# lehduong/Knowledge-Distillation-by-Replacing-Cheap-Conv

Measured on AMD Instinct MI355X. Metric: images/sec KD train step, DeepLabV3+(WRN38) student 1024x2048, higher is better.
Workload: dtype bf16; 1 GPU; KD train step (teacher fwd + student fwd + CE/KD/hint criteria + hint bwd + RAdam), DeepLabV3+(WRN-38) student P92, 1024x2048, 8 img/GPU, random init, teacher through the HIP engine; plan=P92, mode=A, arch=deeplab, hint_loss=mse, per_gpu_batch=8, global_batch=8, parallelism=dp1, teacher_backend=hip, ranks_seen=1

## Files before the change

include/kdcc.h:

```cpp
#ifndef KDCC_H
#define KDCC_H

#include <stddef.h>
#include <stdint.h>

#ifdef __cplusplus
extern "C" {
#endif

typedef void *kd_stream_t;

enum { KD_F32 = 0, KD_BF16 = 1 };
enum {
    KD_OK = 0,
    KD_ERR_INVALID = -1,
    KD_ERR_UNSUPPORTED = -2,
    KD_ERR_WORKSPACE = -3,
    KD_ERR_HIP = -4
};

int kd_version(void);
const char *kd_last_error(void);

typedef struct kd_conv_desc {
    int32_t dtype;
    int32_t N, H, W, Cin;
    int32_t Ho, Wo, Cout;
    int32_t kh, kw, stride, pad, dil;
    int32_t ldx;
} kd_conv_desc;

typedef struct kd_conv_epilogue {
    const void *res_pre;  int32_t ld_res_pre;
    const void *mask;     int32_t ld_mask;     const float *mask_scale;
    const void *res_post; int32_t ld_res_post;
    void *out_raw;        int32_t ld_raw;      int32_t raw_f32;
    void *out_act;        int32_t ld_act;      const float *act_scale; const float *act_shift; int32_t act_relu;
    float *bn_sums;
    const void *cls_w;    float *cls_out;      int32_t ld_cls;      int32_t ncls;
} kd_conv_epilogue;
int32_t kd_conv2d_cls_supported(const kd_conv_desc *d, const kd_conv_epilogue *ep);

int kd_conv2d_fwd(const kd_conv_desc *d, const void *x, const void *w_packed,
                  const kd_conv_epilogue *ep, kd_stream_t stream);
int32_t kd_conv2d_bn_sums_rows(const kd_conv_desc *d, const kd_conv_epilogue *ep);
size_t kd_bn_sums_finish_workspace(int32_t rows, int32_t C);
int kd_bn_sums_finish(const float *part, int32_t rows, int32_t C, float *s1, float *s2, void *workspace, size_t workspace_bytes,
                      kd_stream_t stream);

int32_t kd_conv1x1_dual_supported(const kd_conv_desc *d, int32_t Cin2, int32_t ldx2, const kd_conv_epilogue *ep);
int kd_conv1x1_dual_fwd(const kd_conv_desc *d, const void *x, const void *x2, int32_t Cin2, int32_t ldx2, const void *w_cat,
                        const kd_conv_epilogue *ep, kd_stream_t stream);

int kd_conv_set_persist_cus(int32_t n);

enum { KD_PACK_FWD = 0, KD_PACK_DGRAD = 1 };
int kd_pack_conv_weight(const float *src, void *dst, int32_t dtype, int32_t mode,
                        int32_t Cout, int32_t Cin, int32_t kh, int32_t kw, int32_t cin_pad,
                        kd_stream_t stream);

size_t kd_pw_wgrad_workspace(int32_t M, int32_t Cin, int32_t Cout);
int kd_pw_wgrad(int32_t dtype, int32_t M, int32_t Cin, int32_t Cout,
                const void *a, int32_t lda, const void *dy, int32_t ldy,
                float *dw, int32_t accumulate, void *workspace, size_t workspace_bytes,
                kd_stream_t stream);

size_t kd_conv2d_wgrad_workspace(const kd_conv_desc *d);
int kd_conv2d_wgrad(const kd_conv_desc *d, const void *x, const void *dy, int32_t ld_dy, float *dw,
                    int32_t accumulate, void *workspace, size_t workspace_bytes, kd_stream_t stream);

typedef struct kd_dw_desc {
    int32_t dtype;
    int32_t N, H, W, C;
    int32_t k, pad, dil;
    int32_t ldx, ldy;
} kd_dw_desc;
typedef struct kd_dw_epilogue {
    const void *res_pre;  int32_t ld_res_pre;
    const void *mask;     int32_t ld_mask;     const float *mask_scale;
    const void *res_post; int32_t ld_res_post;
} kd_dw_epilogue;
int kd_pack_dw_weight(const float *src , float *dst ,
                      int32_t C, int32_t k, int32_t flip, kd_stream_t stream);
int kd_dwconv_fwd(const kd_dw_desc *d, const void *x, const float *w_taps, const float *bias,
                  const kd_dw_epilogue *ep, void *y, kd_stream_t stream);
int kd_dwconv_fwd_sum(const kd_dw_desc *d, int32_t n, const void *const *xs, const float *const *w_taps, void *y,
                      kd_stream_t stream);
int kd_dwconv_fwd_fanout(const kd_dw_desc *d, int32_t n, const void *x, const float *const *w_taps, void *const *ys,
                         kd_stream_t stream);
size_t kd_dwconv_wgrad_workspace(const kd_dw_desc *d);
int kd_dwconv_wgrad(const kd_dw_desc *d, const void *x, const void *dy, int32_t ld_dy,
                    float *dw, int32_t accumulate, void *workspace, size_t workspace_bytes,
                    kd_stream_t stream);
size_t kd_dwconv_wgrad_multi_workspace(const kd_dw_desc *d, int32_t n);
int kd_dwconv_wgrad_multi(const kd_dw_desc *d, int32_t n, const void *x, const void *const *dys, int32_t ld_dy,
                          float *const *dws, int32_t accumulate, void *workspace, size_t workspace_bytes,
                          kd_stream_t stream);

int64_t kd_lattice_rows(int32_t N, int32_t H, int32_t W, int32_t dil);
int32_t kd_dwconv_lattice_ok(const kd_dw_desc *d, int32_t n);
int kd_lattice_rows_move(int32_t dtype, int32_t N, int32_t H, int32_t W, int32_t C, int32_t dil, void *img, int32_t ld_img,
                         void *rows, int32_t ld_rows, int32_t to_rows, kd_stream_t stream);
int kd_dwconv_fwd_fanout_lattice(const kd_dw_desc *d, int32_t n, const void *x, const float *const *w_taps, void *const *ys,
                                 kd_stream_t stream);
int kd_dwconv_fwd_sum_lattice(const kd_dw_desc *d, int32_t n, const void *const *xs, const float *const *w_taps, void *y,
                              kd_stream_t stream);
int kd_dwconv_wgrad_multi_lattice(const kd_dw_desc *d, int32_t n, const void *x, const void *const *dys, float *const *dws,
                                  int32_t accumulate, void *workspace, size_t workspace_bytes ,
                                  kd_stream_t stream);

int kd_stem_conv(int32_t dtype, const float *x_nchw, const float *w, void *y,
                 int32_t N, int32_t H, int32_t W, kd_stream_t stream);
int kd_stem_conv_pool(const float *x_nchw, const float *w, void *y_raw, void *y_act, const float *scale,
                      const float *shift, int32_t N, int32_t H, int32_t W, kd_stream_t stream);

int kd_maxpool3x3s2(int32_t dtype, const void *x, int32_t ldx, void *y_raw, int32_t ld_raw,
                    void *y_act, int32_t ld_act, const float *scale, const float *shift,
                    int32_t N, int32_t H, int32_t W, int32_t C, kd_stream_t stream);

int kd_upsample_bilinear_ac(const void *x, int32_t x_dtype, int32_t ldx, void *y, int32_t y_dtype, int32_t ldy,
                            int32_t N, int32_t H, int32_t W, int32_t C, int32_t Ho, int32_t Wo,
                            kd_stream_t stream);

int kd_upsample_bilinear(const void *x, int32_t x_dtype, int32_t ldx, void *y, int32_t y_dtype, int32_t ldy,
// ... 279 lines not shown
```

knowledge-distillation-by-replacing-cheap-conv_amd/_lib.py:

```python
import ctypes as C
import os

_HERE = os.path.dirname(os.path.abspath(__file__))
_sel = os.environ.get("KDCC_LIB", "")
LIB_PATH = (os.path.join(_HERE, "libkdcc_hip_tuning.so") if _sel == "tuning" else _sel if _sel.endswith(".so")
            else os.path.join(_HERE, "libkdcc_hip.so"))


def build_tuning():
    import subprocess
    subprocess.check_call(["make", "-s", "-j", str(min(8, os.cpu_count() or 1)), "-C", os.path.join(_HERE, "csrc"), "TUNING=1"])

KD_F32, KD_BF16 = 0, 1
KD_PACK_FWD, KD_PACK_DGRAD = 0, 1
KD_ERR_UNSUPPORTED = -2
KD_CIFAR_NCHW, KD_CIFAR_NHWC = 0, 1
KD_SEG_NCHW, KD_SEG_NHWC = 0, 1
KD_OPT_SGD, KD_OPT_ADAM, KD_OPT_ADAMW_REF = 0, 1, 2
KD_OPT_FIRST, KD_OPT_NESTEROV, KD_OPT_AMSGRAD, KD_OPT_MAXIMIZE = 1, 2, 4, 8

c_int, c_i64, c_f, c_vp, c_sz = C.c_int32, C.c_int64, C.c_float, C.c_void_p, C.c_size_t


class ConvDesc(C.Structure):
    _fields_ = [(n, c_int) for n in ("dtype", "N", "H", "W", "Cin", "Ho", "Wo", "Cout", "kh", "kw", "stride", "pad",
                                     "dil", "ldx")]


class ConvEpilogue(C.Structure):
    _fields_ = [("res_pre", c_vp), ("ld_res_pre", c_int),
                ("mask", c_vp), ("ld_mask", c_int), ("mask_scale", c_vp),
                ("res_post", c_vp), ("ld_res_post", c_int),
                ("out_raw", c_vp), ("ld_raw", c_int), ("raw_f32", c_int),
                ("out_act", c_vp), ("ld_act", c_int), ("act_scale", c_vp), ("act_shift", c_vp), ("act_relu", c_int),
                ("bn_sums", c_vp),
                ("cls_w", c_vp), ("cls_out", c_vp), ("ld_cls", c_int), ("ncls", c_int)]


class DwDesc(C.Structure):
    _fields_ = [(n, c_int) for n in ("dtype", "N", "H", "W", "C", "k", "pad", "dil", "ldx", "ldy")]


class RadamTensor(C.Structure):
    _fields_ = [("p", c_vp), ("g", c_vp), ("exp_avg", c_vp), ("exp_avg_sq", c_vp), ("n", c_i64), ("step", c_int),
                ("lr", c_f), ("beta1", c_f), ("beta2", c_f), ("eps", c_f), ("weight_decay", c_f)]


class OptimTensor(C.Structure):
    _fields_ = [("p", c_vp), ("g", c_vp), ("state", c_vp * 3), ("n", c_i64), ("step", c_i64), ("flags", c_int), ("reserved", c_int),
                ("lr", C.c_double), ("weight_decay", C.c_double), ("eps", C.c_double), ("momentum", C.c_double),
                ("dampening", C.c_double), ("beta1", C.c_double), ("beta2", C.c_double), ("warmup", C.c_double)]


class DwEpilogue(C.Structure):
    _fields_ = [("res_pre", c_vp), ("ld_res_pre", c_int), ("mask", c_vp), ("ld_mask", c_int), ("mask_scale", c_vp),
                ("res_post", c_vp), ("ld_res_post", c_int)]


class DConvDesc(C.Structure):
    _fields_ = [(n, c_int) for n in ("N", "C", "H", "W", "K", "kh", "kw", "stride", "pad", "dil", "groups")]


class View3(C.Structure):
    _fields_ = [("ptr", c_vp), ("dtype", c_int), ("sN", c_i64), ("sC", c_i64), ("sP", c_i64)]


class HrView(C.Structure):
    _fields_ = [("ptr", c_vp), ("H", c_int), ("W", c_int), ("ld", c_int)]


KD_MULTI_MAX = 16


class MultiTargets(C.Structure):
    _fields_ = [("n", c_int), ("t", View3 * KD_MULTI_MAX), ("w", c_f * KD_MULTI_MAX)]


_P = C.POINTER
_SIGS = {
    "kd_version": (c_int, []),
    "kd_last_error": (C.c_char_p, []),
    "kd_conv2d_fwd": (c_int, [_P(ConvDesc), c_vp, c_vp, _P(ConvEpilogue), c_vp]),
    "kd_conv1x1_dual_supported": (c_int, [_P(ConvDesc), c_int, c_int, _P(ConvEpilogue)]),
    "kd_conv1x1_dual_fwd": (c_int, [_P(ConvDesc), c_vp, c_vp, c_int, c_int, c_vp, _P(ConvEpilogue), c_vp]),
    "kd_conv_set_persist_cus": (c_int, [c_int]),
    "kd_conv2d_bn_sums_rows": (c_int, [_P(ConvDesc), _P(ConvEpilogue)]),
    "kd_conv2d_cls_supported": (c_int, [_P(ConvDesc), _P(ConvEpilogue)]),
    "kd_bn_sums_finish_workspace": (c_sz, [c_int, c_int]),
    "kd_bn_sums_finish": (c_int, [c_vp, c_int, c_int, c_vp, c_vp, c_vp, c_sz, c_vp]),
    "kd_pack_conv_weight": (c_int, [c_vp, c_vp, c_int, c_int, c_int, c_int, c_int, c_int, c_int, c_vp]),
    "kd_pw_wgrad_workspace": (c_sz, [c_int, c_int, c_int]),
    "kd_pw_wgrad": (c_int, [c_int, c_int, c_int, c_int, c_vp, c_int, c_vp, c_int, c_vp, c_int, c_vp, c_sz, c_vp]),
    "kd_conv2d_wgrad_workspace": (c_sz, [_P(ConvDesc)]),
    "kd_conv2d_wgrad": (c_int, [_P(ConvDesc), c_vp, c_vp, c_int, c_vp, c_int, c_vp, c_sz, c_vp]),
    "kd_stem_wgrad_workspace": (c_sz, [c_int, c_int, c_int]),
    "kd_stem_wgrad": (c_int, [c_int, c_vp, c_vp, c_int, c_vp, c_int, c_int, c_int, c_int, c_vp, c_sz, c_vp]),
    "kd_maxpool3x3s2_bwd_workspace": (c_sz, [c_int, c_int, c_int, c_int]),
    "kd_maxpool3x3s2_bwd": (c_int, [c_int, c_vp, c_int, c_vp, c_int, c_vp, c_int, c_int, c_int, c_int, c_int, c_vp, c_sz, c_vp]),
    "kd_upsample_bilinear_ac_bwd_workspace": (c_sz, [c_int] * 6),
    "kd_upsample_bilinear_ac_bwd": (c_int, [c_vp, c_int, c_int, c_vp, c_int, c_int, c_int, c_int, c_int, c_int, c_int, c_int, c_vp,
                                            c_sz, c_vp]),
    "kd_zero_insert": (c_int, [c_int, c_vp, c_int, c_vp, c_int, c_int, c_int, c_int, c_int, c_int, c_int, c_int, c_vp]),
    "kd_relu_bn_bwd": (c_int, [c_int, c_vp, c_int, c_vp, c_int, c_vp, c_vp, c_int, c_vp, c_int, c_i64, c_int, c_vp]),
    "kd_channel_sums_workspace": (c_sz, [c_int, c_i64, c_int]),
    "kd_channel_sums": (c_int, [c_int, c_vp, c_int, c_vp, c_int, c_vp, c_int, c_int, c_i64, c_int, c_vp, c_vp, c_vp, c_sz, c_vp]),
    "kd_bn_eval_param_grads": (c_int, [c_vp, c_vp, c_vp, c_vp, c_vp, c_vp, c_vp, c_int, c_int, c_vp]),
    "kd_broadcast_add": (c_int, [c_int, c_vp, c_vp, c_int, c_int, c_i64, c_int, c_f, c_int, c_vp]),
    "kd_conv2d_direct_fwd": (c_int, [_P(DConvDesc), c_vp, c_vp, c_vp, c_vp, c_vp]),
    "kd_conv2d_direct_dgrad": (c_int, [_P(DConvDesc), c_vp, c_vp, c_vp, c_vp]),
    "kd_conv2d_direct_wgrad": (c_int, [_P(DConvDesc), c_vp, c_vp, c_vp, c_vp, c_int, c_vp]),
    "kd_bn2d_fwd": (c_int, [c_vp, c_vp, c_vp, c_vp, c_vp, c_vp, c_vp, c_vp, c_f, c_f, c_int, c_int, c_int, c_int, c_int, c_vp]),
    "kd_bn2d_bwd": (c_int, [c_vp, c_vp, c_vp, c_vp, c_vp, c_vp, c_vp, c_vp, c_vp, c_int, c_int, c_int, c_int, c_int, c_int, c_vp]),
    "kd_bn_nhwc_workspace": (c_sz, [c_i64, c_int]),
    "kd_bn_nhwc_fwd": (c_int, [c_vp, c_int, c_vp, c_int, c_i64, c_int, c_vp, c_vp, c_vp, c_vp, c_vp, c_vp, c_f, c_f, c_int, c_int,
                               c_vp, c_sz, c_vp]),
    "kd_bn_nhwc_bwd": (c_int, [c_vp, c_int, c_vp, c_int, c_vp, c_int, c_vp, c_int, c_vp, c_int, c_i64, c_int, c_vp, c_vp, c_vp, c_vp,
                               c_vp, c_int, c_int, c_int, c_vp, c_sz, c_vp]),
    "kd_bn_nhwc_lp_workspace": (c_sz, [c_i64, c_int]),
    "kd_bn_nhwc_lp_fwd": (c_int, [c_vp, c_int, c_vp, c_int, c_i64, c_int, c_vp, c_vp, c_vp, c_vp, c_vp, c_vp, c_f, c_f, c_int, c_int,
                                  c_vp, c_sz, c_vp]),
    "kd_bn_nhwc_lp_bwd": (c_int, [c_vp, c_int, c_vp, c_int, c_vp, c_int, c_vp, c_int, c_vp, c_int, c_i64, c_int, c_vp, c_vp, c_vp, c_vp,
                                  c_vp, c_int, c_int, c_int, c_vp, c_sz, c_vp]),
    "kd_bn_nhwc_stats": (c_int, [c_vp, c_int, c_i64, c_int, c_vp, c_vp, c_vp, c_f, c_vp, c_sz, c_vp]),
    "kd_bn_nhwc_apply": (c_int, [c_vp, c_int, c_vp, c_int, c_i64, c_int, c_vp, c_vp, c_vp, c_vp, c_vp, c_vp, c_vp, c_f, c_int, c_vp]),
    "kd_avgpool2x2_nhwc": (c_int, [c_vp, c_int, c_vp, c_int, c_int, c_int, c_int, c_int, c_vp]),
    "kd_avgpool2x2_nhwc_bwd": (c_int, [c_vp, c_int, c_vp, c_int, c_int, c_int, c_int, c_int, c_vp]),
    "kd_pack_dw_weight": (c_int, [c_vp, c_vp, c_int, c_int, c_int, c_vp]),
    "kd_dwconv_fwd": (c_int, [_P(DwDesc), c_vp, c_vp, c_vp, _P(DwEpilogue), c_vp, c_vp]),
    "kd_dwconv_fwd_sum": (c_int, [_P(DwDesc), c_int, c_vp, c_vp, c_vp, c_vp]),
    "kd_dwconv_fwd_fanout": (c_int, [_P(DwDesc), c_int, c_vp, c_vp, c_vp, c_vp]),
    "kd_dwconv_wgrad_workspace": (c_sz, [_P(DwDesc)]),
    "kd_dwconv_wgrad": (c_int, [_P(DwDesc), c_vp, c_vp, c_int, c_vp, c_int, c_vp, c_sz, c_vp]),
    "kd_dwconv_wgrad_multi_workspace": (c_sz, [_P(DwDesc), c_int]),
    "kd_dwconv_wgrad_multi": (c_int, [_P(DwDesc), c_int, c_vp, c_vp, c_int, c_vp, c_int, c_vp, c_sz, c_vp]),
    "kd_lattice_rows": (c_i64, [c_int, c_int, c_int, c_int]),
    "kd_dwconv_lattice_ok": (c_int, [_P(DwDesc), c_int]),
    "kd_lattice_rows_move": (c_int, [c_int, c_int, c_int, c_int, c_int, c_int, c_vp, c_int, c_vp, c_int, c_int, c_vp]),
    "kd_dwconv_fwd_fanout_lattice": (c_int, [_P(DwDesc), c_int, c_vp, c_vp, c_vp, c_vp]),
    "kd_dwconv_fwd_sum_lattice": (c_int, [_P(DwDesc), c_int, c_vp, c_vp, c_vp, c_vp]),
    "kd_dwconv_wgrad_multi_lattice": (c_int, [_P(DwDesc), c_int, c_vp, c_vp, c_vp, c_int, c_vp, c_sz, c_vp]),
    "kd_stem_conv": (c_int, [c_int, c_vp, c_vp, c_vp, c_int, c_int, c_int, c_vp]),
    "kd_scale_by_device_scalar": (c_int, [c_vp, c_int, c_i64, c_vp, c_vp]),
    "kd_pointwise_small": (c_int, [c_vp, c_int, c_vp, c_vp, c_vp, c_int, c_i64, c_int, c_int, c_vp]),
    "kd_conv3x3_small": (c_int, [c_vp, c_int, c_vp, c_vp, c_vp, c_int, c_vp, c_int, c_int, c_int, c_int, c_int, c_int, c_vp]),
    "kd_stem_conv_pool": (c_int, [c_vp, c_vp, c_vp, c_vp, c_vp, c_vp, c_int, c_int, c_int, c_vp]),
    "kd_maxpool3x3s2": (c_int, [c_int, c_vp, c_int, c_vp, c_int, c_vp, c_int, c_vp, c_vp, c_int, c_int, c_int, c_int, c_vp]),
    "kd_upsample_bilinear_ac": (c_int, [c_vp, c_int, c_int, c_vp, c_int, c_int, c_int, c_int, c_int, c_int, c_int, c_int, c_vp]),
    "kd_upsample_bilinear": (c_int, [c_vp, c_int, c_int, c_vp, c_int, c_int, c_int, c_int, c_int, c_int, c_int, c_int, c_int, c_vp]),
    "kd_gated_conv": (c_int, [c_int, c_vp, c_int, c_vp, c_int, c_vp, c_vp, c_int, c_i64, c_int, c_vp]),
    "kd_edge_attention": (c_int, [c_int, c_vp, c_int, c_vp, c_vp, c_vp, c_i64, c_vp]),
    "kd_edge_aspp": (c_int, [c_int, c_vp, c_int, c_int, c_vp, c_vp, c_vp, c_vp, c_int, c_int, c_int, c_int, c_int, c_vp]),
    "kd_canny_workspace": (c_sz, [c_int, c_int, c_int]),
    "kd_canny": (c_int, [c_vp, c_int, c_int, c_int, c_int, c_int, c_int, c_vp, c_vp, c_vp, c_sz, c_vp]),
    "kd_canny_continue": (c_int, [c_int, c_int, c_int, c_int, c_vp, c_vp, c_vp, c_sz, c_vp]),
    "kd_aspp_image_pool_workspace": (c_sz, [c_int, c_int, c_int]),
    "kd_aspp_image_pool": (c_int, [c_int, c_vp, c_int, c_vp, c_vp, c_vp, c_vp, c_int, c_int, c_int, c_int, c_int, c_int,
                                   c_vp, c_sz, c_vp]),
    "kd_aspp_image_pool_sums": (c_int, [c_int, c_vp, c_vp, c_vp, c_vp, c_vp, c_int, c_int, c_int, c_int, c_int, c_int, c_vp, c_sz, c_vp]),
    "kd_bn_fold": (c_int, [c_vp, c_vp, c_vp, c_vp, c_f, c_vp, c_vp, c_int, c_vp]),
    "kd_copy_cast": (c_int, [c_vp, c_int, c_i64, c_i64, c_i64, c_vp, c_int, c_i64, c_i64, c_i64, c_int, c_int, c_i64, c_vp]),
    "kd_loss_workspace": (c_sz, [c_int, c_int, c_i64]),
    "kd_kldiv": (c_int, [_P(View3), _P(View3), c_f, c_int, c_int, c_i64, c_vp, _P(View3), c_f, c_vp, c_sz, c_vp]),
    "kd_hint_mse": (c_int, [_P(View3), _P(View3), c_f, c_int, c_int, c_i64, c_vp, _P(View3), c_f, c_vp, c_sz, c_vp]),
    "kd_weighted_hint_mse": (c_int, [_P(View3), _P(View3), c_vp, c_int, c_int, c_int, c_i64, c_vp, _P(View3), c_f, c_vp,
                                     c_sz, c_vp]),
    "kd_ce2d": (c_int, [_P(View3), c_vp, c_int, c_int, c_int, c_i64, c_vp, c_vp, c_sz, c_vp]),
    "kd_ce2d_up": (c_int, [c_vp, c_vp, c_int, c_int, c_int, c_int, c_int, c_int, c_int, c_int, c_vp, c_vp, c_sz, c_vp]),
    "kd_kldiv_up": (c_int, [c_vp, c_vp, c_f, c_int, c_int, c_int, c_int, c_int, c_int, c_int, c_vp, c_vp, c_sz, c_vp]),
    "kd_logit_metrics_up": (c_int, [c_vp, c_vp, c_vp, c_int, c_int, c_int, c_int, c_int, c_int, c_int, c_int, c_vp, c_vp, c_vp, c_int,
                                    c_vp, c_sz, c_vp]),
# ... 113 lines not shown
```

knowledge-distillation-by-replacing-cheap-conv_amd/csrc/conv_common.h:

```cpp
#pragma once
#include "igemm_core.h"

namespace kdconv {
struct ConvParams {
    const void *x;
    const void *w;
    int M, H, W, Cin, Ho, Wo, Cout, kh, kw, stride, pad, dil, ldx;
    int HoWo, nkc, nk, Ktot, tiles_n, ntiles, tiles_m, tn_group;
    int vec_ok;
    int epi_batch;
    int tune;
    int stagger_us;
    const void *x2;
    int ldx2, nk1;
    kd_conv_epilogue ep;
};
}
using kdconv::ConvParams;

namespace {

__device__ __forceinline__ void wait_vm_stores(int nst)
{
    if (nst == 16) asm volatile("s_waitcnt vmcnt(16) lgkmcnt(0)" ::: "memory");
    else if (nst == 32) asm volatile("s_waitcnt vmcnt(32) lgkmcnt(0)" ::: "memory");
    else if (nst == 48) asm volatile("s_waitcnt vmcnt(48) lgkmcnt(0)" ::: "memory");
    else if (nst == 20) asm volatile("s_waitcnt vmcnt(20) lgkmcnt(0)" ::: "memory");
    else if (nst == 36) asm volatile("s_waitcnt vmcnt(36) lgkmcnt(0)" ::: "memory");
    else asm volatile("s_waitcnt vmcnt(0) lgkmcnt(0)" ::: "memory");
    __builtin_amdgcn_s_barrier();
}

__device__ __forceinline__ void wait_vm_only(int nst)
{
    if (nst == 16) asm volatile("s_waitcnt vmcnt(16)" ::: "memory");
    else if (nst == 32) asm volatile("s_waitcnt vmcnt(32)" ::: "memory");
    else if (nst == 48) asm volatile("s_waitcnt vmcnt(48)" ::: "memory");
    else if (nst == 20) asm volatile("s_waitcnt vmcnt(20)" ::: "memory");
    else if (nst == 36) asm volatile("s_waitcnt vmcnt(36)" ::: "memory");
    else asm volatile("s_waitcnt vmcnt(0)" ::: "memory");
}

__device__ __forceinline__ uint2 ig_pack_acc(const f32x4_t &v) { return make_uint2(pack_bf16x2(v[0], v[1]), pack_bf16x2(v[2], v[3])); }
__device__ __forceinline__ uint2 ig_pack_acc(const uint2 &v) { return v; }

__device__ __forceinline__ uint32_t pack_bf16x2_v(float lo, float hi)
{
    typedef __bf16 bf16x2_t __attribute__((ext_vector_type(2)));
    typedef float f32x2_t __attribute__((ext_vector_type(2)));
    return __builtin_bit_cast(uint32_t, __builtin_convertvector((f32x2_t){lo, hi}, bf16x2_t));
}
__device__ __forceinline__ void st8_v(bf16_t *p, const float (&v)[8])
{
    *(uint4 *)p = make_uint4(pack_bf16x2_v(v[0], v[1]), pack_bf16x2_v(v[2], v[3]), pack_bf16x2_v(v[4], v[5]), pack_bf16x2_v(v[6], v[7]));
}

typedef float f32x2_v __attribute__((ext_vector_type(2)));
typedef short i16x2_v __attribute__((ext_vector_type(2)));
typedef unsigned int u32x4_v __attribute__((ext_vector_type(4)));
__device__ __forceinline__ __amdgpu_buffer_rsrc_t rows_rsrc(const void *base)
{
    return __builtin_amdgcn_make_buffer_rsrc((void *)base, 0, 0x7fffffff, 0x00020000);
}
__device__ __forceinline__ uint32_t act_pair(float lo, float hi, f32x2_v sc, f32x2_v sh, i16x2_v relu_lo)
{
    const f32x2_v r = __builtin_elementwise_fma((f32x2_v){lo, hi}, sc, sh);
    const i16x2_v q = __builtin_bit_cast(i16x2_v, pack_bf16x2_v(r[0], r[1]));
    return __builtin_bit_cast(uint32_t, __builtin_elementwise_max(q, relu_lo));
}

template <int MI, int NOPS_, int PT = 1, typename ACC = f32x4_t, int OUTS = 0>
__device__ __forceinline__ void ig_epilogue_rows16(const ConvParams &p, char *patch, ACC (&acc)[MI][4], int mw, int nw,
                                                   int lane)
{
    typedef bf16_t T;
    constexpr int NOPS = NOPS_ & 3;
    constexpr bool SUMS = (NOPS_ & 4) != 0;
    constexpr bool OSUMS = NOPS_ == 8;
    static_assert((MI == 8 || (MI == 4 && !(NOPS_ & 12))) && NOPS_ >= 0 && (NOPS_ <= 7 || NOPS_ == 8) && NOPS_ != 4,
                  "128-row wave sub-tiles (64 rows at a time: conv_row_duo_kernel, no sums); eval-BN sums need the mask operand, output sums no operand");
    const kd_conv_epilogue &e = p.ep;
    asm volatile("" : "+v"(lane));
    const int frow = lane & 15, fq = lane >> 4;
    const int c0 = nw + (lane & 7) * 8, lrow = lane >> 3, c2 = (lane & 7) * 2;
    float mscale[8], ascale[8], ashift[8];
#pragma unroll
    for (int q = 0; q < 8; ++q) { mscale[q] = 1.f; ascale[q] = 1.f; ashift[q] = 0.f; }
    const bool has_p = NOPS == 3 || (NOPS > 0 && e.res_pre != nullptr), has_m = NOPS == 3 || (NOPS > 0 && e.mask != nullptr),
               has_q = NOPS == 3 || (NOPS > 0 && e.res_post != nullptr);
    const float relu_lo = e.act_relu ? 0.f : -INFINITY;
    if (has_m && e.mask_scale) ld8(e.mask_scale + c0, mscale);
    if (e.act_scale) ld8(e.act_scale + c0, ascale);
    if (e.act_shift) ld8(e.act_shift + c0, ashift);
    const int mwu = __builtin_amdgcn_readfirstlane(mw);
    const __amdgpu_buffer_rsrc_t rs_raw = rows_rsrc((OUTS & 1) ? (const T *)e.out_raw + (size_t)mwu * e.ld_raw : nullptr);
    const __amdgpu_buffer_rsrc_t rs_act = rows_rsrc((OUTS & 2) ? (const T *)e.out_act + (size_t)mwu * e.ld_act : nullptr);
    const uint32_t vo_raw = (uint32_t)(lrow * e.ld_raw + c0) * 2u, vo_act = (uint32_t)(lrow * e.ld_act + c0) * 2u;
    const short relu_w = e.act_relu ? (short)0 : (short)-32768;
    const i16x2_v relu_i16 = {relu_w, relu_w};
    const T *s0 = (const T *)(has_p ? e.res_pre : has_m ? e.mask : e.res_post);
    const int ld0 = has_p ? e.ld_res_pre : has_m ? e.ld_mask : e.ld_res_post;
    const T *s1 = (const T *)(has_p && has_m ? e.mask : e.res_post);
    const int ld1 = has_p && has_m ? e.ld_mask : e.ld_res_post;
    constexpr int nops = NOPS;
    const bool m_in1 = has_p && has_m, q_in1 = has_q && nops == 2;
    uint4 ra[8], rb[8], rc[NOPS == 3 ? 8 : 1];
    auto rowof = [&](int pass) { return (size_t)(mw + pass * 8 + lrow); };
    auto load64 = [&](const T *src, int ld, int hb, uint4 (&r)[8]) __attribute__((always_inline)) {
        if constexpr (OUTS != 0) {
            const __amdgpu_buffer_rsrc_t rs = rows_rsrc(src + (size_t)__builtin_amdgcn_readfirstlane(mw) * ld);
            const uint32_t vo = (uint32_t)(lrow * ld + c0) * 2u;
#pragma unroll
            for (int ps = 0; ps < 8; ++ps) {
                const u32x4_v q = __builtin_amdgcn_raw_buffer_load_b128(rs, vo, (hb * 8 + ps) * 16 * ld, 0);
                r[ps] = make_uint4(q[0], q[1], q[2], q[3]);
            }
        } else {
#pragma unroll
            for (int ps = 0; ps < 8; ++ps) r[ps] = *(const uint4 *)(src + rowof(hb * 8 + ps) * ld + c0);
        }
    };
    float bs1[8], bs2[8];
#pragma unroll
    for (int q = 0; q < 8; ++q) { bs1[q] = 0.f; bs2[q] = 0.f; }
    uint2 pk[MI][4];
#pragma unroll
    for (int i = 0; i < MI; ++i)
#pragma unroll
        for (int j = 0; j < 4; ++j) pk[i][j] = ig_pack_acc(acc[i][j]);
    if (nops >= 1) load64(s0, ld0, 0, ra);
    if (nops >= 2) load64(s1, ld1, 0, rb);
    if (nops == 1 && MI == 8) load64(s0, ld0, 1, rb);
    if constexpr (NOPS == 3) load64((const T *)e.res_post, e.ld_res_post, 0, rc);
    asm volatile("" ::"v"(ascale[0]), "v"(ascale[1]), "v"(ascale[2]), "v"(ascale[3]), "v"(ascale[4]), "v"(ascale[5]), "v"(ascale[6]),
                 "v"(ascale[7]), "v"(ashift[0]), "v"(ashift[1]), "v"(ashift[2]), "v"(ashift[3]), "v"(ashift[4]), "v"(ashift[5]),
                 "v"(ashift[6]), "v"(ashift[7]));
    if (NOPS > 0)
        asm volatile("" ::"v"(mscale[0]), "v"(mscale[1]), "v"(mscale[2]), "v"(mscale[3]), "v"(mscale[4]), "v"(mscale[5]), "v"(mscale[6]),
                     "v"(mscale[7]));
    const f32x2_v asc2[4] = {{ascale[0], ascale[1]}, {ascale[2], ascale[3]}, {ascale[4], ascale[5]}, {ascale[6], ascale[7]}};
    const f32x2_v ash2[4] = {{ashift[0], ashift[1]}, {ashift[2], ashift[3]}, {ashift[4], ashift[5]}, {ashift[6], ashift[7]}};
#pragma unroll
    for (int hb = 0; hb < MI / 4; ++hb) {
        if (nops >= 2 && hb == 1) { load64(s0, ld0, 1, ra); load64(s1, ld1, 1, rb); }
        if constexpr (NOPS == 3) { if (hb == 1) load64((const T *)e.res_post, e.ld_res_post, 1, rc); }
#pragma unroll
        for (int ig = 0; ig < 4; ig += PT) {
#pragma unroll
            for (int it = 0; it < PT; ++it) {
                const int i = 4 * hb + ig + it;
#pragma unroll
                for (int j = 0; j < 4; ++j) *(uint2 *)(patch + it * 2048 + frow * 128 + (((j * 4 + fq) ^ frow) << 3)) = pk[i][j];
            }
            __builtin_amdgcn_fence(__ATOMIC_RELEASE, "wavefront");
            __builtin_amdgcn_wave_barrier();
            __builtin_amdgcn_fence(__ATOMIC_ACQUIRE, "wavefront");
#pragma unroll
            for (int it = 0; it < PT; ++it) {
            const int ii = ig + it;
            const char *pt = patch + it * 2048;
#pragma unroll
            for (int h = 0; h < 2; ++h) {
                const int row = h * 8 + lrow, ps = 2 * ii + h;
                const size_t m = rowof(hb * 8 + ps);
                const uint2 lo = *(const uint2 *)(pt + row * 128 + ((c2 ^ row) << 3));
                const uint2 hi = *(const uint2 *)(pt + row * 128 + (((c2 + 1) ^ row) << 3));
                const uint4 rawv = make_uint4(lo.x, lo.y, hi.x, hi.y);
                float v[8], t[8];
                ld8((const bf16_t *)&rawv, v);
                const uint4 o0 = (hb == 1 && nops == 1) ? rb[ps] : ra[ps], o1 = rb[ps];
                if (NOPS >= 1) asm volatile("" ::"v"(o0.x), "v"(o0.y), "v"(o0.z), "v"(o0.w));
                if (NOPS >= 2) asm volatile("" ::"v"(o1.x), "v"(o1.y), "v"(o1.z), "v"(o1.w));
                if constexpr (NOPS == 3) asm volatile("" ::"v"(rc[ps].x), "v"(rc[ps].y), "v"(rc[ps].z), "v"(rc[ps].w));
                if (has_p) {
                    ld8((const T *)&o0, t);
#pragma unroll
                    for (int q = 0; q < 8; ++q) v[q] += t[q];
                }
                if (has_m) {
                    const uint4 om = m_in1 ? o1 : o0;
                    ld8((const T *)&om, t);
#pragma unroll
                    for (int q = 0; q < 8; ++q) v[q] = t[q] > 0.f ? v[q] * mscale[q] : 0.f;
                    if constexpr (SUMS) {
#pragma unroll
                        for (int q = 0; q < 8; ++q) { bs1[q] += v[q]; bs2[q] = fmaf(v[q], t[q], bs2[q]); }
                    }
                }
                if (has_q) {
                    const uint4 oq = NOPS == 3 ? rc[NOPS == 3 ? ps : 0] : (q_in1 ? o1 : o0);
                    ld8((const T *)&oq, t);
#pragma unroll
                    for (int q = 0; q < 8; ++q) v[q] += t[q];
                }
                if constexpr (OSUMS) {
#pragma unroll
                    for (int q = 0; q < 8; ++q) bs1[q] += v[q];
                }
                if constexpr (OUTS != 0) {
                    const int srow = (hb * 8 + ps) * 16;
                    if constexpr ((OUTS & 1) != 0) {
                        const u32x4_v o = nops == 0 ? (u32x4_v){rawv.x, rawv.y, rawv.z, rawv.w}
                                                    : (u32x4_v){pack_bf16x2_v(v[0], v[1]), pack_bf16x2_v(v[2], v[3]), pack_bf16x2_v(v[4], v[5]), pack_bf16x2_v(v[6], v[7])};
                        __builtin_amdgcn_raw_buffer_store_b128(o, rs_raw, vo_raw + (uint32_t)(srow * e.ld_raw), 0, 0);
                    }
                    if constexpr ((OUTS & 2) != 0) {
                        const u32x4_v o = {act_pair(v[0], v[1], asc2[0], ash2[0], relu_i16), act_pair(v[2], v[3], asc2[1], ash2[1], relu_i16),
                                           act_pair(v[4], v[5], asc2[2], ash2[2], relu_i16), act_pair(v[6], v[7], asc2[3], ash2[3], relu_i16)};
#ifdef KDCC_TUNING
                        if (p.tune & 128) { asm volatile("" ::"v"(o)); continue; }
                        if (p.tune & 256) { *(u32x4_v *)((T *)e.out_act + (size_t)(((m & 15) + 16 * (blockIdx.x * 8 + (threadIdx.x >> 6))) % 4096) * e.ld_act + c0) = o; continue; }
#endif
                        __builtin_amdgcn_raw_buffer_store_b128(o, rs_act, vo_act + (uint32_t)(srow * e.ld_act), 0, 0);
                    }
                    continue;
                }
                if (OUTS ? (OUTS & 1) != 0 : e.out_raw != nullptr) {
                    if (nops == 0) *(uint4 *)((T *)e.out_raw + m * e.ld_raw + c0) = rawv;
                    else if (OUTS) st8_v((T *)e.out_raw + m * e.ld_raw + c0, v);
                    else st8((T *)e.out_raw + m * e.ld_raw + c0, v);
                }
                if (OUTS ? (OUTS & 2) != 0 : e.out_act != nullptr) {
#pragma unroll
                    for (int q = 0; q < 8; ++q) {
                        t[q] = fmaxf(v[q] * ascale[q] + ashift[q], relu_lo);
                    }
#ifdef KDCC_TUNING
                    if (p.tune & 128) { asm volatile("" ::"v"(t[0]), "v"(t[1]), "v"(t[2]), "v"(t[3]), "v"(t[4]), "v"(t[5]), "v"(t[6]), "v"(t[7])); continue; }
                    if (p.tune & 256) { st8((T *)e.out_act + (size_t)(((m & 15) + 16 * (blockIdx.x * 8 + (threadIdx.x >> 6))) % 4096) * e.ld_act + c0, t); continue; }
#endif
                    if (OUTS) st8_v((T *)e.out_act + m * e.ld_act + c0, t);
                    else st8((T *)e.out_act + m * e.ld_act + c0, t);
                }
            }
            }
            __builtin_amdgcn_fence(__ATOMIC_RELEASE, "wavefront");
            __builtin_amdgcn_wave_barrier();
            __builtin_amdgcn_fence(__ATOMIC_ACQUIRE, "wavefront");
        }
    }
    if constexpr (SUMS || OSUMS) {
#pragma unroll
        for (int q = 0; q < 8; ++q) {
#pragma unroll
            for (int sft = 8; sft < 64; sft <<= 1) {
                bs1[q] += __shfl_xor(bs1[q], sft, 64);
                bs2[q] += __shfl_xor(bs2[q], sft, 64);
            }
        }
        if (lane < 8) {
            float *dst = e.bn_sums + (size_t)(mw >> 7) * 2 * p.Cout + c0;
            *(float4 *)dst = make_float4(bs1[0], bs1[1], bs1[2], bs1[3]);
            *(float4 *)(dst + 4) = make_float4(bs1[4], bs1[5], bs1[6], bs1[7]);
            *(float4 *)(dst + p.Cout) = make_float4(bs2[0], bs2[1], bs2[2], bs2[3]);
            *(float4 *)(dst + p.Cout + 4) = make_float4(bs2[4], bs2[5], bs2[6], bs2[7]);
        }
    }
}

struct LwEpiConsts {
    float mscale[8], ascale[8], ashift[8];
};
template <int NOPS_>
__device__ __forceinline__ void lw_epilogue_consts(const ConvParams &p, int nw, int lane, LwEpiConsts &k)
{
    constexpr int NOPS = NOPS_ & 3;
    const kd_conv_epilogue &e = p.ep;
    asm volatile("" : "+v"(lane));
    const int c0 = nw + (lane & 7) * 8;
#pragma unroll
    for (int q = 0; q < 8; ++q) { k.mscale[q] = 1.f; k.ascale[q] = 1.f; k.ashift[q] = 0.f; }
    const bool has_m = NOPS == 3 || (NOPS > 0 && e.mask != nullptr);
    if (has_m && e.mask_scale) ld8(e.mask_scale + c0, k.mscale);
    if (e.act_scale) ld8(e.act_scale + c0, k.ascale);
    if (e.act_shift) ld8(e.act_shift + c0, k.ashift);
}

template <int NOPS_, int OUTS>
__device__ __forceinline__ void lw_epilogue_rows16(const ConvParams &p, char *patch, uint2 (&acc)[8][4], int mw, int nw, int lane, const LwEpiConsts &kc)
{
    typedef bf16_t T;
    constexpr int NOPS = NOPS_ & 3;
    constexpr bool SUMS = (NOPS_ & 4) != 0;
    static_assert(NOPS_ >= 0 && NOPS_ <= 7 && NOPS_ != 4 && OUTS >= 1 && OUTS <= 3, "operands | 4 (eval-BN sums, with the mask operand); raw / act / both");
    const kd_conv_epilogue &e = p.ep;
    asm volatile("" : "+v"(lane));
    const int frow = lane & 15, fq = lane >> 4;
    const int c0 = nw + (lane & 7) * 8, lrow = lane >> 3, c2 = (lane & 7) * 2;
    const bool has_p = NOPS == 3 || (NOPS > 0 && e.res_pre != nullptr), has_m = NOPS == 3 || (NOPS > 0 && e.mask != nullptr),
               has_q = NOPS == 3 || (NOPS > 0 && e.res_post != nullptr);
    const int mwu = __builtin_amdgcn_readfirstlane(mw);
    const __amdgpu_buffer_rsrc_t rs_raw = rows_rsrc((OUTS & 1) ? (const T *)e.out_raw + (size_t)mwu * e.ld_raw : nullptr);
    const __amdgpu_buffer_rsrc_t rs_act = rows_rsrc((OUTS & 2) ? (const T *)e.out_act + (size_t)mwu * e.ld_act : nullptr);
    const uint32_t vo_raw = (uint32_t)(lrow * e.ld_raw + c0) * 2u, vo_act = (uint32_t)(lrow * e.ld_act + c0) * 2u;
    const short relu_w = e.act_relu ? (short)0 : (short)-32768;
    const i16x2_v relu_i16 = {relu_w, relu_w};
    const T *s0 = (const T *)(has_p ? e.res_pre : has_m ? e.mask : e.res_post);
    const int ld0 = has_p ? e.ld_res_pre : has_m ? e.ld_mask : e.ld_res_post;
    const T *s1 = (const T *)(has_p && has_m ? e.mask : e.res_post);
    const int ld1 = has_p && has_m ? e.ld_mask : e.ld_res_post;
    constexpr int nops = NOPS;
    const bool m_in1 = has_p && has_m, q_in1 = has_q && nops == 2;
    uint4 ra[8], rb[8], rc[NOPS == 3 ? 8 : 1];
    auto load64 = [&](const T *src, int ld, int hb, uint4 (&r)[8]) __attribute__((always_inline)) {
        const __amdgpu_buffer_rsrc_t rs = rows_rsrc(src + (size_t)mwu * ld);
        const uint32_t vo = (uint32_t)(lrow * ld + c0) * 2u;
#pragma unroll
        for (int ps = 0; ps < 8; ++ps) {
            const u32x4_v q = __builtin_amdgcn_raw_buffer_load_b128(rs, vo, (hb * 8 + ps) * 16 * ld, 0);
            r[ps] = make_uint4(q[0], q[1], q[2], q[3]);
        }
    };
    float bs1[8], bs2[8];
#pragma unroll
    for (int q = 0; q < 8; ++q) { bs1[q] = 0.f; bs2[q] = 0.f; }
    if (nops >= 1) load64(s0, ld0, 0, ra);
    if (nops >= 2) load64(s1, ld1, 0, rb);
    if (nops == 1) load64(s0, ld0, 1, rb);
    if constexpr (NOPS == 3) load64((const T *)e.res_post, e.ld_res_post, 0, rc);
    const f32x2_v asc2[4] = {{kc.ascale[0], kc.ascale[1]}, {kc.ascale[2], kc.ascale[3]}, {kc.ascale[4], kc.ascale[5]}, {kc.ascale[6], kc.ascale[7]}};
    const f32x2_v ash2[4] = {{kc.ashift[0], kc.ashift[1]}, {kc.ashift[2], kc.ashift[3]}, {kc.ashift[4], kc.ashift[5]}, {kc.ashift[6], kc.ashift[7]}};

    auto write_tile = [&](int i) __attribute__((always_inline)) {
        char *pt = patch + (i & 1) * 2048;
#pragma unroll
        for (int j = 0; j < 4; ++j) *(uint2 *)(pt + frow * 128 + (((j * 4 + fq) ^ frow) << 3)) = acc[i][j];
    };
    auto read_tile = [&](int i, uint4 (&r)[2]) __attribute__((always_inline)) {
        const char *pt = patch + (i & 1) * 2048;
#pragma unroll
        for (int h = 0; h < 2; ++h) {
            const int row = h * 8 + lrow;
            const uint2 lo = *(const uint2 *)(pt + row * 128 + ((c2 ^ row) << 3));
            const uint2 hi = *(const uint2 *)(pt + row * 128 + (((c2 + 1) ^ row) << 3));
// ... 249 lines not shown
```

knowledge-distillation-by-replacing-cheap-conv_amd/csrc/conv_igemm.hip:

```cpp
#include <stdlib.h>
#include <atomic>
#include <string.h>

#include "conv_common.h"
#include "conv_select.h"

namespace {

constexpr int EP_LD = 68;

template <int MI_, int WM_, int WN_, int NST_, int RB_, int WPE_ = 2, int PIPE_ = 0> struct Cfg {
    static constexpr int MI = MI_, WM = WM_, WN = WN_, NST = NST_, RB = RB_, WPE = WPE_, PIPE = PIPE_;
    static constexpr int BM = WM * MI * 16, BN = WN * 64;
    static constexpr int STAGE_A = BM * RB, STAGE_B = BN * RB, STAGE = STAGE_A + STAGE_B;
    static constexpr int PR = 1024 / RB;
    static constexpr int NW = WM * WN;
    static constexpr int GA = BM / PR / NW, GB = BN / PR / NW;
    static constexpr int LDS_BYTES = NST * STAGE;
    static_assert(NW * 32 * EP_LD * 4 <= LDS_BYTES && NW * 16 * MI * 128 <= LDS_BYTES, "epilogue patches must fit the stage buffers");
    static_assert(LDS_BYTES <= 160 * 1024, "LDS budget");
};
typedef Cfg<4, 4, 2, 3, 128> CfgNarrow;
typedef Cfg<8, 2, 4, 2, 128, 2, 1> CfgWide;
typedef Cfg<8, 2, 4, 2, 128> CfgWideF;
// ... 848 lines not shown
    const T *__restrict__ xg = (const T *)p.x;
    const T *__restrict__ wg = (const T *)p.w;
    TileWalk walk(p.ntiles);
    if (walk.t >= walk.t_end) return;
    stagger_start(p);

    const int srow = lane / CPR;
    const int chunk = (lane & 7) ^ srow;
    const int frow = lane & 15, fq = lane >> 4;
    const bool early = (p.tune & 2048) ? true : wv < CF::NW / 2;

    int m0 = 0, n0 = 0, a_off0 = 0, b_off0 = 0, s_kt = 0;
    auto setup = [&](int tile) {
        int tn, tm;
        if (p.tn_group > 0) {
            const int per = p.tiles_m * p.tn_group, blk = tile / per, r = tile - blk * per;
            tm = r / p.tn_group;
            tn = blk * p.tn_group + (r - tm * p.tn_group);
        } else {
            tn = tile % p.tiles_n;
            tm = tile / p.tiles_n;
        }
        m0 = tm * CF::BM;
        n0 = tn * CF::BN;
        a_off0 = (m0 + wv * GA * PR + srow) * p.ldx + chunk * EPC;
        b_off0 = (n0 + wv * (PP ? 2 : 1) * GB * PR + srow) * p.Ktot + chunk * EPC;
        s_kt = 0;
    };
    auto stage = [&]() {
        char *la = lds + (s_kt & 1) * CF::STAGE + wv * (GA * 1024);
        static_assert(GA == 4 && GB == 4, "piece groups below");
        const char *ga[GA], *gb[GB];
#pragma unroll
        for (int j = 0; j < GA; ++j) ga[j] = (const char *)(xg + (a_off0 + j * PR * p.ldx + s_kt * BK)) - j * 1024;
        glds16_x4(ga[0], ga[1], ga[2], ga[3], la);
        if constexpr (PP) {
            if (wv < 4) {
                char *lb = lds + (s_kt & 1) * CF::STAGE + CF::STAGE_A + wv * (2 * GB * 1024);
#pragma unroll
                for (int h2 = 0; h2 < 2; ++h2) {
#pragma unroll
                    for (int j = 0; j < GB; ++j)
                        gb[j] = (const char *)(wg + (b_off0 + (h2 * GB + j) * PR * p.Ktot + s_kt * BK)) - j * 1024;
                    glds16_x4(gb[0], gb[1], gb[2], gb[3], lb + h2 * GB * 1024);
                }
            }
        } else {
            char *lb = lds + (s_kt & 1) * CF::STAGE + CF::STAGE_A + wv * (GB * 1024);
#pragma unroll
            for (int j = 0; j < GB; ++j) gb[j] = (const char *)(wg + (b_off0 + j * PR * p.Ktot + s_kt * BK)) - j * 1024;
            glds16_x4(gb[0], gb[1], gb[2], gb[3], lb);
        }
        ++s_kt;
        __builtin_amdgcn_sched_barrier(0);
    };
    const int nk = p.nk;
    auto prologue = [&]() {
        stage();
        if (nk > 1) stage();
    };

    f32x4_t acc[MI][4];
    uint4 a0[MI], b0[4], a1[MI], b1[4];
    auto read_frags = [&](int kt, int ks, uint4 (&a)[MI], uint4 (&b)[4]) __attribute__((always_inline)) {
        const char *sA = lds + (kt & 1) * CF::STAGE;
        const int sw = ((fq + 4 * ks) ^ (lane & 7)) << 4;
        const char *A = sA + (wm * 16 * MI + frow) * RB + sw, *B = sA + CF::STAGE_A + (wn * 64 + frow) * RB + sw;
#pragma unroll
        for (int i = 0; i < MI; ++i) a[i] = *(const uint4 *)(A + i * 16 * RB);
#pragma unroll
        for (int j = 0; j < 4; ++j) b[j] = *(const uint4 *)(B + j * 16 * RB);
        __builtin_amdgcn_sched_barrier(0);
    };
    auto mfmas = [&](const uint4 (&a)[MI], const uint4 (&b)[4]) __attribute__((always_inline)) {
        if (!(p.tune & 8192)) __builtin_amdgcn_s_setprio(2);
#pragma unroll
        for (int i = 0; i < MI; ++i)
#pragma unroll
            for (int j = 0; j < 4; ++j) Mma<T>::run(b[j], a[i], acc[i][j]);
        if (!(p.tune & 8192)) __builtin_amdgcn_s_setprio(0);
        __builtin_amdgcn_sched_barrier(0);
    };

    const int nst_epi = 2 * MI * ((p.ep.out_raw ? 1 : 0) + (p.ep.out_act ? 1 : 0)) + ((NOPS & 12) ? 4 : 0);
    if constexpr (PP) {
        auto offsets = [&](int tile, int &tm0, int &tn0, int &ao, int &bo) {
            int tn, tm;
            if (p.tn_group > 0) {
                const int per = p.tiles_m * p.tn_group, blk = tile / per, r = tile - blk * per;
                tm = r / p.tn_group;
                tn = blk * p.tn_group + (r - tm * p.tn_group);
            } else {
                tn = tile % p.tiles_n;
                tm = tile / p.tiles_n;
            }
            tm0 = tm * CF::BM;
            tn0 = tn * CF::BN;
            ao = tm0 + wv * GA * PR + srow;
            bo = (tn0 + wv * 2 * GB * PR + srow) * p.Ktot + chunk * EPC;
        };
        int it_tile = walk.t, it_k = 0, it_g = 0, it_ao = 0, it_bo = 0, it_m0, it_n0;
        offsets(it_tile, it_m0, it_n0, it_ao, it_bo);
        const T *__restrict__ xg2 = (const T *)p.x2;
        auto issue = [&]() {
            if (it_tile >= walk.t_end) return;
            char *la = lds + (it_g & 1) * CF::STAGE + wv * (GA * 1024);
            const char *ga[GA], *gb[GB];
            const bool second = it_k >= p.nk1;
            const T *src = second ? xg2 : xg;
            const int ldr = second ? p.ldx2 : p.ldx, ks = second ? it_k - p.nk1 : it_k;
            const int a0 = it_ao * ldr + chunk * EPC + ks * BK;
#pragma unroll
            for (int j = 0; j < GA; ++j) ga[j] = (const char *)(src + (a0 + j * PR * ldr)) - j * 1024;
            glds16_x4(ga[0], ga[1], ga[2], ga[3], la);
            if (wv < 4) {
                char *lb = lds + (it_g & 1) * CF::STAGE + CF::STAGE_A + wv * (2 * GB * 1024);
#pragma unroll
                for (int h2 = 0; h2 < 2; ++h2) {
#pragma unroll
                    for (int j = 0; j < GB; ++j)
                        gb[j] = (const char *)(wg + (it_bo + (h2 * GB + j) * PR * p.Ktot + it_k * BK)) - j * 1024;
                    glds16_x4(gb[0], gb[1], gb[2], gb[3], lb + h2 * GB * 1024);
                }
            }
            ++it_g;
            if (++it_k == nk) {
                it_k = 0;
                it_tile += walk.step;
                if (it_tile < walk.t_end) offsets(it_tile, it_m0, it_n0, it_ao, it_bo);
            }
            __builtin_amdgcn_sched_barrier(0);
        };
        auto read_all = [&](int g) __attribute__((always_inline)) {
            read_frags(g, 0, a0, b0);
            read_frags(g, 1, a1, b1);
            asm volatile("s_waitcnt lgkmcnt(0)" ::: "memory");
        };
        int g = 0;
        bool first = true;
        if (wv < 4) { issue(); issue(); } else { issue(); }
        asm volatile("s_waitcnt vmcnt(0)" ::: "memory");
        __builtin_amdgcn_s_barrier();
#pragma unroll 1
        for (int tile = walk.t; tile < walk.t_end; tile += walk.step) {
            int a_dummy, b_dummy;
            offsets(tile, m0, n0, a_dummy, b_dummy);
#pragma unroll
            for (int i = 0; i < MI; ++i)
#pragma unroll
                for (int j = 0; j < 4; ++j) acc[i][j] = (f32x4_t){0.f, 0.f, 0.f, 0.f};
            if (wv < 4) {
#pragma unroll 1
                for (int sc = 0; sc < nk; ++sc, ++g) {
                    read_all(g);
                    __builtin_amdgcn_s_barrier();
                    mfmas(a0, b0);
                    mfmas(a1, b1);
                    asm volatile("s_waitcnt vmcnt(0)" ::: "memory");
                    __builtin_amdgcn_s_barrier();
                    issue();
                }
            } else {
#pragma unroll 1
                for (int sc = 0; sc < nk; ++sc, ++g) {
                    if (sc == 0 && !first) wait_vm_only((p.tune & 64) ? 0 : nst_epi);
                    else asm volatile("s_waitcnt vmcnt(0)" ::: "memory");
                    __builtin_amdgcn_s_barrier();
// ... 208 lines not shown
                __builtin_amdgcn_s_barrier();
                if (DBG) c5 = clock64();
                mfmas();
                if (DBG) { const unsigned long long c6 = clock64(); ph[0] += c1 - c0; ph[1] += c2 - c1; ph[2] += c3 - c2; ph[3] += c4 - c3; ph[4] += c5 - c4; ph[5] += c6 - c5; }
            }
        }
        if (DBG && lane == 0 && tcount == 1) {
            unsigned long long *o = kd_conv_tlog + 256 * 32 * 8 + (blockIdx.x * 8 + wv) * 8;
            for (int q = 0; q < 6; ++q) o[q] = ph[q];
            o[6] = ns;
        }
        ++tcount;
        const int mw = m0 + wm * 128, nw = n0 + wn * 64;
        walk.t += walk.step;
        const bool more = walk.t < walk.t_end;
        if (more) { setup(walk.t); prologue(); }
        if (!(p.tune & 64)) ig_epilogue_rows16<MI, NOPS, 4>(p, lds + NEED + wv * 8192, acc, mw, nw, lane);
        if (!more) break;
        nst = (p.tune & 64) ? 0 : nst_epi;
    }
}

template <typename T>
__global__ void pack_conv_weight_kernel(const float *__restrict__ src, T *__restrict__ dst, int mode, int Cout,
                                        int Cin, int kh, int kw, int cin_pad)
{
    const int taps = kh * kw;
    const size_t total = mode == KD_PACK_FWD ? (size_t)Cout * taps * cin_pad : (size_t)Cin * taps * Cout;
    for (size_t i = (size_t)blockIdx.x * blockDim.x + threadIdx.x; i < total; i += (size_t)gridDim.x * blockDim.x) {
        float v = 0.f;
        if (mode == KD_PACK_FWD) {
            const int ci = (int)(i % cin_pad);
            const size_t r = i / cin_pad;
            const int t = (int)(r % taps), co = (int)(r / taps);
            if (ci < Cin) v = src[((size_t)co * Cin + ci) * taps + t];
        } else {
            const int co = (int)(i % Cout);
            const size_t r = i / Cout;
            const int tf = (int)(r % taps), ci = (int)(r / taps);
            const int t = taps - 1 - tf;
            v = src[((size_t)co * Cin + ci) * taps + t];
        }
        Elem<T>::st(dst + i, v);
    }
}

}

template <typename CF> constexpr bool tile_is(ConvTile t) { return CF::BM == 256 && CF::BN == t.bn && CF::RB == t.rb; }
static_assert(tile_is<CfgNarrow>(CONV_TILE_128) && tile_is<CfgWide>(CONV_TILE_256) && tile_is<CfgWideF>(CONV_TILE_256) && tile_is<CfgDeep>(CONV_TILE_256_K64) &&
                  tile_is<CfgHalf>(CONV_TILE_128_K64) && tile_is<CfgNarrow2>(CONV_TILE_128_K64) && tile_is<CfgRow>(CONV_TILE_256) && tile_is<CfgRowX>(CONV_TILE_256) &&
                  tile_is<CfgRowF>(CONV_TILE_256) && tile_is<CfgRowXF>(CONV_TILE_256) && tile_is<CfgRowH>(CONV_TILE_128_K64) && tile_is<CfgRowHX>(CONV_TILE_128_K64) &&
                  tile_is<CfgRowN>(CONV_TILE_128_K64) && CfgRow::MAXDIL == CONV_ROW_MAXDIL && CfgRowX::MAXDIL == CONV_ROWX_MAXDIL && CfgRowN::MAXDIL == CONV_ROWN_MAXDIL,
              "conv_select.h restates a tile configuration wrongly");

static const ConvSwitches &conv_switches()
{
    static const ConvSwitches sw = [] {
        auto on = [](const char *name) { const char *v = getenv(name); return !(v && v[0] == '0') ? 1 : 0; };
        auto num = [](const char *name, int dflt) { const char *v = getenv(name); return v ? atoi(v) : dflt; };
        ConvSwitches s;
        s.lw = on("KDCC_CONV_LW"); s.pp = on("KDCC_CONV_PP"); s.persist = on("KDCC_CONV_PERSIST");
        s.dual = on("KDCC_CONV_DUAL"); s.epi_batch = on("KDCC_EPI_BATCH");
        s.duo = num("KDCC_CONV_DUO", 0); s.tngroup = num("KDCC_CONV_TNGROUP", 4); s.persist_cus = num("KDCC_PERSIST_CUS", 0);
        if (const char *v = getenv("KDCC_CONV_LW_PW")) s.lw_pw = v[0] == '1';
        if (const char *e = getenv("KDCC_CONV_CFG"))
            s.cfg = !strcmp(e, "narrow") ? CONV_CFG_NARROW : !strcmp(e, "norow") ? CONV_CFG_NOROW : !strcmp(e, "half") ? CONV_CFG_HALF
                  : !strcmp(e, "deep") ? CONV_CFG_DEEP : !strcmp(e, "narrow1") ? CONV_CFG_NARROW1 : CONV_CFG_DEFAULT;
        s.tune = KD_TUNING_ENV_INT("KDCC_CONV_TUNE");
        s.stagger_us = KD_TUNING_ENV_INT("KDCC_CONV_STAGGER");
        return s;
    }();
    return sw;
}

static int conv_ncu()
{
    static const int ncu = [] {
        int dev = 0, n = 0;
        return hipGetDevice(&dev) == hipSuccess && hipDeviceGetAttribute(&n, hipDeviceAttributeMultiprocessorCount, dev) == hipSuccess && n > 0 ? n : 256;
    }();
    return ncu;
}
static ConvSel conv_select_here(const kd_conv_desc *d, const kd_conv_epilogue *ep, int cin1) { return conv_select(d, ep, cin1, conv_ncu(), conv_switches()); }

extern "C" int32_t kd_conv2d_bn_sums_rows(const kd_conv_desc *d, const kd_conv_epilogue *ep)
{
    if (!d || !ep || d->dtype != KD_BF16 || d->N <= 0 || d->Ho <= 0 || d->Wo <= 0) return 0;
    return conv_select_here(d, ep, 0).sums_rows;
}

extern "C" int32_t kd_conv2d_cls_supported(const kd_conv_desc *d, const kd_conv_epilogue *ep)
{
    if (!d || !ep || !ep->cls_w || !ep->cls_out || d->dtype != KD_BF16 || d->N <= 0 || d->Ho <= 0 || d->Wo <= 0) return 0;
    if (d->Cout != 256 || ep->ncls < 1 || ep->ncls > 32 || ep->ld_cls < ep->ncls || !kd_aligned16(ep->cls_w)) return 0;
    if (ep->out_raw || ep->out_act || ep->bn_sums || ep->raw_f32) return 0;
    return conv_select_here(d, ep, 0).cls_ok;
}

static std::atomic<int> g_persist_cus{-1};
extern "C" int kd_conv_set_persist_cus(int32_t n)
{
    KD_REQUIRE(n >= 0, KD_ERR_INVALID, "kd_conv_set_persist_cus: n must be >= 0 (0 = one workgroup per CU)");
    g_persist_cus.store(n);
    return KD_OK;
}

static int conv2d_fwd_impl(const kd_conv_desc *d, const void *x, const void *w_packed, const kd_conv_epilogue *ep,
                           kd_stream_t stream, const void *x2, int cin1, int ldx2)
{
    KD_REQUIRE(d && x && w_packed && ep, KD_ERR_INVALID, "kd_conv2d_fwd: null argument");
    KD_REQUIRE(d->dtype == KD_F32 || d->dtype == KD_BF16, KD_ERR_INVALID, "kd_conv2d_fwd: bad dtype %d", d->dtype);
    const int es = kd_elem_size(d->dtype);
    const int bk = 128 / es;
    KD_REQUIRE(d->N > 0 && d->H > 0 && d->W > 0 && d->Cin > 0 && d->Cout > 0 && d->Ho > 0 && d->Wo > 0,
               KD_ERR_INVALID, "kd_conv2d_fwd: non-positive dimension");
    KD_REQUIRE((d->kh == 1 && d->kw == 1) || (d->kh == 3 && d->kw == 3), KD_ERR_UNSUPPORTED,
               "kd_conv2d_fwd: kernel %dx%d not supported (1x1, 3x3)", d->kh, d->kw);
    KD_REQUIRE(d->stride >= 1 && d->dil >= 1 && d->pad >= 0, KD_ERR_INVALID, "kd_conv2d_fwd: bad stride/dil/pad");
    KD_REQUIRE(d->Cin % bk == 0, KD_ERR_UNSUPPORTED, "kd_conv2d_fwd: Cin=%d must be a multiple of %d", d->Cin, bk);
    KD_REQUIRE(d->ldx >= (x2 ? cin1 : d->Cin) && (d->ldx * es) % 16 == 0, KD_ERR_INVALID, "kd_conv2d_fwd: bad ldx=%d", d->ldx);
    KD_REQUIRE(kd_aligned16(x) && kd_aligned16(w_packed), KD_ERR_INVALID, "kd_conv2d_fwd: x/w must be 16-B aligned");
    const int ho = (d->H + 2 * d->pad - d->dil * (d->kh - 1) - 1) / d->stride + 1;
    const int wo = (d->W + 2 * d->pad - d->dil * (d->kw - 1) - 1) / d->stride + 1;
    KD_REQUIRE(ho == d->Ho && wo == d->Wo, KD_ERR_INVALID, "kd_conv2d_fwd: Ho/Wo (%d,%d) inconsistent, expect (%d,%d)",
               d->Ho, d->Wo, ho, wo);
    const long long in_elems = (long long)d->N * d->H * d->W * d->ldx;
    const long long w_elems = (long long)d->Cout * d->kh * d->kw * d->Cin;
    KD_REQUIRE(in_elems < (1ll << 31) && w_elems < (1ll << 31), KD_ERR_UNSUPPORTED,
               "kd_conv2d_fwd: tensor exceeds 2^31 elements");
    const bool cls = ep->cls_w != nullptr || ep->cls_out != nullptr;
    KD_REQUIRE(!cls || (!x2 && kd_conv2d_cls_supported(d, ep)), KD_ERR_UNSUPPORTED,
               "kd_conv2d_fwd: the classifier epilogue needs conv_row_lw_kernel with one N tile and nothing else in the epilogue (ask kd_conv2d_cls_supported first)");
    KD_REQUIRE(cls || ep->out_raw || ep->out_act, KD_ERR_INVALID, "kd_conv2d_fwd: no output requested");

    const ConvSwitches &sw = conv_switches();
    ConvParams p;
    p.x = x; p.w = w_packed;
    p.M = d->N * d->Ho * d->Wo;
    p.H = d->H; p.W = d->W; p.Cin = d->Cin; p.Ho = d->Ho; p.Wo = d->Wo; p.Cout = d->Cout;
    p.kh = d->kh; p.kw = d->kw; p.stride = d->stride; p.pad = d->pad; p.dil = d->dil; p.ldx = d->ldx;
    p.HoWo = d->Ho * d->Wo;
    p.Ktot = d->kh * d->kw * d->Cin;
    p.x2 = x2; p.ldx2 = ldx2;
    p.ep = *ep;
    p.epi_batch = sw.epi_batch; p.tune = sw.tune; p.stagger_us = sw.stagger_us;
    const ConvSel sel = conv_select_here(d, ep, x2 ? cin1 : 0);
    p.vec_ok = sel.vec_ok;
    p.nkc = sel.nkc; p.nk = sel.nk; p.nk1 = sel.nk1;
    p.tiles_m = sel.tiles_m; p.tiles_n = sel.tiles_n; p.ntiles = sel.ntiles; p.tn_group = sel.tn_group;
    KD_REQUIRE(!ep->bn_sums || kd_conv2d_bn_sums_rows(d, ep) > 0, KD_ERR_UNSUPPORTED,
               "kd_conv2d_fwd: bn_sums is not produced by the kernel this problem selects (ask kd_conv2d_bn_sums_rows first)");
    if (ep->bn_sums) KD_NOTE_KERNEL(ep->mask ? "bn_sums_epilogue" : "out_sums_epilogue");
    if (cls) KD_NOTE_KERNEL("cls_epilogue");
    if (x2)
        KD_REQUIRE(sel.dual_ok, KD_ERR_UNSUPPORTED,
                   "kd_conv1x1_dual_fwd: this shape does not select conv_igemm_persist_kernel<pp> (ask kd_conv1x1_dual_supported first)");
    hipStream_t s = (hipStream_t)stream;
    const int nops = sel.nops, gpc = g_persist_cus.load(std::memory_order_relaxed);
    const dim3 grid(conv_grid(sel, conv_persist_cus(gpc < 0 ? sw.persist_cus : gpc, conv_ncu())));
#define KD_LAUNCH(threads, ...) hipLaunchKernelGGL((__VA_ARGS__), grid, dim3(threads), 0, s, p)
#define KD_CASE(epi, ...) case epi: KD_LAUNCH(512, __VA_ARGS__); break;
    switch (sel.kernel) {
    case CONV_ROW_DUO: KD_NOTE_KERNEL("conv_row_duo_kernel");
        KD_REQUIRE(kd_launch_conv_row_duo(p, sel.epi, grid.x, s), KD_ERR_UNSUPPORTED, "kd_conv2d_fwd: no conv_row_duo_kernel instantiation"); break;
    case CONV_ROW_PERSIST_DBG: KD_NOTE_KERNEL("conv_row_persist_kernel<dbg>");
        switch (sel.epi) {
        KD_CASE(0, conv_row_persist_kernel<CfgRow, 0, true, true>) KD_CASE(1, conv_row_persist_kernel<CfgRow, 1, true, true>)
        default: KD_LAUNCH(512, conv_row_persist_kernel<CfgRow, 2, true, true>);
        } break;
    case CONV_ROW_LW: KD_NOTE_KERNEL("conv_row_lw_kernel");
        KD_REQUIRE(kd_launch_conv_row_lw(p, sel.epi, grid.x, s), KD_ERR_UNSUPPORTED, "kd_conv2d_fwd: no conv_row_lw_kernel instantiation for %d epilogue operands", nops); break;
    case CONV_ROW_PERSIST_PP: KD_NOTE_KERNEL("conv_row_persist_kernel<pp>");
        switch (sel.epi) {
        KD_CASE(0, conv_row_persist_kernel<CfgRow, 0, false, true>) KD_CASE(5, conv_row_persist_kernel<CfgRow, 5, false, true>)
        KD_CASE(6, conv_row_persist_kernel<CfgRow, 6, false, true>) KD_CASE(1, conv_row_persist_kernel<CfgRow, 1, false, true>)
        KD_CASE(2, conv_row_persist_kernel<CfgRow, 2, false, true>) default: KD_LAUNCH(512, conv_row_persist_kernel<CfgRow, 3, false, true>);
        } break;
    case CONV_ROW_PERSIST_LOCKSTEP: KD_NOTE_KERNEL("conv_row_persist_kernel<lockstep>");
        switch (sel.epi) {
        KD_CASE(0, conv_row_persist_kernel<CfgRow, 0>) KD_CASE(1, conv_row_persist_kernel<CfgRow, 1>) default: KD_LAUNCH(512, conv_row_persist_kernel<CfgRow, 2>);
        } break;
    case CONV_PW_LW: KD_NOTE_KERNEL("conv_pw_lw_kernel");
        KD_REQUIRE(kd_launch_conv_pw_lw(p, sel.epi, grid.x, s), KD_ERR_UNSUPPORTED, "kd_conv2d_fwd: no conv_pw_lw_kernel instantiation for %d epilogue operands", nops); break;
    case CONV_IGEMM_PERSIST_PP_DUAL:
    case CONV_IGEMM_PERSIST_PP:
        if (sel.kernel == CONV_IGEMM_PERSIST_PP_DUAL) KD_NOTE_KERNEL("conv_igemm_persist_kernel<pp,dual>");
        else KD_NOTE_KERNEL("conv_igemm_persist_kernel<pp>");
        switch (sel.epi) {
        KD_CASE(8, conv_igemm_persist_kernel<CfgWide, 8, true>) KD_CASE(0, conv_igemm_persist_kernel<CfgWide, 0, true>) KD_CASE(5, conv_igemm_persist_kernel<CfgWide, 5, true>)
        KD_CASE(6, conv_igemm_persist_kernel<CfgWide, 6, true>) KD_CASE(1, conv_igemm_persist_kernel<CfgWide, 1, true>) KD_CASE(2, conv_igemm_persist_kernel<CfgWide, 2, true>)
        default: KD_LAUNCH(512, conv_igemm_persist_kernel<CfgWide, 3, true>);
        } break;
    case CONV_IGEMM_PERSIST_LOCKSTEP: KD_NOTE_KERNEL("conv_igemm_persist_kernel<lockstep>");
        switch (sel.epi) {
        KD_CASE(0, conv_igemm_persist_kernel<CfgWide, 0>) KD_CASE(1, conv_igemm_persist_kernel<CfgWide, 1>) default: KD_LAUNCH(512, conv_igemm_persist_kernel<CfgWide, 2>);
        } break;
    case CONV_ROW_HALF: KD_NOTE_KERNEL("conv_igemm_row_kernel<half>");
        if (sel.row_x) KD_LAUNCH(256, conv_igemm_row_kernel<bf16_t, CfgRowHX>);
        else KD_LAUNCH(256, conv_igemm_row_kernel<bf16_t, CfgRowH>);
        break;
    case CONV_ROW_TALL: KD_NOTE_KERNEL("conv_row_tall_kernel");
        KD_REQUIRE(kd_launch_conv_row_tall(p, sel.epi, grid.x, s), KD_ERR_UNSUPPORTED, "kd_conv2d_fwd: no conv_row_tall_kernel instantiation for %d epilogue operands", nops); break;
    case CONV_ROW_PP128: KD_NOTE_KERNEL("conv_row_pp128_kernel");
        switch (sel.epi) {
        KD_CASE(-1, conv_row_pp128_kernel<0, true>)
        KD_CASE(0, conv_row_pp128_kernel<0>) KD_CASE(5, conv_row_pp128_kernel<5>) KD_CASE(6, conv_row_pp128_kernel<6>) KD_CASE(1, conv_row_pp128_kernel<1>)
        default: KD_LAUNCH(512, conv_row_pp128_kernel<2>);
        } break;
    case CONV_ROW_NARROW: KD_NOTE_KERNEL("conv_igemm_row_kernel<narrow>"); KD_LAUNCH(512, conv_igemm_row_kernel<bf16_t, CfgRowN>); break;
    case CONV_ROW_X: KD_NOTE_KERNEL("conv_igemm_row_kernel<x>"); KD_LAUNCH(512, conv_igemm_row_kernel<bf16_t, CfgRowX>); break;
    case CONV_ROW_WIDE: KD_NOTE_KERNEL("conv_igemm_row_kernel<wide>"); KD_LAUNCH(512, conv_igemm_row_kernel<bf16_t, CfgRow>); break;
    case CONV_ROW_F32_X: KD_NOTE_KERNEL("conv_igemm_row_kernel<f32,x>"); KD_LAUNCH(512, conv_igemm_row_kernel<float, CfgRowXF>); break;
    case CONV_ROW_F32_WIDE: KD_NOTE_KERNEL("conv_igemm_row_kernel<f32,wide>"); KD_LAUNCH(512, conv_igemm_row_kernel<float, CfgRowF>); break;
    case CONV_IGEMM_HALF: KD_NOTE_KERNEL("conv_igemm_kernel<half>");
        if (sel.plain) KD_LAUNCH(64 * CfgWideF::NW, conv_igemm_kernel<bf16_t, CfgWideF>);
        else KD_LAUNCH(64 * CfgHalf::NW, conv_igemm_kernel<bf16_t, CfgHalf>);
        break;
    case CONV_IGEMM_WIDE: KD_NOTE_KERNEL("conv_igemm_kernel<wide>");
        if (sel.plain) KD_LAUNCH(64 * CfgWideF::NW, conv_igemm_kernel<bf16_t, CfgWideF>);
        else KD_LAUNCH(64 * CfgWide::NW, conv_igemm_kernel<bf16_t, CfgWide>);
        break;
    case CONV_IGEMM_DEEP: KD_NOTE_KERNEL("conv_igemm_kernel<deep>"); KD_LAUNCH(64 * CfgDeep::NW, conv_igemm_kernel<bf16_t, CfgDeep>); break;
    case CONV_IGEMM_NARROW: KD_NOTE_KERNEL("conv_igemm_kernel<narrow>"); KD_LAUNCH(64 * CfgNarrow::NW, conv_igemm_kernel<bf16_t, CfgNarrow>); break;
    case CONV_IGEMM_NARROW2: KD_NOTE_KERNEL("conv_igemm_kernel<narrow2>"); KD_LAUNCH(64 * CfgNarrow2::NW, conv_igemm_kernel<bf16_t, CfgNarrow2>); break;
    case CONV_IGEMM_F32_WIDE: KD_NOTE_KERNEL("conv_igemm_kernel<f32,wide>"); KD_LAUNCH(64 * CfgWideF::NW, conv_igemm_kernel<float, CfgWideF>); break;
    case CONV_IGEMM_F32_DEEP: KD_NOTE_KERNEL("conv_igemm_kernel<f32,deep>"); KD_LAUNCH(64 * CfgDeep::NW, conv_igemm_kernel<float, CfgDeep>); break;
    case CONV_IGEMM_F32_NARROW: KD_NOTE_KERNEL("conv_igemm_kernel<f32,narrow>"); KD_LAUNCH(64 * CfgNarrow::NW, conv_igemm_kernel<float, CfgNarrow>); break;
    }
#undef KD_CASE
#undef KD_LAUNCH
    KD_CHECK_LAUNCH("kd_conv2d_fwd");
    return KD_OK;
}

extern "C" int kd_conv2d_fwd(const kd_conv_desc *d, const void *x, const void *w_packed, const kd_conv_epilogue *ep,
                             kd_stream_t stream)
{
    return conv2d_fwd_impl(d, x, w_packed, ep, stream, nullptr, 0, 0);
}

static bool dual_shape_ok(const kd_conv_desc *d, int Cin2, int ldx2, const kd_conv_epilogue *ep, kd_conv_desc *tot)
{
    if (!d || !ep || d->dtype != KD_BF16 || d->kh != 1 || d->kw != 1 || d->stride != 1 || d->pad != 0 || d->H != d->Ho || d->W != d->Wo) return false;
    if (Cin2 <= 0 || d->Cin % 64 != 0 || Cin2 % 64 != 0 || ldx2 < Cin2 || (ldx2 * 2) % 16 != 0) return false;
    *tot = *d;
    tot->Cin = d->Cin + Cin2;
    return conv_select_here(tot, ep, d->Cin).dual_ok;
}

extern "C" int32_t kd_conv1x1_dual_supported(const kd_conv_desc *d, int32_t Cin2, int32_t ldx2, const kd_conv_epilogue *ep)
{
    kd_conv_desc tot;
    return dual_shape_ok(d, Cin2, ldx2, ep, &tot) ? 1 : 0;
}

extern "C" int kd_conv1x1_dual_fwd(const kd_conv_desc *d, const void *x, const void *x2, int32_t Cin2, int32_t ldx2, const void *w_cat,
                                   const kd_conv_epilogue *ep, kd_stream_t stream)
{
    KD_REQUIRE(d && x && x2 && w_cat && ep, KD_ERR_INVALID, "kd_conv1x1_dual_fwd: null argument");
    KD_REQUIRE(kd_aligned16(x2), KD_ERR_INVALID, "kd_conv1x1_dual_fwd: x2 must be 16-B aligned");
    kd_conv_desc tot;
    KD_REQUIRE(dual_shape_ok(d, Cin2, ldx2, ep, &tot), KD_ERR_UNSUPPORTED,
               "kd_conv1x1_dual_fwd: needs a bf16 1x1 / stride-1 conv on the persistent 256 x 256 tiles (kd_conv1x1_dual_supported)");
    KD_REQUIRE((long long)d->N * d->H * d->W * ldx2 < (1ll << 31), KD_ERR_UNSUPPORTED, "kd_conv1x1_dual_fwd: x2 exceeds 2^31 elements");
    return conv2d_fwd_impl(&tot, x, w_cat, ep, stream, x2, d->Cin, ldx2);
}

extern "C" int kd_debug_conv_tlog(unsigned long long *dst, size_t bytes)
{
    if (conv_switches().tune & 1024) return kd_lw_tlog_copy(dst, bytes) == 0 ? KD_OK : KD_ERR_HIP;
    return hipMemcpyFromSymbol(dst, HIP_SYMBOL(kd_conv_tlog), bytes < sizeof(kd_conv_tlog) ? bytes : sizeof(kd_conv_tlog), 0,
// ... 25 lines not shown
```

knowledge-distillation-by-replacing-cheap-conv_amd/csrc/conv_select.h:

```cpp
#pragma once
#include <stdint.h>

#include "../../include/kdcc.h"

enum ConvKernel {
    CONV_ROW_DUO, CONV_ROW_PERSIST_DBG, CONV_ROW_LW, CONV_ROW_PERSIST_PP, CONV_ROW_PERSIST_LOCKSTEP,
    CONV_PW_LW, CONV_IGEMM_PERSIST_PP_DUAL, CONV_IGEMM_PERSIST_PP, CONV_IGEMM_PERSIST_LOCKSTEP,
    CONV_ROW_HALF, CONV_ROW_TALL, CONV_ROW_PP128,
    CONV_ROW_NARROW, CONV_ROW_F32_X, CONV_ROW_X, CONV_ROW_F32_WIDE, CONV_ROW_WIDE,
    CONV_IGEMM_HALF, CONV_IGEMM_WIDE, CONV_IGEMM_DEEP, CONV_IGEMM_NARROW, CONV_IGEMM_NARROW2,
    CONV_IGEMM_F32_WIDE, CONV_IGEMM_F32_DEEP, CONV_IGEMM_F32_NARROW,
};
enum ConvCfgSwitch { CONV_CFG_DEFAULT, CONV_CFG_NARROW, CONV_CFG_NOROW, CONV_CFG_HALF, CONV_CFG_DEEP, CONV_CFG_NARROW1 };

struct ConvSwitches {
    int lw = 1;
    int pp = 1;
    int persist = 1;
    int cfg = CONV_CFG_DEFAULT;
    int duo = 0;
    int lw_pw = 0;
    int tngroup = 4;
    int dual = 1;
    int epi_batch = 1;
    int persist_cus = 0;
    int tune = 0, stagger_us = 0;
};

struct ConvTile { int bn, rb; };
constexpr ConvTile CONV_TILE_128{128, 128}, CONV_TILE_256{256, 128}, CONV_TILE_256_K64{256, 64}, CONV_TILE_128_K64{128, 64};
constexpr int CONV_ROW_MAXDIL = 32, CONV_ROWX_MAXDIL = 64, CONV_ROWN_MAXDIL = 64;
struct ConvSel {
    ConvKernel kernel;
    int epi;
    bool row_x, plain;
    int vec_ok, nops;
    int nkc, nk, nk1;
    int tiles_m, tiles_n, ntiles, tn_group;
    int wg_per_cu;
    int sums_rows;
    bool cls_ok, dual_ok;
};

static inline int conv_persist_cus(int n, int ncu)
{
    if (n <= 0 || n > ncu) n = ncu;
    if (n < 8) n = 8;
    return n - n % 8;
}
static inline unsigned conv_grid(const ConvSel &c, int persist_cus)
{
    if (!c.wg_per_cu) return (unsigned)c.ntiles;
    const int cap = c.wg_per_cu * persist_cus, nwg = c.ntiles < cap ? c.ntiles : cap;
    return (unsigned)((nwg + 7) / 8 * 8);
}

static inline ConvSel conv_select(const kd_conv_desc *d, const kd_conv_epilogue *ep, int cin1, int ncu, const ConvSwitches &sw)
{
    ConvSel c{};
    const bool bf16 = d->dtype == KD_BF16, lw_row = sw.lw != 0, pp_row = sw.pp != 0, dbg = (sw.tune & 512) != 0, sums = ep->bn_sums != nullptr;
    const int es = bf16 ? 2 : 4, M = d->N * d->Ho * d->Wo;
    auto ok = [&](const void *ptr, int ld, int esz) { return !ptr || (((uintptr_t)ptr & 15u) == 0 && (ld * esz) % 16 == 0); };
    c.vec_ok = ok(ep->res_pre, ep->ld_res_pre, es) && ok(ep->mask, ep->ld_mask, es) && ok(ep->res_post, ep->ld_res_post, es) &&
               ok(ep->out_raw, ep->ld_raw, ep->raw_f32 ? 4 : es) && ok(ep->out_act, ep->ld_act, es);
    const int nops = c.nops = (ep->res_pre ? 1 : 0) + (ep->mask ? 1 : 0) + (ep->res_post ? 1 : 0);
    const long long wide_tiles = (long long)((M + 255) / 256) * ((d->Cout + CONV_TILE_256.bn - 1) / CONV_TILE_256.bn);
    int cfg = (d->Cout > 128 && wide_tiles >= 224) ? 1 : 0;
    if (sw.cfg == CONV_CFG_NARROW) cfg = 0;
    else if (sw.cfg == CONV_CFG_DEEP && cfg == 1) cfg = 2;
    else if (sw.cfg == CONV_CFG_NARROW1 && cfg == 0) cfg = 3;
    const bool norow = sw.cfg == CONV_CFG_NOROW, half = sw.cfg == CONV_CFG_HALF;
    const bool row_geom = !norow && d->kh == 3 && d->kw == 3 && d->stride == 1 && d->pad == d->dil && d->W % 256 == 0;
    const bool row_wide = row_geom && cfg == 1 && d->dil <= CONV_ROWX_MAXDIL;
    const bool row_x = c.row_x = row_wide && d->dil > CONV_ROW_MAXDIL;
    const bool row_narrow = row_geom && cfg == 0 && bf16 && d->dil <= CONV_ROWN_MAXDIL;
    const bool persist_ok = sw.persist && !half && bf16 && cfg == 1 && c.vec_ok && !ep->raw_f32 && M % 256 == 0 && d->Cout % 256 == 0 &&
                            (nops <= 2 || (pp_row && !dbg));
    const bool use_row_persist = persist_ok && row_wide && !row_x;
    const bool use_igemm_persist = !use_row_persist && persist_ok && d->kh == 1 && d->stride == 1 && d->pad == 0;
    const bool use_pp128 = !use_row_persist && !use_igemm_persist && !(row_wide && half && bf16) && row_narrow && pp_row && sw.persist &&
                           c.vec_ok && !ep->raw_f32 && nops <= 2 && d->Cout % 128 == 0 && d->W % 512 == 0 && d->dil <= 16 && d->Cin % 32 == 0;
    const bool lone_wave_row = lw_row && bf16 && d->kh == 3 && d->kw == 3 && d->stride == 1 && d->pad == d->dil && d->dil <= 32 && d->H >= 2 * d->dil && !dbg;
    const bool duo_ok = sw.duo > 0 && lone_wave_row && d->W % 256 == 0 && M % 256 == 0 && d->Cout % 128 == 0 && d->Cin % 64 == 0 && c.vec_ok &&
                        !ep->raw_f32 && nops <= 1 && !sums && (long long)(M / 256) * (d->Cout / 128) >= 2 * ncu && (sw.duo >= 2 || d->Cout == 128);
    const bool sums_ok = pp_row && !dbg &&
                         (ep->mask ? (use_row_persist || use_igemm_persist || use_pp128) && !(use_row_persist && d->dil > 32) && nops <= 2
                                   : use_igemm_persist && nops == 0 && ep->out_raw && !ep->out_act && !ep->raw_f32 && !sw.lw_pw);
    c.sums_rows = sums_ok ? (int)((long long)d->N * d->Ho * d->Wo / 128) : 0;
    const int pp_epi = (sums && nops >= 1 && nops <= 2) ? (nops | 4) : nops, two_epi = nops < 2 ? nops : 2, lw_epi = nops | (sums ? 4 : 0);
    int bm = 256;
    ConvTile t = CONV_TILE_256;
    if (duo_ok) {
        c.kernel = CONV_ROW_DUO; c.epi = nops; t = CONV_TILE_128_K64; c.wg_per_cu = 2;
    } else if (use_row_persist) {
        const bool lw = lone_wave_row && pp_row;
        c.kernel = dbg ? CONV_ROW_PERSIST_DBG : lw ? CONV_ROW_LW : (pp_row && d->dil <= 32) ? CONV_ROW_PERSIST_PP : CONV_ROW_PERSIST_LOCKSTEP;
        c.epi = c.kernel == CONV_ROW_LW ? ((ep->cls_w || ep->cls_out) ? 16 : lw_epi) : c.kernel == CONV_ROW_PERSIST_PP ? pp_epi : two_epi;
        c.wg_per_cu = 1;
    } else if (use_igemm_persist) {
        const bool lw = sw.lw_pw && lw_row && pp_row && d->Cin % 128 == 0 && !dbg && !cin1;
        c.kernel = lw ? CONV_PW_LW : !pp_row ? CONV_IGEMM_PERSIST_LOCKSTEP : cin1 ? CONV_IGEMM_PERSIST_PP_DUAL : CONV_IGEMM_PERSIST_PP;
        c.epi = lw ? lw_epi : !pp_row ? two_epi : (sums && nops == 0) ? 8 : pp_epi;
        c.wg_per_cu = 1;
    } else if (row_wide && half && bf16) {
        c.kernel = CONV_ROW_HALF; t = CONV_TILE_128_K64;
    } else if (use_pp128) {
        const bool tall = lw_row && d->Cin % 64 == 0 && d->H > d->dil && !dbg && !(sums && nops == 0);
        c.kernel = tall ? CONV_ROW_TALL : CONV_ROW_PP128;
        c.epi = tall ? lw_epi : dbg ? -1 : pp_epi;
        bm = 512; t = CONV_TILE_128_K64; c.wg_per_cu = 1;
    } else if (row_wide || row_narrow) {
        c.kernel = row_narrow ? CONV_ROW_NARROW : row_x ? (bf16 ? CONV_ROW_X : CONV_ROW_F32_X) : (bf16 ? CONV_ROW_WIDE : CONV_ROW_F32_WIDE);
        if (row_narrow) t = CONV_TILE_128_K64;
    } else if (bf16) {
        c.kernel = cfg == 1 ? (half ? CONV_IGEMM_HALF : CONV_IGEMM_WIDE) : cfg == 2 ? CONV_IGEMM_DEEP : cfg == 3 ? CONV_IGEMM_NARROW : CONV_IGEMM_NARROW2;
        c.plain = cfg == 1 && (sw.tune & 8);
        t = c.plain ? CONV_TILE_256 : cfg == 1 ? (half ? CONV_TILE_128_K64 : CONV_TILE_256) : cfg == 2 ? CONV_TILE_256_K64 : cfg == 3 ? CONV_TILE_128 : CONV_TILE_128_K64;
    } else {
        c.kernel = cfg == 1 ? CONV_IGEMM_F32_WIDE : cfg == 2 ? CONV_IGEMM_F32_DEEP : CONV_IGEMM_F32_NARROW;
        t = cfg == 1 ? CONV_TILE_256 : cfg == 2 ? CONV_TILE_256_K64 : CONV_TILE_128;
    }
    c.nkc = d->Cin / (t.rb / es);
    c.nk = d->kh * d->kw * c.nkc;
    c.nk1 = c.kernel == CONV_IGEMM_PERSIST_PP_DUAL ? cin1 / (t.rb / es) : 0x7fffffff;
    c.tiles_m = (M + bm - 1) / bm;
    c.tiles_n = (d->Cout + t.bn - 1) / t.bn;
    c.ntiles = c.tiles_m * c.tiles_n;
    const int tng = (256 / t.bn) * sw.tngroup;
    c.tn_group = (c.wg_per_cu && bm == 256 && sw.tngroup > 0 && c.tiles_n > tng && c.tiles_n % tng == 0) ? tng : 0;
    c.cls_ok = c.kernel == CONV_ROW_LW && nops == 0 && sw.duo < 2;
    c.dual_ok = c.kernel == CONV_IGEMM_PERSIST_PP_DUAL && sw.dual && cin1 % (t.rb / es) == 0;
    return c;
}

enum WgradKernel { WGRAD_LW, WGRAD_ROW, WGRAD_PW_LW, WGRAD_WIDE, WGRAD_WIDE_GENERAL, WGRAD_TR, WGRAD_BF16, WGRAD_F32 };

struct WgradSwitches {
    int row = 2;
    int lw = 1;
    int wide = 1;
    int wide_general = 0;
    int pw_lw = 1;
    int target = 0, wide_target = 0;
    int nst = 2;
    int il = 1;
    int dbg = 0;
};

struct WgradSel {
    WgradKernel kernel;
    int tiles, tiles_ci, splits, rps;
    unsigned grid[3];
};

constexpr int WR_XROWS = 96;

static inline void wgrad_plan(int dtype, int M, int Cin, int Cout, int taps, WgradSel &c)
{
    const int krows = 128 / (dtype == KD_BF16 ? 2 : 4);
    c.tiles_ci = (Cin + 127) / 128;
    c.tiles = c.tiles_ci * ((Cout + 127) / 128);
    const int stages = (M + krows - 1) / krows;
    const int want = (1024 + c.tiles * taps - 1) / (c.tiles * taps);
    const int max_splits = (stages + 3) / 4;
    c.splits = want > max_splits ? max_splits : want;
    if (c.splits < 1) c.splits = 1;
    c.rps = (stages + c.splits - 1) / c.splits * krows;
    c.splits = (M + c.rps - 1) / c.rps;
}

static inline int wgrad_fill_splits(int per, int max_splits)
{
    int splits = 1;
    double best = -1.0;
    for (int k = 1; k <= 4; ++k) {
        int sp = (256 * k) / per;
        sp = sp < 1 ? 1 : (sp > max_splits ? max_splits : sp);
        const long long w = (long long)sp * per;
        const double fill = (double)w / (double)(((w + 255) / 256) * 256);
        if (fill >= 0.95) return sp;
        if (fill > best) { best = fill; splits = sp; }
    }
    return splits;
}

// ... 63 lines not shown
```

knowledge-distillation-by-replacing-cheap-conv_amd/csrc/losses.hip:

```cpp
#include <algorithm>
#include <type_traits>

#include "kd_common.h"
#include "loss_select.h"

namespace {

template <int K> __device__ __forceinline__ void block_partials(const double (&v)[K], double *const (&out)[K])
{
    __shared__ double w[K][4];
    const int lane = threadIdx.x & 63, wv = threadIdx.x >> 6;
#pragma unroll
    for (int q = 0; q < K; ++q) {
        const double s = wave_sum_d(v[q]);
        if (lane == 0) w[q][wv] = s;
    }
    __syncthreads();
    if (threadIdx.x == 0) {
#pragma unroll
        for (int q = 0; q < K; ++q) out[q][blockIdx.x] = w[q][0] + w[q][1] + w[q][2] + w[q][3];
    }
}

__global__ __launch_bounds__(256) void finish_kernel(const double *partial, int n, double scale, const double *count,
// ... 1368 lines not shown
const PairNhwcLaunch pair_nhwc_launches[] = {KD_PAIR_FORMS(PAIR_KLD), KD_PAIR_FORMS(PAIR_JSD), KD_PAIR_FORMS(PAIR_EKL)};
#undef KD_PAIR_FORMS
static_assert(sizeof(pair_nhwc_launches) / sizeof(pair_nhwc_launches[0]) == LK_PAIR_NHWC_LAST - LK_PAIR_NHWC + 1, "a launch per channels-last form");
}

static int pair_impl(const char *who, int kind, const kd_view3 *s, const kd_view3 *t, float invT, int32_t N, int32_t C, int64_t P,
                     float *loss, const kd_mview3 *grad, float gscale, double loss_scale, void *workspace, kd_stream_t stream)
{
    double *partial = (double *)workspace;
    hipStream_t st = (hipStream_t)stream;
    const LossSel sel = loss_select_pair((LossPair)kind, s, t, grad, N, C, P);
    KD_NOTE_PLUMBING(loss_kernel_name(sel.kernel));
    if (sel.kernel >= LK_PAIR_NHWC && sel.kernel <= LK_PAIR_NHWC_LAST) {
        pair_nhwc_launches[sel.kernel - LK_PAIR_NHWC](sel, st, s->ptr, t->ptr, grad ? grad->ptr : nullptr, C, (long long)N * P, invT, gscale, partial);
    } else {
        auto fn = launch_of(sel.kernel, LK_PAIR_KLD, pair_kernel<PAIR_KLD>, LK_PAIR_JSD, pair_kernel<PAIR_JSD>, LK_PAIR_EKL, pair_kernel<PAIR_EKL>);
        if (!fn) return no_launch(who, sel);
        hipLaunchKernelGGL(fn, dim3(sel.blocks), dim3(256), 0, st, v3(s), v3(t), m3(grad), invT, gscale, N, C, (long long)P, partial);
    }
    KD_CHECK_LAUNCH(who);
    hipLaunchKernelGGL(finish_kernel, dim3(1), dim3(256), 0, st, (const double *)partial, sel.blocks, loss_scale, (const double *)nullptr, loss);
    KD_CHECK_LAUNCH(who);
    return KD_OK;
}

extern "C" int kd_kldiv(const kd_view3 *s, const kd_view3 *t, float temperature, int32_t N, int32_t C, int64_t P, float *loss,
                        const kd_mview3 *grad, float grad_scale, void *workspace, size_t workspace_bytes, kd_stream_t stream)
{
    KD_LOSS_COMMON("kd_kldiv");
    KD_REQUIRE(temperature > 0.f, KD_ERR_INVALID, "kd_kldiv: temperature must be positive");
    const float gscale = grad_scale * temperature / ((float)N * (float)P);
    const double scale = (double)temperature * temperature / ((double)N * (double)P);
    return pair_impl("kd_kldiv", PAIR_KLD, s, t, 1.f / temperature, N, C, P, loss, grad, gscale, scale, workspace, stream);
}

extern "C" int kd_jsdiv(const kd_view3 *s, const kd_view3 *t, float temperature, int32_t N, int32_t C, int64_t P, float *loss,
                        const kd_mview3 *grad, float grad_scale, void *workspace, size_t workspace_bytes, kd_stream_t stream)
{
    KD_LOSS_COMMON("kd_jsdiv");
    KD_REQUIRE(temperature > 0.f, KD_ERR_INVALID, "kd_jsdiv: temperature must be positive");
    const float gscale = grad_scale * temperature / (2.f * (float)N);
    const double scale = (double)temperature * temperature / (2.0 * (double)N);
    return pair_impl("kd_jsdiv", PAIR_JSD, s, t, 1.f / temperature, N, C, P, loss, grad, gscale, scale, workspace, stream);
}

extern "C" int kd_ensemble_kldiv(const kd_view3 *s, const kd_view3 *t, int32_t N, int32_t C, int64_t P, float *loss, const kd_mview3 *grad,
                                 float grad_scale, void *workspace, size_t workspace_bytes, kd_stream_t stream)
{
    KD_LOSS_COMMON("kd_ensemble_kldiv");
    const float gscale = grad_scale / ((float)N * (float)P);
    const double scale = 1.0 / ((double)N * (double)P);
    return pair_impl("kd_ensemble_kldiv", PAIR_EKL, s, t, 1.f, N, C, P, loss, grad, gscale, scale, workspace, stream);
}

extern "C" int kd_hint_mse(const kd_view3 *s, const kd_view3 *t, float num_classes, int32_t N, int32_t C, int64_t P,
                           float *loss, const kd_mview3 *grad, float grad_scale, void *workspace, size_t workspace_bytes,
                           kd_stream_t stream)
{
    KD_LOSS_COMMON("kd_hint_mse");
    double *partial = (double *)workspace;
    const long long numel = (long long)N * C * P;
    const float gscale = grad_scale * 2.f * num_classes / (float)numel;
    hipStream_t st = (hipStream_t)stream;
    const LossSel sel = loss_select_mse(s, t, grad, N, C, P);
    KD_NOTE_PLUMBING(loss_kernel_name(sel.kernel));
    auto vec = [&](auto z) {
        using T = decltype(z);
        hipLaunchKernelGGL(mse_vec_kernel<T>, dim3(sel.blocks), dim3(256), 0, st, (const T *)s->ptr, (const T *)t->ptr,
                           (T *)(grad ? grad->ptr : nullptr), gscale, numel / 8, partial);
    };
    switch (sel.kernel) {
    case LK_MSE_VEC_F32: vec(float{}); break;
    case LK_MSE_VEC_BF16: vec(bf16_t{}); break;
    case LK_MSE_STRIDED:
        hipLaunchKernelGGL(mse_strided_kernel, dim3(sel.blocks), dim3(256), 0, st, v3(s), v3(t), m3(grad), gscale, N, C, (long long)P,
                           s->sC == 1 ? 1 : 0, partial);
        break;
    default: return no_launch("kd_hint_mse", sel);
    }
    KD_CHECK_LAUNCH("kd_hint_mse");
    hipLaunchKernelGGL(finish_kernel, dim3(1), dim3(256), 0, st, (const double *)partial, sel.blocks, (double)num_classes / (double)numel,
                       (const double *)nullptr, loss);
    KD_CHECK_LAUNCH("kd_hint_mse(finish)");
    return KD_OK;
}

extern "C" int kd_weighted_hint_mse(const kd_view3 *s, const kd_view3 *t, const float *w, int32_t w_per_sample, int32_t N,
                                    int32_t C, int64_t P, float *loss, const kd_mview3 *grad, float grad_scale, void *workspace,
                                    size_t workspace_bytes, kd_stream_t stream)
{
    KD_LOSS_COMMON("kd_weighted_hint_mse");
    KD_REQUIRE(w, KD_ERR_INVALID, "kd_weighted_hint_mse: null weight");
    hipStream_t st = (hipStream_t)stream;
    const LossSel sel = loss_select_whmse(N, C, P);
    const dim3 grid((unsigned)sel.chunks, (unsigned)((C + 255) / 256), (unsigned)N);
    double *partial = (double *)workspace;
    float *wsum = (float *)((char *)workspace + sel.aux_off);
    KD_NOTE_PLUMBING(loss_kernel_name(LK_WHMSE));
    hipLaunchKernelGGL(wsum_kernel, dim3(N), dim3(64), 0, st, w, w_per_sample, N, C, wsum);
    hipLaunchKernelGGL(whmse_kernel, grid, dim3(256), 0, st, v3(s), v3(t), m3(grad), w, w_per_sample, (const float *)wsum,
                       grad_scale, N, C, (long long)P, sel.per_chunk, partial);
    KD_CHECK_LAUNCH("kd_weighted_hint_mse");
    hipLaunchKernelGGL(finish_kernel, dim3(1), dim3(256), 0, st, (const double *)partial, sel.blocks, 1.0 / (double)N,
                       (const double *)nullptr, loss);
    KD_CHECK_LAUNCH("kd_weighted_hint_mse(finish)");
    return KD_OK;
}

static int ce2d_impl(const char *who, const kd_view3 *x, const int64_t *target, const float *class_weight, int32_t sum_reduction, int32_t ignore_index,
                     int32_t N, int32_t C, int64_t P, float *loss, void *workspace, size_t workspace_bytes, kd_stream_t stream)
{
    KD_REQUIRE(x && x->ptr && target && loss && workspace, KD_ERR_INVALID, "%s: null argument", who);
    KD_REQUIRE(ok_dt(x->dtype) && N > 0 && C > 0 && P > 0, KD_ERR_INVALID, "%s: bad argument", who);
    KD_REQUIRE(workspace_bytes >= kd_loss_workspace(N, C, P), KD_ERR_WORKSPACE, "%s: workspace too small", who);
    double *partial = (double *)workspace, *count = partial + LOSS_MAX_BLOCKS;
    hipStream_t st = (hipStream_t)stream;
    const LossSel sel = loss_select_ce2d(x, N, C, P);
    KD_NOTE_PLUMBING(loss_kernel_name(sel.kernel));
    auto nhwc = [&](auto z) {
        using T = decltype(z);
        hipLaunchKernelGGL(ce2d_nhwc_kernel<T>, dim3(sel.blocks), dim3(256), sel.lds, st, (const T *)x->ptr, target, ignore_index, C,
                           (long long)N * P, partial, count, class_weight);
    };
    switch (sel.kernel) {
    case LK_CE2D_NHWC_F32: nhwc(float{}); break;
    case LK_CE2D_NHWC_BF16: nhwc(bf16_t{}); break;
    case LK_CE2D:
        hipLaunchKernelGGL(ce2d_kernel, dim3(sel.blocks), dim3(256), 0, st, v3(x), target, ignore_index, N, C, (long long)P, partial, count, class_weight);
        break;
    default: return no_launch(who, sel);
    }
    KD_CHECK_LAUNCH(who);
    hipLaunchKernelGGL(finish_kernel, dim3(1), dim3(256), 0, st, (const double *)partial, sel.blocks, 1.0,
                       sum_reduction ? (const double *)nullptr : (const double *)count, loss);
    KD_CHECK_LAUNCH(who);
    return KD_OK;
}

extern "C" int kd_ce2d(const kd_view3 *x, const int64_t *target, int32_t ignore_index, int32_t N, int32_t C, int64_t P,
                       float *loss, void *workspace, size_t workspace_bytes, kd_stream_t stream)
{
    return ce2d_impl("kd_ce2d", x, target, nullptr, 0, ignore_index, N, C, P, loss, workspace, workspace_bytes, stream);
}

extern "C" int kd_ce2d_weighted(const kd_view3 *x, const int64_t *target, const float *class_weight, int32_t sum_reduction, int32_t ignore_index,
                                int32_t N, int32_t C, int64_t P, float *loss, void *workspace, size_t workspace_bytes, kd_stream_t stream)
{
    return ce2d_impl("kd_ce2d_weighted", x, target, class_weight, sum_reduction, ignore_index, N, C, P, loss, workspace, workspace_bytes, stream);
}

static int ce2d_grad_impl(const char *who, const kd_view3 *x, const int64_t *target, const float *class_weight, int32_t sum_reduction, int32_t ignore_index,
                          int32_t N, int32_t C, int64_t P, const kd_mview3 *grad, float grad_scale, void *workspace, size_t workspace_bytes,
                          kd_stream_t stream)
{
    KD_REQUIRE(x && x->ptr && target && grad && grad->ptr && workspace, KD_ERR_INVALID, "%s: null argument", who);
    KD_REQUIRE(ok_dt(x->dtype) && ok_dt(grad->dtype) && N > 0 && C > 0 && P > 0, KD_ERR_INVALID, "%s: bad argument", who);
    KD_REQUIRE(workspace_bytes >= kd_loss_workspace(N, C, P), KD_ERR_WORKSPACE, "%s: workspace too small", who);
    double *count = (double *)workspace;
    const LossSel sel = loss_flat(LK_CE2D_GRAD, (long long)N * P);
    hipStream_t st = (hipStream_t)stream;
    KD_NOTE_PLUMBING(loss_kernel_name(sel.kernel));
    hipLaunchKernelGGL(ce2d_count_kernel, dim3(sel.blocks), dim3(256), 0, st, target, ignore_index, C, (long long)N * P, count, class_weight);
    KD_CHECK_LAUNCH(who);
    hipLaunchKernelGGL(ce2d_grad_kernel, dim3(sel.blocks), dim3(256), 0, st, v3(x), target, ignore_index, N, C, (long long)P, m3(grad), grad_scale,
                       (const double *)count, sel.blocks, class_weight, (int)sum_reduction);
    KD_CHECK_LAUNCH(who);
// ... 459 lines not shown
```

knowledge-distillation-by-replacing-cheap-conv_amd/engine.py:

```python
import itertools
import os

import torch
from torch import nn

from . import ops
from ._lib import KD_PACK_DGRAD, KD_PACK_FWD
from .lazy import LazyLogits
from .models.students.transform_blocks import DepthwiseSeparableBlock, GateLayer, RandomMask2d
from .models.wider_resnet import IdentityResidualBlock

_SMALL_CONV = os.environ.get("KDCC_SMALL_CONV", "1") != "0"
_SPLIT_DEC_DGRAD = os.environ.get("KDCC_SPLIT_DEC_DGRAD", "1") != "0"
_STEM_POOL = os.environ.get("KDCC_STEM_POOL", "1") != "0"
_DW_SUM = os.environ.get("KDCC_DW_SUM", "1") != "0"
_CONV_DUAL = os.environ.get("KDCC_CONV_DUAL", "1") != "0"
_FUSE_BN_SUMS = os.environ.get("KDCC_FUSE_BN_SUMS", "1") != "0"
_FUSE_GAP = os.environ.get("KDCC_FUSE_GAP", "1") != "0"


class EngineError(RuntimeError):
    pass


# ... 7 lines not shown
def _bn_of(bn_seq):
    return bn_seq[0] if isinstance(bn_seq, nn.Sequential) else bn_seq


def _gate_split(mod):
    if isinstance(mod, nn.Sequential) and len(mod) == 2 and isinstance(mod[1], GateLayer):
        return mod[0], mod[1]
    return mod, None


def _is_masked(mod):
    return (isinstance(mod, nn.Sequential) and len(mod) == 3 and isinstance(mod[0], nn.Conv2d) and isinstance(mod[1], RandomMask2d)
            and isinstance(mod[2], nn.Conv2d))


def _act_gate(bn_seq):
    if isinstance(bn_seq, nn.Sequential) and len(bn_seq) > 1:
        return _gate_split(bn_seq[1])[1]
    return None


class _Site:

    def __init__(self, name, mod):
        mod, self.gate = _gate_split(mod)
        self.name, self.mod = name, mod
        self.cheap = isinstance(mod, DepthwiseSeparableBlock)
        self.masked = _is_masked(mod)
        if self.masked:
            self._init_masked(name, mod)
            return
        if self.cheap and self.gate is not None:
            raise EngineError(f"{name}: a gate behind a cheap-conv block is not supported (gates rank the TEACHER's filters)")
        if not self.cheap and not isinstance(mod, nn.Conv2d):
            raise EngineError(f"{name}: unsupported module {type(mod).__name__} in the student graph")
        conv = mod.pointwise_conv if self.cheap else mod
        self.cout = conv.out_channels
        self.cin = (mod.separable_conv if self.cheap else conv).in_channels
        if self.cheap:
            self.k, self.pad, self.dil = mod.geometry
            self.stride = 1
            if mod.separable_conv.bias is not None or mod.pointwise_conv.bias is not None:
                raise EngineError(f"{name}: biased cheap conv inside the fused graph is not supported")
        else:
            if conv.bias is not None or conv.groups != 1:
                raise EngineError(f"{name}: only bias-free dense convs are supported")
            self.k, self.pad, self.dil, self.stride = conv.kernel_size[0], conv.padding[0], conv.dilation[0], conv.stride[0]
        self.trainable = _is_trainable(mod) or (self.gate is not None and self.gate.weight.requires_grad)

    def _init_masked(self, name, mod):
        conv, mask, pw = mod[0], mod[1], mod[2]
        if self.gate is not None:
            raise EngineError(f"{name}: a gate behind a masked site is not supported")
        if conv.bias is not None or conv.groups != 1 or _is_trainable(conv):
            raise EngineError(f"{name}: the conv in front of a RandomMask2d must be a frozen, bias-free dense conv")
        if pw.bias is not None or pw.kernel_size != (1, 1) or pw.stride != (1, 1) or pw.padding != (0, 0) or pw.groups != 1 or \
                pw.in_channels != conv.out_channels or mask.in_channels != conv.out_channels:
            raise EngineError(f"{name}: the conv behind a RandomMask2d must be a bias-free 1x1 over the masked channels")
        self.cin, self.cout = conv.in_channels, pw.out_channels
        self.k, self.pad, self.dil, self.stride = conv.kernel_size[0], conv.padding[0], conv.dilation[0], conv.stride[0]
        self.trainable = pw.weight.requires_grad


class StudentEngine:
    def __init__(self, net, dtype=torch.bfloat16):
        self.net = net
        self.dtype = dtype
        self.hint_names = []
        self._pack = {}
        self._bn = {}
        self._tape = None
        self.last_hint_names = []
        self.reducer = None
        self.probe_names = []
        self.probe_grads = {}
        self._probe_active = False
        self._probes = set()
        self.is_gscnn = net is not None and hasattr(net, "gate1")
        self._gate_prm = {}
        self._persist = {}
        self.edge_prior = None
        self.exported = None
        self._next_prefix = None
        self.logits_need_grad = False
        self.lazy_logits = os.environ.get("KDCC_LAZY_LOGITS", "1") != "0"
        self._lazy_call = False
        self._differentiable = False

    def compute_edge_prior(self, x_nchw):
        fn = getattr(self.net, "canny_fn", None)
        N, _, H, W = x_nchw.shape
        if fn is None:
            return ops.canny(x_nchw.detach().float().contiguous())
        return fn(x_nchw).reshape(N, H, W).float().contiguous()

    def _final(self):
        return self.net.final_seg if self.is_gscnn else self.net.final

    def _aspp_lead(self, aspp):
        return 2 if hasattr(aspp, "edge_conv") else 1

    def _grad_like(self, p):
        if self.reducer is not None:
            return self.reducer.grad_buffer(p)
        return torch.empty_like(p, dtype=torch.float32, memory_format=torch.contiguous_format)

    def _grad_done(self, p):
        if self.reducer is not None:
            self.reducer.grad_ready(p)

    def _packed(self, p, tag, fn, extra=None):
        key = (id(p), tag)
        ent = self._pack.get(key)
        if ent is not None:
            first = ent[1][0] if isinstance(ent[1], tuple) else ent[1]
        ver = p._version if extra is None else (p._version, extra)
        if ent is None or ent[2] is not p or ent[0] != ver or first.device != p.device:
            ent = (ver, fn(), p)
            self._pack[key] = ent
        return ent[1]

    def drop_caches(self):
        self._pack.clear()
        self._bn.clear()
        self._persist.clear()

    def _w_fwd(self, conv, cin_pad=None, cin_rot=0, cout_pad=None, gate=None):
        def make():
            w = conv.weight if not cin_rot else torch.cat([conv.weight.detach()[:, cin_rot:], conv.weight.detach()[:, :cin_rot]], 1).contiguous()
            if gate is not None:
                gv = gate.weight.detach().float()
                if not bool((gv != 0).all()):
                    raise EngineError("a gate folded into a conv's weights has a zero entry: d loss / d gate is recovered from the "
                                      "gated output by a division (_probe), which a zero gate makes undefined (gates start at 1 and "
                                      "the reference's optimizer moves them by ~1e-5 per step)")
                w = w.detach().float() * gv.view(-1, 1, 1, 1)
            if cout_pad is not None and cout_pad > w.shape[0]:
                wp = torch.zeros((cout_pad,) + tuple(w.shape[1:]), dtype=w.dtype, device=w.device)
                wp[:w.shape[0]] = w.detach()
                w = wp
            return ops.pack_conv_weight(w, self.dtype, KD_PACK_FWD, cin_pad)
        return self._packed(conv.weight, ("fwd", self.dtype, cin_pad, cin_rot, cout_pad, id(gate) if gate is not None else None), make,
                            extra=gate.weight._version if gate is not None else None)

    def _w_dgrad(self, conv, cout_pad=None, cin_rot=0, gate=None):
        def make():
            w = conv.weight.detach()
            if gate is not None:
                w = w.float() * gate.weight.detach().float().view(-1, 1, 1, 1)
            if cin_rot:
                w = torch.cat([w[:, cin_rot:], w[:, :cin_rot]], 1).contiguous()
            if cout_pad is not None and cout_pad != w.shape[0]:
                wp = torch.zeros((cout_pad,) + tuple(w.shape[1:]), dtype=w.dtype, device=w.device)
                wp[:w.shape[0]] = w
                w = wp
            return ops.pack_conv_weight(w, self.dtype, KD_PACK_DGRAD)
        return self._packed(conv.weight, ("dgrad", self.dtype, cout_pad, cin_rot, id(gate) if gate is not None else None), make,
                            extra=gate.weight._version if gate is not None else None)

    def _w_cat(self, conv_a, conv_b, mode):
        def make():
            wa = (self._w_fwd if mode == "fwd" else self._w_dgrad)(conv_a)
            wb = (self._w_fwd if mode == "fwd" else self._w_dgrad)(conv_b)
            return torch.cat([wa, wb], dim=3).contiguous()
        return self._packed(conv_a.weight, ("cat", mode, self.dtype, id(conv_b.weight)), make, extra=conv_b.weight._version)

# ... 82 lines not shown
    def _act_fold(self, bn, gate):
        scale, shift = self._bn_fold(bn)
        if gate is None:
            return scale, shift
        key = ("gated", id(_bn_of(bn)), id(gate))
        ver = (scale._kd_serial, gate.weight._version, gate.weight.device)
        ent = self._bn.get(key)
        if ent is None or ent[0] != ver or ent[2] is not gate:
            g = gate.weight.detach().float()
            if not bool((g > 0).all()):
                raise EngineError("a gate behind a ReLU must stay positive to be folded into the BN+ReLU epilogue "
                                  "(gates start at 1 and the reference's optimizer moves them by ~1e-5 per step)")
            ent = (ver, ((scale * g).contiguous(), (shift * g).contiguous()), gate)
            ent[1][0]._kd_serial = next(_FOLD_SERIAL)
            self._bn[key] = ent
        return ent[1]

    def _new(self, N, H, W, C, dtype=None, zero=False):
        f = torch.zeros if zero else torch.empty
        return f((N, H, W, C), dtype=dtype or self.dtype, device=self.device)

    def check_hint_names(self, names):
        ok = {f"aspp.features.{i}.0" for i in range(len(self.net.aspp.features))}
        ok.add("aspp")
        for name, blk in self._flat_blocks():
            ok.add(name)
            ok.add(f"{name}.convs")
            ok.update(f"{name}.convs.{n}" for n, _ in blk.convs.named_children() if n.startswith("conv"))
        bad = [n for n in names if n not in ok]
        if bad:
            raise EngineError(f"hint layers the fused student graph cannot capture: {bad} (supported: conv sites, "
                              "`<block>.convs`, `<block>`, `aspp.features.N.0`, `aspp`)")

    def _flat_blocks(self):
        net = self.net
        flat = [(f"mod{i}.{bn}", blk) for i in range(2, 8) for bn, blk in getattr(net, f"mod{i}").named_children()]
        for name, blk in flat:
            if not isinstance(blk, IdentityResidualBlock):
                raise EngineError(f"{name}: expected an IdentityResidualBlock")
        return flat

    def shareable_prefix(self, teacher_engine):
        if self.is_gscnn or teacher_engine.is_gscnn or self.dtype != teacher_engine.dtype:
            return 0
        sn, tn = self.net, teacher_engine.net
        key = tuple((id(p), p._version, p.requires_grad) for p in sn.parameters()) + tuple(self.hint_names) + tuple(self.probe_names)
        ent = getattr(self, "_prefix_cache", None)
        if ent is not None and ent[0] == key and ent[1] is tn:
            return ent[2]

        def same(a, b):
            sa, sb = a.state_dict(), b.state_dict()
            if list(sa) != list(sb) or any(p.requires_grad for p in a.parameters()):
                return False
            return all(type(x) is type(y) for x, y in zip(a.modules(), b.modules())) and \
                all(sa[k].shape == sb[k].shape and sa[k].device == sb[k].device and torch.equal(sa[k], sb[k]) for k in sa)
        k = 0
        if same(sn.mod1, tn.mod1):
            sflat, tflat = self._flat_blocks(), teacher_engine._flat_blocks()
            named = set(self.hint_names) | set(self.probe_names)
            for (name, sb), (_, tb) in zip(sflat, tflat):
                if any(h == name or h.startswith(name + ".") for h in named) or not same(sb, tb):
                    break
                k += 1
            while k > 0 and k < len(sflat) and not same(sflat[k][1].bn1, tflat[k][1].bn1):
                k -= 1
        self._prefix_cache = (key, tn, k)
        return k

    def forward(self, x, collect_hints=True, export_at=None, prefix=None):
        net = self.net
        if x.dim() != 4 or x.shape[1] != 3:
            raise EngineError(f"expected an (N,3,H,W) batch, got {tuple(x.shape)}")
        if x.shape[2] % 8 or x.shape[3] % 8:
            raise EngineError("input height/width must be multiples of 8 (two stride-2 pools and one stride-2 conv)")
        self.device = x.device
        N, _, H, W = x.shape
        want = set(self.hint_names) if collect_hints else set()
        self._probes = set(self.probe_names) if self._probe_active else set()
        seen = []
        hints = []
        tape = {"blocks": [], "aspp": None, "hint_slots": [], "pools": {}}

        def note_hint(name, tensor, slot):
            seen.append(name)
            hints.append(tensor)
            tape["hint_slots"].append(slot)

        xin = x.detach()
        if xin.dtype != torch.float32 or not xin.is_contiguous():
            xin = xin.float().contiguous()
        flat = self._flat_blocks()
        start = 0
        if prefix is None:
            stem = net.mod1.conv1
            stem_w = stem.weight.detach()
            stem_w = stem_w if stem_w.is_contiguous() else stem_w.contiguous()
            rg = stem.weight.requires_grad
            sc1, sh1 = self._bn_fold(flat[0][1].bn1)
            if _STEM_POOL and self.dtype == torch.bfloat16 and not rg and not self.is_gscnn:
                s = None
                _, a = ops.stem_conv_pool(xin, stem_w, sc1, sh1, want_raw=False)
            else:
                s = ops.stem_conv(xin, stem_w, self.dtype)
                _, a = ops.maxpool3x3s2(s, sc1, sh1, want_raw=False)
            tape["stem"] = dict(x=xin, s=s, rg=rg)
            x_raw = None
            m2 = None
        else:
            start, a, x_raw, m2, s, rg = prefix["k"], prefix["a"], prefix["x_raw"], prefix["m2"], None, False
            tape["blocks"] = [None] * start
            if prefix["pool3"] is not None:
                tape["pools"]["pool3"] = dict(prefix["pool3"], rg=False)
        self.exported = None
        for bi, (name, blk) in enumerate(flat):
            if bi < start:
                continue
            if export_at is not None and bi == export_at:
                self.exported = dict(k=bi, a=a, x_raw=x_raw, m2=m2, pool3=tape["pools"].get("pool3"))
            last_of_mod2 = name.startswith("mod2.") and (bi + 1 == len(flat) or not flat[bi + 1][0].startswith("mod2."))
            is_last = bi + 1 == len(flat)
            nxt = None if (is_last or last_of_mod2) else flat[bi + 1][1]
            need_raw = is_last or last_of_mod2 or (nxt is not None and not hasattr(nxt, "proj_conv"))
            mod_end = is_last or flat[bi + 1][0].split(".")[0] != name.split(".")[0]
            if self.is_gscnn and mod_end and name.split(".")[0] in ("mod3", "mod4"):
                need_raw = True
            gap = [] if (is_last and _FUSE_GAP and self.dtype == torch.bfloat16) else None
            x_raw, a, rg, rec = self._block_fwd(name, blk, x_raw, a, rg, nxt.bn1 if nxt is not None else None, need_raw,
                                                want, note_hint, bi, out_sums=gap)
            if gap:
                tape["x7_sums"] = gap[0]
            tape["blocks"].append(rec)
            if self.is_gscnn and mod_end:
                tape.setdefault("mods", {})[name.split(".")[0]] = x_raw
                tape.setdefault("mod_end", {})[name.split(".")[0]] = (bi, rg)
            if last_of_mod2:
                m2 = x_raw
                sc, sh = self._bn_fold(flat[bi + 1][1].bn1)
                _, a = ops.maxpool3x3s2(m2, sc, sh, want_raw=False)
                tape["pools"]["pool3"] = dict(x=m2, after=bi, rg=rg)
                x_raw = None
        x7, rg7 = x_raw, rg

        if self.is_gscnn:
            train_shape = self._differentiable and (self.logits_need_grad or "aspp" in want)
            tape["shape"] = {} if train_shape else None
            tape["acts"] = self._shape_stream(xin, s, tape["mods"]["mod3"], tape["mods"]["mod4"], x7, rec=tape["shape"])
        cat, rg_cat = self._aspp_fwd(net.aspp, x7, rg7, want, note_hint, tape)
        logits = self._decoder_fwd(cat, rg_cat, m2, tape["pools"]["pool3"]["rg"], (H, W), tape)

        missing = want - set(seen)
        if missing:
            raise EngineError(f"hint layers not found in the student graph: {sorted(missing)}")
        self._tape = tape
        self.last_hint_names = list(seen)
        return logits, hints

    def _aspp_fwd(self, aspp, x7, rg7, want, note_hint, tape):
        N, h8, w8, _ = x7.shape
        red = aspp.img_conv[0].out_channels
        nb = len(aspp.features)
        lead = self._aspp_lead(aspp)
        cat = self._new(N, h8, w8, red * (nb + lead))
        sc, sh = self._bn_fold(aspp.img_conv[1])
        ops.aspp_image_pool(x7, aspp.img_conv[0].weight.detach(), sc, sh, cat[..., 0:red], sums=tape.get("x7_sums"))
        if lead == 2:
            sc, sh = self._bn_fold(aspp.edge_conv[1])
            ops.edge_aspp(tape["acts"], aspp.edge_conv[0].weight.detach().float().reshape(-1).contiguous(), sc, sh, cat[..., red:2 * red])
        arec = {"x7": x7, "rg7": rg7, "branches": [], "cat": cat, "red": red, "mod": aspp, "lead": lead}
        rg_cat = rg7 or _is_trainable(aspp.img_conv)
        mids, fan = {}, {}
        if _DW_SUM:
            for i, br in enumerate(aspp.features):
                site = _Site(f"aspp.features.{i}.0", br[0])
                if site.cheap:
                    fan.setdefault((site.k, site.pad, site.dil), []).append((i, site))
            for (k, pad, dil), members in fan.items():
                if len(members) > 1:
                    outs = ops.dwconv_fanout(x7, [self._w_dw(st.mod.separable_conv, False) for _, st in members], k, pad, dil)
                    mids.update({i: o for (i, _), o in zip(members, outs)})
        for i, br in enumerate(aspp.features):
            site = _Site(f"aspp.features.{i}.0", br[0])
            act_gate = _gate_split(br[2])[1] if len(br) > 2 else None
            sc, sh = self._act_fold(br[1], act_gate)
            hinted = site.name in want
            probed = site.name in self._probes or site.gate is not None
            raw = self._new(N, h8, w8, red) if (hinted or probed) else None
            out = cat[..., red * (i + lead):red * (i + lead + 1)]
            mid = None
            if site.cheap:
                mid = mids.get(i)
                if mid is None:
                    mid = ops.dwconv(x7, self._w_dw(site.mod.separable_conv, False), site.k, site.pad, site.dil)
                ops.conv2d(mid, self._w_fwd(site.mod.pointwise_conv), out_raw=raw, out_act=out, act_scale=sc, act_shift=sh,
                           act_relu=True)
            elif site.masked:
                mid = self._masked_fwd(site, x7, out_raw=raw, out_act=out, act_scale=sc, act_shift=sh, act_relu=True)
            else:
                ops.conv2d(x7, self._w_fwd(site.mod, gate=site.gate), 1, site.pad, site.dil, out_raw=raw, out_act=out, act_scale=sc,
                           act_shift=sh, act_relu=True)
            if hinted:
                note_hint(site.name, raw, ("aspp", i))
            arec["branches"].append({"site": site, "mid": mid, "bn": br[1], "probe_raw": raw if probed else None, "act_gate": act_gate})
            rg_cat = rg_cat or site.trainable or _is_trainable(br[1]) or probed or act_gate is not None
        if "aspp" in want:
            note_hint("aspp", cat, ("aspp_out",))
        tape["aspp"] = arec
        return cat, rg_cat

    def _w_bn_folded(self, conv, bn, cpad):
        def make():
            scale, shift = self._bn_fold(bn)
            w = conv.weight.detach().float() * scale.view(-1, 1, 1, 1)
            wp = torch.zeros((cpad, cpad) + tuple(w.shape[2:]), dtype=torch.float32, device=w.device)
            wp[:w.shape[0], :w.shape[1]] = w
            sp = torch.zeros(cpad, dtype=torch.float32, device=w.device)
            sp[:shift.numel()] = shift
            return (ops.pack_conv_weight(wp, self.dtype, KD_PACK_FWD), sp)
        bnm = _bn_of(bn)
        return self._packed(conv.weight, ("bnfold", self.dtype, cpad, id(bn)), make,
                            extra=(bnm.weight._version, bnm.bias._version, bnm.running_mean._version, bnm.running_var._version))

    def _basic_block(self, blk, x, cpad=64, rec=None):
        if rec is None:
            for p in blk.parameters():
                if p.requires_grad:
                    raise EngineError("trainable shape-stream parameters need the differentiable shape stream: set "
                                      "DepthwiseStudent.logits_need_grad = True (trainers that back-propagate a logit loss do)")
        N, H, W, cx = x.shape
        planes = blk.conv1.out_channels
        if rec is None and _SMALL_CONV and self.dtype == torch.bfloat16 and planes in (16, 32, 64) and blk.conv1.in_channels == planes:
            w1, s1 = self._w_bn_folded(blk.conv1, blk.bn1, planes)
            w2, s2 = self._w_bn_folded(blk.conv2, blk.bn2, planes)
            xin = x if cx == planes else x[..., :planes]
            t = self._new(N, H, W, planes)
            ops.conv3x3_small(xin, w1, s1, relu=True, out=t)
            y = self._zero_padded(("basic_block", id(blk)), N, H, W, cpad) if planes < cpad else self._new(N, H, W, planes)
            ops.conv3x3_small(t, w2, s2, res=xin, relu=True, out=y[..., :planes])
            return y
        w1, s1 = self._w_bn_folded(blk.conv1, blk.bn1, cpad)
        w2, s2 = self._w_bn_folded(blk.conv2, blk.bn2, cpad)
        t = self._new(N, H, W, cpad)
        ops.conv2d(x, w1, 1, 1, 1, out_act=t, act_shift=s1, act_relu=True)
        y = self._new(N, H, W, cpad)
        ops.conv2d(t, w2, 1, 1, 1, res_pre=x, out_act=y, act_shift=s2, act_relu=True)
        if rec is not None:
            rec.append((blk, x, t, y))
        return y

    def _zero_padded(self, tag, N, H, W, C):
        key = (tag, N, H, W, C, self.dtype)
        buf = self._persist.get(key)
        if buf is None or buf.device != self.device:
            buf = torch.zeros((N, H, W, C), dtype=self.dtype, device=self.device)
            self._persist[key] = buf
        return buf

    def _gate_params(self, gate):
        ent = self._gate_prm.get(id(gate))
        ver = tuple(t._version for t in list(gate.parameters()) + list(gate.buffers()))
        if ent is not None and ent[0] is gate and ent[2] == ver:
            return ent[1]
        bn0, c1, _, c2, bn4, _ = gate._gate_conv
        hdim = c1.in_channels
        s0, t0 = self._bn_fold(bn0)
        s4, t4 = self._bn_fold(bn4)
        w1 = c1.weight.detach().float().view(hdim, hdim)
        prm = torch.cat([(w1 * s0.view(1, -1)).reshape(-1), c1.bias.detach().float() + w1 @ t0,
                         c2.weight.detach().float().view(hdim) * s4, c2.bias.detach().float() * s4 + t4,
                         gate.weight.detach().float().reshape(-1)]).contiguous()
        self._gate_prm[id(gate)] = (gate, prm, ver)
        return prm

    def _w_bn_folded_dgrad(self, conv, bn, cpad):
        def make():
            scale, _ = self._bn_fold(bn)
            w = conv.weight.detach().float() * scale.view(-1, 1, 1, 1)
            wp = torch.zeros((cpad, cpad) + tuple(w.shape[2:]), dtype=torch.float32, device=w.device)
            wp[:w.shape[0], :w.shape[1]] = w
            return ops.pack_conv_weight(wp, self.dtype, KD_PACK_DGRAD)
        bnm = _bn_of(bn)
        return self._packed(conv.weight, ("bnfold_dgrad", self.dtype, cpad, id(bn)), make,
                            extra=(bnm.weight._version, bnm.bias._version, bnm.running_var._version))

    def _shape_stream(self, x_nchw, m1, m3, m4, m7, rec=None):
# ... 198 lines not shown
        ops.conv2d(dec0, self._w_fwd(f[0], cin_pad=cpad, cin_rot=nf), 1, 1, 1, out_act=d1, act_scale=sc, act_shift=sh, act_relu=True,
                   algo_cin=cdec)
        sc, sh = self._bn_fold(f[4])
        ncls = f[6].out_channels
        d3 = self._new(N, h2, w2, ncls, dtype=torch.float32)
        fuse_cls = (not self.logits_need_grad and not any(q.requires_grad for q in list(f[3].parameters()) + list(f[6].parameters())) and
                    f[6].bias is None and ncls <= 32 and f[6].kernel_size == (1, 1) and ops.conv_cls_ok(d1, f[3].out_channels, 3, 1))
        d2 = None
        if fuse_cls:
            try:
                ops.conv2d(d1, self._w_fwd(f[3]), 1, 1, 1, act_scale=sc, act_shift=sh, act_relu=True, cls_w=self._w_fwd(f[6], cout_pad=32), cls_out=d3)
            except ops.ClsUnsupported:
                fuse_cls = False
        if not fuse_cls:
            d2 = self._new(N, h2, w2, f[3].out_channels)
            ops.conv2d(d1, self._w_fwd(f[3]), 1, 1, 1, out_act=d2, act_scale=sc, act_shift=sh, act_relu=True)
            ops.conv2d(d2, self._w_fwd(f[6]), out_raw=d3)
        if self.lazy_logits and self._lazy_call and not self.logits_need_grad:
            logits = LazyLogits(d3, size, align_corners=not self.is_gscnn)
        else:
            logits = ops.upsample_bilinear_ac(d3, size, out_dtype=torch.float32, align_corners=not self.is_gscnn)
        tape["dec"] = dict(cat=cat, rg_cat=rg_cat, m2=m2, rg_m2=rg_m2, dec0=dec0, d1=d1, d2=d2, cdec=cdec, nf=nf, nu=nu, size=size,
                           small=(h8, w8))
        return logits

    def _block_fwd(self, name, blk, x_raw, a1, rg_in, next_bn, need_raw, want, note_hint, bi, out_sums=None):
        convs = [(n, m) for n, m in blk.convs.named_children() if n.startswith("conv")]
        bns = {n: m for n, m in blk.convs.named_children() if n.startswith("bn")}
        for n, m in blk.convs.named_children():
            if isinstance(m, (nn.Dropout, nn.Dropout2d)) and m.training:
                raise EngineError(f"{name}: training-mode dropout is not supported (student runs in eval mode, SURVEY F3)")
        sites = [_Site(f"{name}.convs.{n}", m) for n, m in convs]
        N = a1.shape[0]
        rec = {"name": name, "blk": blk, "sites": sites, "a_in": [], "mid": [], "rg_a": [], "hint_raw": [None] * len(sites),
               "x_raw": x_raw, "rg_in": rg_in, "proj": hasattr(blk, "proj_conv")}
        rg_a1 = rg_in or _is_trainable(blk.bn1)
        dual = (rec["proj"] and len(sites) == 3 and sites[-1].k == 1 and sites[-1].stride == 1 and
                self._dual_ok(a1.shape, sites[-1].cin, a1.shape[3], sites[-1].cout, 0, sites[-1].mod, blk.proj_conv, sites[-1]))
        rec["dual"] = dual
        if dual:
            shortcut = None
            rg_short = rg_a1 or blk.proj_conv.weight.requires_grad
        elif rec["proj"]:
            pc = blk.proj_conv
            ho = ops.conv_out_size(a1.shape[1], 1, pc.stride[0], 0, 1)
            wo = ops.conv_out_size(a1.shape[2], 1, pc.stride[0], 0, 1)
            shortcut = self._new(N, ho, wo, pc.out_channels)
            ops.conv2d(a1, self._w_fwd(pc), pc.stride[0], 0, 1, out_raw=shortcut)
            rg_short = rg_a1 or pc.weight.requires_grad
        else:
            if x_raw is None:
                raise EngineError(f"{name}: identity shortcut needs the raw block input")
            shortcut = x_raw
            rg_short = rg_in
        a, rg = a1, rg_a1
        x_out = a_next = None
        for i, site in enumerate(sites):
            last = i + 1 == len(sites)
            rec["a_in"].append(a)
            rec["rg_a"].append(rg)
            ho = ops.conv_out_size(a.shape[1], site.k, site.stride, site.pad, site.dil)
            wo = ops.conv_out_size(a.shape[2], site.k, site.stride, site.pad, site.dil)
            hinted = site.name in want or (last and (f"{name}.convs" in want or name in want))
            probed = site.name in self._probes or site.gate is not None
            kw = {}
            if last:
                want_raw = need_raw or hinted or probed
                raw = self._new(N, ho, wo, site.cout) if want_raw else None
                if not dual:
                    kw["res_pre"] = shortcut
                if next_bn is not None:
                    sc, sh = self._bn_fold(next_bn)
                    a_next = self._new(N, ho, wo, site.cout)
                    kw.update(out_act=a_next, act_scale=sc, act_shift=sh, act_relu=True)
                kw["out_raw"] = raw
                x_out = raw
                if out_sums is not None and not site.cheap and not site.masked and site.gate is None and (ho * wo) % 128 == 0:
                    kw["out_sums"] = out_sums
            else:
                sc, sh = self._act_fold(bns[f"bn{i + 2}"], _act_gate(bns[f"bn{i + 2}"]))
                act = self._new(N, ho, wo, site.cout)
                raw = self._new(N, ho, wo, site.cout) if (hinted or probed) else None
                kw.update(out_raw=raw, out_act=act, act_scale=sc, act_shift=sh, act_relu=True)
            if site.cheap:
                mid = ops.dwconv(a, self._w_dw(site.mod.separable_conv, False), site.k, site.pad, site.dil)
                ops.conv2d(mid, self._w_fwd(site.mod.pointwise_conv), **kw)
            elif site.masked:
                mid = self._masked_fwd(site, a, **kw)
            elif last and dual:
                mid = None
                try:
                    ops.conv2d(a, self._w_cat(site.mod, blk.proj_conv, "fwd"), x2=a1, **kw)
                except ops.DualUnsupported:
                    rec["dual"] = False
                    if kw.get("out_sums") is not None:
                        del kw["out_sums"][:]
                    shortcut = self._new(N, ho, wo, site.cout)
                    ops.conv2d(a1, self._w_fwd(blk.proj_conv), 1, 0, 1, out_raw=shortcut)
                    ops.conv2d(a, self._w_fwd(site.mod, gate=site.gate), site.stride, site.pad, site.dil, res_pre=shortcut, **kw)
            else:
                mid = None
                ops.conv2d(a, self._w_fwd(site.mod, gate=site.gate), site.stride, site.pad, site.dil, **kw)
            rec["mid"].append(mid)
            rg = rg or site.trainable or probed
            if probed:
                rec.setdefault("probe", {})[i] = (raw, shortcut if last else None)
            if hinted:
                if last:
                    for nm in (site.name, f"{name}.convs", name):
                        if nm in want:
                            note_hint(nm, raw, ("block", bi, "out"))
                else:
                    rec["hint_raw"][i] = raw
                    note_hint(site.name, raw, ("block", bi, i))
            if not last:
                a = act
                rg = rg or _is_trainable(bns[f"bn{i + 2}"])
        rec["rg_out"] = rg or rg_short
        return x_out, a_next, rec["rg_out"], rec

    def grad_production_order(self):
        net, order = self.net, []

        def add_p(*ps):
            for p in ps:
                if p is not None and p.requires_grad and all(p is not q for q in order):
                    order.append(p)

        def add_conv(mod):
            mod, gate = _gate_split(mod)
            if gate is not None:
                add_p(gate.weight)
            if isinstance(mod, DepthwiseSeparableBlock):
                add_p(mod.pointwise_conv.weight, mod.separable_conv.weight)
            elif _is_masked(mod):
                add_p(mod[2].weight)
            else:
                add_p(mod.weight)

        def add_bn(seq, gate=None):
            bn = _bn_of(seq)
            gate = gate if gate is not None else _act_gate(seq)
            if gate is not None:
                add_p(gate.weight)
            add_p(bn.weight, bn.bias)
        f = self._final()
        add_conv(f[6]); add_bn(f[4]); add_conv(f[3]); add_bn(f[1]); add_conv(f[0])
        add_conv(net.bot_fine); add_conv(net.bot_aspp)
        add_bn(net.aspp.img_conv[1]); add_conv(net.aspp.img_conv[0])
        if self.is_gscnn:
            add_bn(net.aspp.edge_conv[1]); add_conv(net.aspp.edge_conv[0])
            add_p(net.fuse.weight, net.cw.weight)
            for gate, dsn, d, res in ((net.gate3, net.dsn7, net.d3, net.res3), (net.gate2, net.dsn4, net.d2, net.res2),
                                      (net.gate1, net.dsn3, net.d1, net.res1)):
                add_p(*gate.parameters()); add_p(*dsn.parameters()); add_p(*d.parameters()); add_p(*res.parameters())
        for br in net.aspp.features:
            add_bn(br[1], _gate_split(br[2])[1] if len(br) > 2 else None); add_conv(br[0])
        for _, blk in reversed(self._flat_blocks()):
            items = list(blk.convs.named_children())
            for n, m in reversed(items):
                if n.startswith("conv"):
                    add_conv(m)
                elif n.startswith("bn"):
                    add_bn(m)
            if hasattr(blk, "proj_conv"):
                add_conv(blk.proj_conv)
            add_bn(blk.bn1)
        add_conv(net.mod1.conv1)
        return order

    def backward(self, hint_grads, g_logits=None):
        tape = self._tape
        if tape is None:
            raise EngineError("backward() called without a recorded forward()")
        if len(hint_grads) != len(tape["hint_slots"]):
            raise EngineError("hint gradient list does not match the recorded hints")
        grads = {}
        self.probe_grads = {}
        g_block_out = {}
        g_site_hint = {}
        g_aspp = {}
        g_cat_hint = None

        def acc(d, k, g):
            d[k] = g if k not in d else d[k] + g
        for g, slot in zip(hint_grads, tape["hint_slots"]):
            if g is None:
                continue
            g = self._as_nhwc(g)
            if slot[0] == "aspp":
                acc(g_aspp, slot[1], g)
            elif slot[0] == "aspp_out":
                g_cat_hint = g if g_cat_hint is None else g_cat_hint + g
            elif slot[2] == "out":
                acc(g_block_out, slot[1], g)
            else:
                acc(g_site_hint, (slot[1], slot[2]), g)
# ... 419 lines not shown
            tmp = torch.empty((kpad, f[6].weight.shape[1], 1, 1), dtype=torch.float32, device=g_d3.device)
            ops.conv2d_wgrad(dec["d2"], g_d3, tmp, 1, 0, 1)
            gw = self._grad_like(f[6].weight)
            gw.copy_(tmp[:ncls])
            grads[f[6].weight] = gw
            self._grad_done(f[6].weight)
        else:
            self._conv_wgrad(f[6], dec["d2"], g_d3[..., :ncls], grads)
        if not rg_d2:
            return None, None
        sc, _ = self._bn_fold(f[4])
        g_c2 = self._new(N, h2, w2, f[3].out_channels)
        fused = [] if _FUSE_BN_SUMS and self._wants_bn_sums(f[4]) else None
        ops.conv2d(g_d3, self._w_dgrad(f[6], cout_pad=kpad), out_raw=g_c2, mask=dec["d2"], mask_scale=sc, bn_sums=fused)
        self._bn_param_grads(f[4], g_c2, dec["d2"], grads, sums=fused[0] if fused else None)
        self._conv_wgrad(f[3], dec["d1"], g_c2, grads)
        if not rg_d1:
            return None, None
        sc, _ = self._bn_fold(f[1])
        fused = [] if _FUSE_BN_SUMS and self._wants_bn_sums(f[1]) else None
        g_c1 = self._dense_dgrad(_Site("final.3", f[3]), g_c2, mask=dec["d1"], mask_scale=sc, bn_sums=fused)
        self._bn_param_grads(f[1], g_c1, dec["d1"], grads, sums=fused[0] if fused else None)
        self._conv_wgrad(f[0], dec["dec0"], g_c1, grads, cin=cdec, cin_rot=nf)
        if not rg_dec0:
            return None, None
        nu = dec["nu"]
        kf = ((nf + 63) // 64) * 64
        g_dec0 = self._new(N, h2, w2, nu + kf)
        if nu + kf > cdec:
            g_dec0[..., cdec:].zero_()
        wd = self._w_dgrad(f[0], cin_rot=nf)
        if _SPLIT_DEC_DGRAD and self.dtype == torch.bfloat16 and nu % 256 == 0 and cdec > nu:
            ops.conv2d(g_c1, wd[:nu], 1, 1, 1, out_raw=g_dec0[..., 0:nu])
            ops.conv2d(g_c1, wd[nu:cdec], 1, 1, 1, out_raw=g_dec0[..., nu:cdec])
        else:
            ops.conv2d(g_c1, wd, 1, 1, 1, out_raw=g_dec0[..., 0:cdec])
        g_m2 = None
        self._conv_wgrad(net.bot_fine, dec["m2"], g_dec0[..., nu:cdec], grads)
        if dec["rg_m2"]:
            g_m2 = self._new(N, h2, w2, net.bot_fine.in_channels)
            ops.conv2d(g_dec0[..., nu:nu + kf], self._w_dgrad(net.bot_fine, cout_pad=kf), out_raw=g_m2)
        g_cat = None
        if dec["rg_cat"] or _is_trainable(net.bot_aspp):
            g_up = ops.upsample_bilinear_ac_bwd(g_dec0[..., 0:nu], dec["small"])
            self._conv_wgrad(net.bot_aspp, dec["cat"], g_up, grads)
            if dec["rg_cat"]:
                cat = dec["cat"]
                g_cat = self._new(N, cat.shape[1], cat.shape[2], cat.shape[3])
                fused = [] if _FUSE_BN_SUMS else None
                ops.conv2d(g_up, self._w_dgrad(net.bot_aspp), out_raw=g_cat, mask=cat, mask_scale=self._cat_scale(net.aspp), bn_sums=fused)
                self._tape["aspp"]["cat_sums"] = fused[0] if fused else None
        return g_cat, g_m2


class _StudentFunction(torch.autograd.Function):

    @staticmethod
    def forward(ctx, engine, x, *params):
        ctx.set_materialize_grads(False)
        logits, hints = engine.forward(x, prefix=engine._next_prefix)
        ctx.engine, ctx.params = engine, params
        lazy = isinstance(logits, LazyLogits)
        outs = (logits if lazy else logits.permute(0, 3, 1, 2),) + tuple(h.permute(0, 3, 1, 2) for h in hints)
        ctx.nh = len(hints)
        if lazy:
            ctx.mark_non_differentiable(outs[0])
            outs = outs + (x.new_zeros(()),)
        ctx.lazy = outs[0] if lazy else None
        return outs

    @staticmethod
    def backward(ctx, g_logits, *g_rest):
        g_hints = g_rest[:ctx.nh]
        if ctx.lazy is not None:
            g_logits, ctx.lazy.pending_grad = ctx.lazy.pending_grad, None
            ctx.lazy = None
        grads = ctx.engine.backward(list(g_hints), g_logits)
        return (None, None) + tuple(grads.get(p) for p in ctx.params)


def run_student(engine, x, prefix=None):
    engine._next_prefix = prefix
    engine._lazy_call = True
    try:
        return _run_student(engine, x, prefix)
    finally:
        engine._next_prefix = None
        engine._lazy_call = False


def _run_student(engine, x, prefix):
    params = tuple(p for p in engine.net.parameters() if p.requires_grad)
    if torch.is_grad_enabled() and (params or engine.probe_names):
        if not params:
            x = x.detach().requires_grad_(True)
        engine._probe_active = bool(engine.probe_names)
        engine._differentiable = True
        try:
            outs = _StudentFunction.apply(engine, x, *params)
            if isinstance(outs[0], LazyLogits):
                outs[0].anchor = outs[-1]
                outs = outs[:-1]
        finally:
            engine._probe_active = False
            engine._differentiable = False
    else:
        logits, hints = engine.forward(x, prefix=prefix)
        engine._tape = None
        outs = (logits if isinstance(logits, LazyLogits) else logits.permute(0, 3, 1, 2),) + tuple(h.permute(0, 3, 1, 2) for h in hints)
    return outs[0], list(outs[1:])
```

knowledge-distillation-by-replacing-cheap-conv_amd/losses/__init__.py:

```python
import torch
from torch import nn

from .. import ops
from .._lib import KdccError
from ..lazy import LazyLogits, deferred


class _FusedLoss(torch.autograd.Function):

    @staticmethod
    def forward(ctx, kind, inputs, targets, arg, weight):
        want = inputs.requires_grad
        s, t = inputs.detach(), targets.detach()
        if kind == "kld":
            loss, grad = ops.kldiv(s, t, arg, want_grad=want)
        elif kind == "mse":
            loss, grad = ops.hint_mse(s, t, arg, want_grad=want)
        elif kind == "jsd":
            loss, grad = ops.jsdiv(s, t, arg, want_grad=want)
        elif kind == "ekl":
            loss, grad = ops.ensemble_kldiv(s, t, want_grad=want)
        elif kind == "topk":
            loss, grad, _ = ops.topk_hint_mse(s, t, arg, want_grad=want)
        else:
            loss, grad = ops.weighted_hint_mse(s, t, weight, want_grad=want)
        ctx.grad = grad
        return loss

    @staticmethod
    def backward(ctx, g):
        grad = ctx.grad
        ctx.grad = None
        if grad is None:
            return None, None, None, None, None
        if g.numel() == 1 and grad.dtype in (torch.float32, torch.bfloat16) and grad.data_ptr() % 16 == 0:
            return None, ops.scale_by_device_scalar_(grad, g), None, None, None
        return None, grad * g.to(grad.dtype), None, None, None


def _same_device_dtype(inputs, targets):
    if targets.dtype != inputs.dtype and not (targets.dtype in (torch.float32, torch.bfloat16)):
        targets = targets.to(inputs.dtype)
    return targets


class KLDivergenceLoss(nn.Module):

    def __init__(self, temperature=1):
        super().__init__()
        self.temperature = temperature

    def forward(self, inputs, targets):
        if isinstance(inputs, LazyLogits) and isinstance(targets, LazyLogits) and inputs.pending and targets.pending and \
                inputs.size_hw == targets.size_hw and inputs.align_corners == targets.align_corners:
            try:
                return deferred(ops.kldiv_up(inputs.low, targets.low, inputs.size_hw, float(self.temperature), inputs.align_corners),
                                "kld", inputs, targets, float(self.temperature))
            except KdccError:
                pass
        return _FusedLoss.apply("kld", inputs, _same_device_dtype(inputs, targets), float(self.temperature), None)


class MSELoss(nn.Module):

    def __init__(self, reduction='mean', num_classes=19):
        super().__init__()
        if reduction not in ('mean', 'sum'):
            raise NotImplementedError("reduction='none' returns a tensor no KD trainer consumes: 'mean' or 'sum'")
        self.reduction = reduction
        self.num_classes = num_classes

    def forward(self, inputs, targets):
        scale = float(self.num_classes) * (inputs.numel() if self.reduction == 'sum' else 1)
        return _FusedLoss.apply("mse", inputs, _same_device_dtype(inputs, targets), scale, None)


class WeightedHintMSELoss(nn.Module):

    def __init__(self, reduction='mean', num_classes=19):
        super().__init__()
        self.reduction = reduction
        self.num_classes = num_classes

    def forward(self, inputs, targets, filter_weight):
        return _FusedLoss.apply("whmse", inputs, _same_device_dtype(inputs, targets), None, filter_weight)


class _CEFunction(torch.autograd.Function):
    @staticmethod
    def forward(ctx, inputs, targets, ignore_index, weight=None, size_average=True):
        ctx.save_for_backward(inputs.detach(), targets)
        ctx.ignore_index, ctx.weight, ctx.size_average = ignore_index, weight, size_average
        return ops.ce2d(inputs.detach(), targets, ignore_index, weight, size_average)

    @staticmethod
    def backward(ctx, g):
        x, tgt = ctx.saved_tensors
        grad = ops.ce2d_grad(x, tgt, ctx.ignore_index, 1.0, ctx.weight, ctx.size_average)
        return grad * g.to(grad.dtype), None, None, None, None


class CrossEntropyLoss2d(nn.Module):

    def __init__(self, weight=None, size_average=True, ignore_index=255):
        super().__init__()
        self.register_buffer('weight', None if weight is None else torch.as_tensor(weight, dtype=torch.float32))
        self.size_average = bool(size_average)
        self.ignore_index = ignore_index

    def forward(self, inputs, targets):
        if self.weight is not None and self.weight.device != inputs.device:
            self.weight = self.weight.to(inputs.device)
        if self.weight is not None or not self.size_average:
            if inputs.requires_grad and torch.is_grad_enabled():
                return _CEFunction.apply(inputs, targets, self.ignore_index, self.weight, self.size_average)
            return ops.ce2d(inputs, targets, self.ignore_index, self.weight, self.size_average)
        if isinstance(inputs, LazyLogits) and inputs.pending:
            try:
                return deferred(ops.ce2d_up(inputs.low, targets, inputs.size_hw, self.ignore_index, inputs.align_corners),
                                "ce", inputs, targets, self.ignore_index)
            except KdccError:
                pass
        if inputs.requires_grad and torch.is_grad_enabled():
            return _CEFunction.apply(inputs, targets, self.ignore_index)
        return ops.ce2d(inputs, targets, self.ignore_index)


class JSDivergenceLoss(nn.Module):

    def __init__(self, temperature=1):
        super().__init__()
        self.temperature = temperature

    def forward(self, inputs, targets):
        if isinstance(inputs, LazyLogits) and isinstance(targets, LazyLogits) and inputs.pending and targets.pending and \
                inputs.size_hw == targets.size_hw and inputs.align_corners == targets.align_corners:
            try:
                return deferred(ops.jsdiv_up(inputs.low, targets.low, inputs.size_hw, float(self.temperature), inputs.align_corners),
                                "jsd", inputs, targets, float(self.temperature))
            except KdccError:
                pass
        return _FusedLoss.apply("jsd", inputs, _same_device_dtype(inputs, targets), float(self.temperature), None)


class EnsembleKLDivergenceLoss(nn.Module):

    def __init__(self):
        super().__init__()

    def forward(self, inputs, targets):
        return _FusedLoss.apply("ekl", inputs, _same_device_dtype(inputs, targets), None, None)


class TopkHintMSELoss(nn.Module):

    def __init__(self, reduction='mean', num_classes=19, topk=0.5):
        super().__init__()
        self.reduction = reduction
        self.num_classes = num_classes
        self.topk = topk

    def forward(self, inputs, targets):
        if targets.dim() != 4 or inputs.shape != targets.shape:
            raise ValueError(f"TopkHintMSELoss: (N,C,H,W) inputs and targets of one shape only, got {tuple(inputs.shape)} and "
                             f"{tuple(targets.shape)}")
        num_channels = targets.shape[1]
        k = int(self.topk * num_channels)
        if k <= 0:
            raise ValueError(f"TopkHintMSELoss: topk={self.topk} keeps no channel of {num_channels}")
        return _FusedLoss.apply("topk", inputs, _same_device_dtype(inputs, targets), min(k, num_channels), None)


class _FocalFunction(torch.autograd.Function):

    @staticmethod
    def forward(ctx, inputs, targets, gamma, alpha, ignore_index, reduction):
        x = inputs.detach()
        loss, stats, amap, cemap = ops.focal(x, targets, gamma, alpha, ignore_index, reduction)
        ctx.save_for_backward(x, targets)
        ctx.args, ctx.stats, ctx.maps = (gamma, alpha, ignore_index, reduction), stats, (amap, cemap)
        if reduction == 'none':
            N, sp = x.shape[0], tuple(x.shape[2:])
            return amap.view(N, 1, *sp) * cemap.view(N, *sp)
        return loss

    @staticmethod
    def backward(ctx, g):
        x, tgt = ctx.saved_tensors
        gamma, alpha, ignore_index, reduction = ctx.args
        grad = ops.focal_grad(x, tgt, gamma, alpha, ignore_index, reduction, g, ctx.stats, *ctx.maps)
        ctx.stats = ctx.maps = None
        return grad, None, None, None, None, None


class FocalLoss(nn.CrossEntropyLoss):

    def __init__(self, gamma, alpha=None, ignore_index=-100, reduction='none'):
        if alpha is not None and not torch.is_tensor(alpha):
            alpha = torch.as_tensor(alpha, dtype=torch.float32)
        super().__init__(weight=alpha, ignore_index=ignore_index, reduction='none')
        if reduction not in ('none', 'mean', 'sum'):
            raise ValueError(f"FocalLoss: reduction must be 'none', 'mean' or 'sum', got {reduction!r}")
        self.reduction = reduction
        self.gamma = gamma

    def forward(self, input_, target):
        if self.weight is not None and self.weight.device != input_.device:
            self.weight = self.weight.to(input_.device)
        gamma = float(self.gamma)
        if isinstance(input_, LazyLogits) and input_.pending and self.reduction in ('mean', 'sum'):
            try:
                loss, stats = ops.focal_up(input_.low, target, input_.size_hw, gamma, self.weight, self.ignore_index, self.reduction,
                                           input_.align_corners)
                return deferred(loss, "focal", input_, target, (gamma, self.weight, self.ignore_index, self.reduction, stats))
            except KdccError:
                pass
        return _FocalFunction.apply(input_, target, gamma, self.weight, self.ignore_index, self.reduction)
```

knowledge-distillation-by-replacing-cheap-conv_amd/models/students/depthwise_student.py:

```python
import copy
import gc
from functools import reduce

import torch
from torch import nn

from ..deeplabv3 import DeepWV3Plus
from ..gscnn import GSCNN
from ..hrnet_ocr import HighResolutionNet
from ..cifar_models.wrn import WideResNet
from ... import nn_hip
from ...lazy import LazyLogits
from .transform_blocks import DepthwiseSeparableBlock

BLOCKS_LEVEL_SPLIT_CHAR = '.'


class DepthwiseStudent(nn.Module):
    def __init__(self, teacher_model, config=None, dtype=None):
        super().__init__()
        self.config = config
        self.teacher = copy.deepcopy(teacher_model)
        if self.teacher.training:
            self.teacher.eval()
# ... 189 lines not shown
            k = 0
            if self.share_frozen_prefix and self.engine_plan and not self.hip_teacher_side_stream:
                k = self._student_engine().shareable_prefix(eng)
            eng._lazy_call = True
            try:
                with torch.no_grad():
                    logits, hints = eng.forward(x, export_at=k if k > 0 else None)
            finally:
                eng._lazy_call = False
            self._prefix = eng.exported if k > 0 else None
            eng.exported = None
            eng._tape = None
            if self.save_hidden:
                self.teacher_hidden_outputs = [h.permute(0, 3, 1, 2) for h in hints]
            return logits if hasattr(logits, "materialize") else logits.permute(0, 3, 1, 2)
        self._prepare_teacher(x.device)
        xt = x.to(dtype=self.dtype, memory_format=torch.channels_last)
        with torch.no_grad():
            return self.teacher(xt)

    def prefetch_teacher(self, x):
        self._prefetched = None
        if not self.engine_plan or not x.is_cuda or self.share_frozen_prefix or isinstance(self.teacher, GSCNN):
            return False
        if self._side_stream is None or self._side_stream.device != x.device:
            self._side_stream = torch.cuda.Stream(device=x.device)
        main = torch.cuda.current_stream()
        ready = torch.cuda.Event()
        ready.record(main)
        self._side_stream.wait_event(ready)
        x.record_stream(self._side_stream)
        keep = self.teacher_hidden_outputs
        self.teacher_hidden_outputs = []
        import os
        tcus, scus = os.environ.get("KDCC_TEACHER_CUS"), os.environ.get("KDCC_STUDENT_CUS")
        if tcus is not None:
            from ... import _lib
            _lib.check(_lib.lib().kd_conv_set_persist_cus(int(tcus)), "kd_conv_set_persist_cus")
        with torch.cuda.stream(self._side_stream):
            pred = self._teacher_forward(x)
        if tcus is not None:
            _lib.check(_lib.lib().kd_conv_set_persist_cus(int(scus or 0)), "kd_conv_set_persist_cus")
        hints = self.teacher_hidden_outputs
        self.teacher_hidden_outputs = keep
        self._prefix = None
        done = torch.cuda.Event()
        done.record(self._side_stream)
        self._prefetched = ((x.data_ptr(), tuple(x.shape), x._version), pred, hints, done)
        return True

    def forward(self, x):
        self.student_hidden_outputs = []
        self.teacher_hidden_outputs = []
        pre, self._prefetched = getattr(self, "_prefetched", None), None
        if not self.engine_plan:
            if self.fused:
                self._check_module_graph_input(x)
            x = self._module_graph_batch(x)
            with torch.no_grad():
                teacher_pred = self.teacher(x)
            return self.student(x), teacher_pred
        if not x.is_cuda:
            raise RuntimeError("the fused DeepWV3Plus student runs on the GPU only (no CPU fallback)")
        from ...engine import run_student
        engine = self._student_engine()
        if engine.is_gscnn:
            engine.edge_prior = engine.compute_edge_prior(x)
            if self._teacher_engine is not None:
                self._teacher_engine.edge_prior = engine.edge_prior
            self._shared_prior = engine.edge_prior
        hip_teacher = self.teacher_backend == "hip" and isinstance(self.teacher, (DeepWV3Plus, GSCNN))
        if pre is not None and pre[0] == (x.data_ptr(), tuple(x.shape), x._version):
            _, teacher_pred, thints, done = pre
            main = torch.cuda.current_stream()
            main.wait_event(done)
            for t in [teacher_pred] + list(thints):
                if isinstance(t, LazyLogits) and t.pending:
                    t.low.record_stream(main)
                else:
                    t.record_stream(main)
            self.teacher_hidden_outputs = thints
            self.prefetch_hits = getattr(self, "prefetch_hits", 0) + 1
            self._prefix = None
            student_pred, hints = run_student(engine, x)
        elif self.overlap_teacher and (not hip_teacher or self.hip_teacher_side_stream):
            if self._side_stream is None or self._side_stream.device != x.device:
                self._side_stream = torch.cuda.Stream(device=x.device)
            main = torch.cuda.current_stream()
            self._side_stream.wait_stream(main)
            with torch.cuda.stream(self._side_stream):
                teacher_pred = self._teacher_forward(x)
            student_pred, hints = run_student(engine, x)
            main.wait_stream(self._side_stream)
            for t in [teacher_pred] + list(self.teacher_hidden_outputs):
                if isinstance(t, LazyLogits) and t.pending:
                    t.low.record_stream(main)
                else:
                    t.record_stream(main)
        else:
            self._prefix = None
            teacher_pred = self._teacher_forward(x)
            student_pred, hints = run_student(engine, x, prefix=self._prefix)
            self._prefix = None
        if self.save_hidden:
            self.student_hidden_outputs = hints
            self.student_hint_names = list(engine.last_hint_names)
        engine.edge_prior = None
        self._shared_prior = None
        if self._teacher_engine is not None:
            self._teacher_engine.edge_prior = None
        return student_pred, teacher_pred

    def _check_module_graph_input(self, x):
        if not x.is_cuda:
            raise RuntimeError(f"the {type(self.student).__name__} student runs on the GPU only (no CPU fallback)")
        if x.dtype != torch.float32:
            raise TypeError(f"the {type(self.student).__name__} student is fp32 only (bf16 is not implemented for this network)")

    def inference(self, x):
        self.student_hidden_outputs = []
        self.teacher_hidden_outputs = []
        if not self.engine_plan:
            if self.fused:
                self._check_module_graph_input(x)
            return self.student(self._module_graph_batch(x))
        from ...engine import run_student
        engine = self._student_engine()
        engine.hint_names = []
        with torch.no_grad():
            pred, _ = run_student(engine, x)
        return pred

    @staticmethod
    def sliding_windows(h, w, tile, overlap=1 / 3):
        from math import ceil
        stride = ceil(tile * (1 - overlap))
        n_x = max(int(ceil((w - tile) / stride) + 1), 1)
        n_y = max(int(ceil((h - tile) / stride) + 1), 1)
        boxes = []
        for ix in range(n_x):
            for iy in range(n_y):
                x2, y2 = min(ix * stride + tile, w), min(iy * stride + tile, h)
                boxes.append((max(x2 - tile, 0), max(y2 - tile, 0), x2, y2))
        return boxes

    def inference_test(self, data, args, max_windows_per_pass=8):
        import torch.nn.functional as F
        self.student_hidden_outputs = []
        self.teacher_hidden_outputs = []
        scales = [float(sc) for sc in args.get('scales', [1.0])]
        crop = int(args['crop_size'])
        mode = str(args.get('window_count', 'reference'))
        if mode not in ('reference', 'pixel'):
            raise ValueError("test.args.window_count must be 'reference' or 'pixel'")
        N, _, H, W = data.shape
        outs = []
        with torch.no_grad():
            for n in range(N):
                img = data[n:n + 1]
                per_scale = []
                for scale in scales:
                    if abs(scale - 1.0) < 1e-9:
                        img_s = img
                    else:
                        img_s = F.interpolate(img.float(), size=(int(H * scale), int(W * scale)), mode='bilinear', align_corners=False,
                                              antialias=scale < 1.0).to(img.dtype)
                    hs, ws = img_s.shape[2:]
                    boxes = self.sliding_windows(hs, ws, int(scale * crop))
                    acc = None
                    for flipped in (False, True):
                        src = torch.flip(img_s, dims=[3]) if flipped else img_s
                        full = cnt = None
                        for i in range(0, len(boxes), max_windows_per_pass):
                            part = boxes[i:i + max_windows_per_pass]
                            wins = torch.cat([src[:, :, y1:y2, x1:x2] for (x1, y1, x2, y2) in part], 0).contiguous()
                            logits = self.inference(wins).float()
                            if full is None:
                                C = logits.shape[1]
                                full = torch.zeros((C, hs, ws), dtype=torch.float32, device=data.device)
                                cnt = torch.zeros((C, hs, ws) if mode == 'reference' else (1, hs, ws), dtype=torch.float32,
                                                  device=data.device)
                            for j, (x1, y1, x2, y2) in enumerate(part):
                                full[:, y1:y2, x1:x2] += logits[j][:, :y2 - y1, :x2 - x1]
                                if mode == 'reference':
                                    cnt[y1:y2, x1:x2] += 1
# ... 42 lines not shown
```

knowledge-distillation-by-replacing-cheap-conv_amd/ops.py:

```python
import ctypes as C
import os

import torch

from . import _lib
from ._lib import (KD_BF16, KD_F32, KD_PACK_DGRAD, KD_PACK_FWD, ConvDesc, ConvEpilogue, DConvDesc, DwDesc, DwEpilogue, MultiTargets, View3,
                   check)


PROFILER = None


def _prof_start():
    if PROFILER is None:
        return None
    e0 = torch.cuda.Event(enable_timing=True)
    e0.record()
    return e0


def _prof_stop(e0, family, work, label, kernel=None):
    if e0 is None or PROFILER is None:
        return
    e1 = torch.cuda.Event(enable_timing=True)
# ... 4 lines not shown
def _nbytes(*ts):
    return sum(t.numel() * t.element_size() for t in ts if t is not None)


def _ws(nbytes, device, floor=16):
    return torch.empty(max(int(nbytes), floor), dtype=torch.uint8, device=device)


def _scratch(shape, dtype, device):
    return torch.empty(shape, dtype=dtype, device=device)


def dt_of(t):
    if t.dtype == torch.bfloat16:
        return KD_BF16
    if t.dtype == torch.float32:
        return KD_F32
    raise TypeError(f"unsupported dtype {t.dtype} (float32 / bfloat16 only)")


def stream_ptr():
    return C.c_void_p(torch.cuda.current_stream().cuda_stream)


def _ptr(t):
    if t is None:
        return None
    if type(t) is not torch.Tensor and hasattr(t, "materialize"):
        t = t.materialize()
    return C.c_void_p(t.data_ptr())


def _need_cuda(*ts):
    for t in ts:
        if t is not None and not t.is_cuda:
            raise _lib.KdccError("kdcc kernels need device tensors (there is no CPU fallback)")


def nhwc_ld(t):
    if t.dim() != 4 or t.stride(3) != 1:
        raise ValueError(f"expected an (N,H,W,C) tensor with dense channels, got shape {tuple(t.shape)} stride {t.stride()}")
    N, H, W, _ = t.shape
    ld = t.stride(2)
    if (W > 1 and ld < t.shape[3]) or (H > 1 and t.stride(1) != W * ld) or (N > 1 and t.stride(0) != H * W * ld):
        raise ValueError(f"not a pixel-strided NHWC view: shape {tuple(t.shape)} stride {t.stride()}")
    return ld


def new_nhwc(N, H, W, Cc, dtype, device, zero=False):
    f = torch.zeros if zero else torch.empty
    return f((N, H, W, Cc), dtype=dtype, device=device)


def as_nchw(t):
    return t.permute(0, 3, 1, 2)


def conv_out_size(h, k, stride, pad, dil):
    return (h + 2 * pad - dil * (k - 1) - 1) // stride + 1


def pack_conv_weight(w, dtype, mode=KD_PACK_FWD, cin_pad=None):
    _need_cuda(w)
    w = w.detach().contiguous().float()
    Cout, Cin, kh, kw = w.shape
    cin_pad = Cin if cin_pad is None else cin_pad
    if mode == KD_PACK_FWD:
        out = torch.empty((Cout, kh, kw, cin_pad), dtype=dtype, device=w.device)
    else:
        out = torch.empty((Cin, kh, kw, Cout), dtype=dtype, device=w.device)
    check(_lib.lib().kd_pack_conv_weight(_ptr(w), _ptr(out), dt_of(out), mode, Cout, Cin, kh, kw, cin_pad, stream_ptr()),
          "kd_pack_conv_weight")
    return out


class DualUnsupported(_lib.KdccError):
    """conv2d(..., x2=...) on a shape the K-concatenated 1x1 kernel does not take: run the two convs instead."""


class ClsUnsupported(_lib.KdccError):
    """conv2d(..., cls_w=, cls_out=) on a problem whose kernel does not carry the classifier epilogue: store the activation and run the 1x1."""


def conv2d(x, w_packed, stride=1, pad=0, dil=1, *, res_pre=None, mask=None, mask_scale=None, res_post=None,
           out_raw=None, out_act=None, act_scale=None, act_shift=None, act_relu=False, algo_cin=None, algo_cout=None, bn_sums=None,
           x2=None, out_sums=None, cls_w=None, cls_out=None):
    _need_cuda(x, w_packed)
    N, H, W, Cin = x.shape
    Cout, kh, kw, Cin_w = w_packed.shape
    Cin2 = 0
    if x2 is not None:
        _need_cuda(x2)
        if tuple(x2.shape[:3]) != (N, H, W) or x2.dtype != x.dtype or (kh, kw, stride, pad) != (1, 1, 1, 0):
            raise ValueError("conv2d: x2 needs a 1x1 / stride-1 conv and a source of the same pixels and dtype")
        Cin2 = x2.shape[3]
    if Cin_w != Cin + Cin2:
        raise ValueError(f"conv2d: input has {Cin + Cin2} channels, packed weight expects {Cin_w}")
    if w_packed.dtype != x.dtype or not w_packed.is_contiguous():
        raise ValueError("conv2d: packed weight must be contiguous and of the activation dtype")
    Ho, Wo = conv_out_size(H, kh, stride, pad, dil), conv_out_size(W, kw, stride, pad, dil)
    d = ConvDesc(dt_of(x), N, H, W, Cin, Ho, Wo, Cout, kh, kw, stride, pad, dil, nhwc_ld(x))
    ep = ConvEpilogue()

    def chk(t, name, f32_ok=False):
        if t is None:
            return 0
        if tuple(t.shape) != (N, Ho, Wo, Cout):
            raise ValueError(f"conv2d: {name} has shape {tuple(t.shape)}, expected {(N, Ho, Wo, Cout)}")
        if t.dtype != x.dtype and not (f32_ok and t.dtype == torch.float32):
            raise ValueError(f"conv2d: {name} dtype {t.dtype} != {x.dtype}")
        _need_cuda(t)
        return nhwc_ld(t)

    def chk_vec(v, name):
        if v is not None and (v.dtype != torch.float32 or v.numel() != Cout or not v.is_contiguous()):
            raise ValueError(f"conv2d: {name} must be a contiguous fp32 vector of {Cout}")
        _need_cuda(v)

    ep.res_pre, ep.ld_res_pre = _ptr(res_pre), chk(res_pre, "res_pre")
    ep.mask, ep.ld_mask = _ptr(mask), chk(mask, "mask")
    chk_vec(mask_scale, "mask_scale"); ep.mask_scale = _ptr(mask_scale)
    ep.res_post, ep.ld_res_post = _ptr(res_post), chk(res_post, "res_post")
    ep.out_raw, ep.ld_raw = _ptr(out_raw), chk(out_raw, "out_raw", f32_ok=True)
    ep.raw_f32 = int(out_raw is not None and out_raw.dtype == torch.float32 and x.dtype != torch.float32)
    ep.out_act, ep.ld_act = _ptr(out_act), chk(out_act, "out_act")
    chk_vec(act_scale, "act_scale"); chk_vec(act_shift, "act_shift")
    ep.act_scale, ep.act_shift, ep.act_relu = _ptr(act_scale), _ptr(act_shift), int(act_relu)
    ep.bn_sums = None
    if (cls_w is None) != (cls_out is None):
        raise ValueError("conv2d: cls_w and cls_out come together")
    if cls_w is not None:
        _need_cuda(cls_w, cls_out)
        if tuple(cls_w.shape) != (32, 1, 1, Cout) or cls_w.dtype != x.dtype or not cls_w.is_contiguous():
            raise ValueError(f"conv2d: cls_w must be a contiguous (32,1,1,{Cout}) packed weight of the activation dtype")
        if cls_out.dtype != torch.float32 or tuple(cls_out.shape[:3]) != (N, Ho, Wo) or cls_out.shape[3] > 32 or cls_out.stride(3) != 1:
            raise ValueError("conv2d: cls_out must be (N,Ho,Wo,ncls <= 32) fp32")
        ep.cls_w, ep.cls_out, ep.ld_cls, ep.ncls = _ptr(cls_w), _ptr(cls_out), nhwc_ld(cls_out), cls_out.shape[3]
        if x2 is not None or not _lib.lib().kd_conv2d_cls_supported(C.byref(d), C.byref(ep)):
            raise ClsUnsupported(f"conv2d: no classifier epilogue for {kh}x{kw} {H}x{W} {Cin}->{Cout}")
    sums_rows = 0
    if bn_sums is not None and mask is not None:
        sums_rows = int(_lib.lib().kd_conv2d_bn_sums_rows(C.byref(d), C.byref(ep)))
        if sums_rows > 0:
            part = _scratch((sums_rows, 2, Cout), torch.float32, x.device)
            ep.bn_sums = _ptr(part)
    out_rows = 0
    if out_sums is not None and mask is None and res_pre is None and res_post is None and out_act is None and out_raw is not None:
        out_rows = int(_lib.lib().kd_conv2d_bn_sums_rows(C.byref(d), C.byref(ep)))
        if out_rows > 0:
            opart = _scratch((out_rows, 2, Cout), torch.float32, x.device)
            ep.bn_sums = _ptr(opart)
    prof = PROFILER
    if prof is not None:
        e0 = torch.cuda.Event(enable_timing=True)
        e0.record()
    if x2 is not None:
        ld2 = nhwc_ld(x2)
        if not _lib.lib().kd_conv1x1_dual_supported(C.byref(d), Cin2, ld2, C.byref(ep)):
            raise DualUnsupported(f"conv2d: no K-concatenated kernel for {H}x{W} {Cin}+{Cin2}->{Cout}")
        check(_lib.lib().kd_conv1x1_dual_fwd(C.byref(d), _ptr(x), _ptr(x2), Cin2, ld2, _ptr(w_packed), C.byref(ep), stream_ptr()), "kd_conv1x1_dual_fwd")
    else:
        check(_lib.lib().kd_conv2d_fwd(C.byref(d), _ptr(x), _ptr(w_packed), C.byref(ep), stream_ptr()), "kd_conv2d_fwd")
    if out_rows > 0:
        out_sums.append(opart)
    if prof is not None:
        e1 = torch.cuda.Event(enable_timing=True)
        e1.record()
        epi = "".join(c for c, t in (("p", res_pre), ("m", mask), ("q", res_post), ("r", out_raw), ("a", out_act), ("c", cls_out)) if t is not None)
        prof.append(("conv_igemm", 2.0 * N * Ho * Wo * (algo_cout or Cout) * kh * kw * (algo_cin or (Cin + Cin2)), e0, e1,
                     f"{kh}x{kw} s{stride} d{dil} {H}x{W} {Cin}{'+%d' % Cin2 if Cin2 else ''}->{Cout} [{epi}{'s' if sums_rows or out_rows else ''}]", _lib.last_kernel()))
    if sums_rows > 0:
        s12 = torch.empty((2, Cout), dtype=torch.float32, device=x.device)
        need = _lib.lib().kd_bn_sums_finish_workspace(sums_rows, Cout)
        ws = _ws(need, x.device) if need else None
        check(_lib.lib().kd_bn_sums_finish(_ptr(part), sums_rows, Cout, _ptr(s12[0]), _ptr(s12[1]), _ptr(ws), need, stream_ptr()),
              "kd_bn_sums_finish")
        bn_sums.append((s12[0], s12[1]))
    return out_raw, out_act


def conv_cls_ok(x, Cout, k=3, dil=1):
    if not x.is_cuda or x.dtype != torch.bfloat16 or os.environ.get("KDCC_FUSE_CLS", "1") == "0":
        return False
    N, H, W, Cin = x.shape
    d = ConvDesc(dt_of(x), N, H, W, Cin, H, W, Cout, k, k, 1, dil * (k // 2), dil, nhwc_ld(x))
    ep = ConvEpilogue()
    ep.cls_w, ep.cls_out, ep.ld_cls, ep.ncls = C.c_void_p(256), C.c_void_p(256), 32, 19
    return bool(_lib.lib().kd_conv2d_cls_supported(C.byref(d), C.byref(ep)))


def conv1x1_dual_ok(x, x2, Cout, operands=0):
    if x2 is None or not x.is_cuda or x.dtype != torch.bfloat16 or x2.dtype != x.dtype or tuple(x2.shape[:3]) != tuple(x.shape[:3]):
        return False
    N, H, W, Cin = x.shape
    d = ConvDesc(dt_of(x), N, H, W, Cin, H, W, Cout, 1, 1, 1, 0, 1, nhwc_ld(x))
    ep = ConvEpilogue()
    some = C.c_void_p(x.data_ptr())
    if operands >= 1:
        ep.mask, ep.ld_mask = some, Cout
    if operands >= 2:
        ep.res_post, ep.ld_res_post = some, Cout
    if operands >= 3:
        ep.res_pre, ep.ld_res_pre = some, Cout
    ep.out_raw, ep.ld_raw = some, Cout
    return bool(_lib.lib().kd_conv1x1_dual_supported(C.byref(d), x2.shape[3], nhwc_ld(x2), C.byref(ep)))


def conv1x1_dual_ok_dims(N, H, W, Cin, Cin2, Cout, dtype, operands=0):
    if dtype != torch.bfloat16:
        return False
    d = ConvDesc(KD_BF16, N, H, W, Cin, H, W, Cout, 1, 1, 1, 0, 1, Cin)
    ep = ConvEpilogue()
    if operands >= 1:
        ep.mask, ep.ld_mask = C.c_void_p(256), Cout
    if operands >= 2:
        ep.res_post, ep.ld_res_post = C.c_void_p(256), Cout
    if operands >= 3:
        ep.res_pre, ep.ld_res_pre = C.c_void_p(256), Cout
    ep.out_raw, ep.ld_raw = C.c_void_p(256), Cout
    return bool(_lib.lib().kd_conv1x1_dual_supported(C.byref(d), Cin2, Cin2, C.byref(ep)))


def pw_wgrad(a, dy, dw, accumulate=False, workspace=None):
    _need_cuda(a, dy, dw)
    N, H, W, Cin = a.shape
    Cout = dy.shape[3]
    if tuple(dy.shape[:3]) != (N, H, W) or a.dtype != dy.dtype:
        raise ValueError("pw_wgrad: a / dy mismatch")
    if dw.dtype != torch.float32 or dw.numel() != Cout * Cin or not dw.is_contiguous():
        raise ValueError("pw_wgrad: dw must be contiguous fp32 (Cout,Cin,1,1)")
    M = N * H * W
    need = _lib.lib().kd_pw_wgrad_workspace(M, Cin, Cout)
    if workspace is None or workspace.numel() * workspace.element_size() < need:
        workspace = _ws(need, a.device, 0)
    e0 = _prof_start()
    check(_lib.lib().kd_pw_wgrad(dt_of(a), M, Cin, Cout, _ptr(a), nhwc_ld(a), _ptr(dy), nhwc_ld(dy), _ptr(dw),
                                 int(accumulate), _ptr(workspace), workspace.numel() * workspace.element_size(),
                                 stream_ptr()), "kd_pw_wgrad")
    _prof_stop(e0, "pw_wgrad", 2.0 * M * Cin * Cout, f"pw wgrad {H}x{W} {Cin}->{Cout}")
    return dw


def conv2d_wgrad(x, dy, dw, stride=1, pad=0, dil=1, accumulate=False, workspace=None):
    _need_cuda(x, dy, dw)
    N, H, W, Cin = x.shape
    Cout, Cin_w, kh, kw = dw.shape
    Ho, Wo = conv_out_size(H, kh, stride, pad, dil), conv_out_size(W, kw, stride, pad, dil)
# ... 1819 lines not shown
```

Measured before the change: 45.95 images/sec.

## Fuse hint MSE loss and gradient into the student conv epilogue

Adds a hint epilogue to the persistent ping-pong conv kernel. It reads the teacher hint, writes the scaled MSE gradient, and accumulates per-tile squared-difference sums, which a small two-stage reduction kernel turns into the loss. The Python engine passes the teacher hint targets into the student run, and the MSE loss module uses the fused result when the target and scale match. This removes a separate pass over the student and teacher hint tensors for loss and gradient. In exchange it adds extra epilogue stores and register pressure to the conv, plus bookkeeping that ties the loss object to the engine state.

```diff
diff --git a/include/kdcc.h b/include/kdcc.h
--- a/include/kdcc.h
+++ b/include/kdcc.h
@@ -38,8 +38,16 @@
     void *out_act;        int32_t ld_act;      const float *act_scale; const float *act_shift; int32_t act_relu;
     float *bn_sums;
     const void *cls_w;    float *cls_out;      int32_t ld_cls;      int32_t ncls;
+    const void *hint_t;   int32_t ld_hint_t;
+    void *hint_grad;      int32_t ld_hint_grad;
+    float hint_gscale;
+    float *hint_sums;
 } kd_conv_epilogue;
 int32_t kd_conv2d_cls_supported(const kd_conv_desc *d, const kd_conv_epilogue *ep);
+int32_t kd_conv2d_hint_supported(const kd_conv_desc *d, const kd_conv_epilogue *ep);
+enum { KD_HINT_SUMS_FINISH_WORKSPACE = 8192 };
+int kd_hint_sums_finish(const float *part, int32_t rows, int32_t C, double factor, float *loss, void *workspace,
+                        size_t workspace_bytes, kd_stream_t stream);
 
 int kd_conv2d_fwd(const kd_conv_desc *d, const void *x, const void *w_packed,
                   const kd_conv_epilogue *ep, kd_stream_t stream);
diff --git a/knowledge-distillation-by-replacing-cheap-conv_amd/_lib.py b/knowledge-distillation-by-replacing-cheap-conv_amd/_lib.py
--- a/knowledge-distillation-by-replacing-cheap-conv_amd/_lib.py
+++ b/knowledge-distillation-by-replacing-cheap-conv_amd/_lib.py
@@ -14,6 +14,7 @@
 KD_F32, KD_BF16 = 0, 1
 KD_PACK_FWD, KD_PACK_DGRAD = 0, 1
 KD_ERR_UNSUPPORTED = -2
+KD_HINT_SUMS_FINISH_WORKSPACE = 8192
 KD_CIFAR_NCHW, KD_CIFAR_NHWC = 0, 1
 KD_SEG_NCHW, KD_SEG_NHWC = 0, 1
 KD_OPT_SGD, KD_OPT_ADAM, KD_OPT_ADAMW_REF = 0, 1, 2
@@ -34,7 +35,9 @@
                 ("out_raw", c_vp), ("ld_raw", c_int), ("raw_f32", c_int),
                 ("out_act", c_vp), ("ld_act", c_int), ("act_scale", c_vp), ("act_shift", c_vp), ("act_relu", c_int),
                 ("bn_sums", c_vp),
-                ("cls_w", c_vp), ("cls_out", c_vp), ("ld_cls", c_int), ("ncls", c_int)]
+                ("cls_w", c_vp), ("cls_out", c_vp), ("ld_cls", c_int), ("ncls", c_int),
+                ("hint_t", c_vp), ("ld_hint_t", c_int), ("hint_grad", c_vp), ("ld_hint_grad", c_int), ("hint_gscale", C.c_float),
+                ("hint_sums", c_vp)]
 
 
 class DwDesc(C.Structure):
@@ -86,6 +89,8 @@
     "kd_conv_set_persist_cus": (c_int, [c_int]),
     "kd_conv2d_bn_sums_rows": (c_int, [_P(ConvDesc), _P(ConvEpilogue)]),
     "kd_conv2d_cls_supported": (c_int, [_P(ConvDesc), _P(ConvEpilogue)]),
+    "kd_conv2d_hint_supported": (c_int, [_P(ConvDesc), _P(ConvEpilogue)]),
+    "kd_hint_sums_finish": (c_int, [c_vp, c_int, c_int, C.c_double, c_vp, c_vp, c_sz, c_vp]),
     "kd_bn_sums_finish_workspace": (c_sz, [c_int, c_int]),
     "kd_bn_sums_finish": (c_int, [c_vp, c_int, c_int, c_vp, c_vp, c_vp, c_sz, c_vp]),
     "kd_pack_conv_weight": (c_int, [c_vp, c_vp, c_int, c_int, c_int, c_int, c_int, c_int, c_int, c_vp]),
diff --git a/knowledge-distillation-by-replacing-cheap-conv_amd/csrc/conv_common.h b/knowledge-distillation-by-replacing-cheap-conv_amd/csrc/conv_common.h
--- a/knowledge-distillation-by-replacing-cheap-conv_amd/csrc/conv_common.h
+++ b/knowledge-distillation-by-replacing-cheap-conv_amd/csrc/conv_common.h
@@ -27,6 +27,7 @@
     else if (nst == 48) asm volatile("s_waitcnt vmcnt(48) lgkmcnt(0)" ::: "memory");
     else if (nst == 20) asm volatile("s_waitcnt vmcnt(20) lgkmcnt(0)" ::: "memory");
     else if (nst == 36) asm volatile("s_waitcnt vmcnt(36) lgkmcnt(0)" ::: "memory");
+    else if (nst == 52) asm volatile("s_waitcnt vmcnt(52) lgkmcnt(0)" ::: "memory");
     else asm volatile("s_waitcnt vmcnt(0) lgkmcnt(0)" ::: "memory");
     __builtin_amdgcn_s_barrier();
 }
@@ -38,6 +39,7 @@
     else if (nst == 48) asm volatile("s_waitcnt vmcnt(48)" ::: "memory");
     else if (nst == 20) asm volatile("s_waitcnt vmcnt(20)" ::: "memory");
     else if (nst == 36) asm volatile("s_waitcnt vmcnt(36)" ::: "memory");
+    else if (nst == 52) asm volatile("s_waitcnt vmcnt(52)" ::: "memory");
     else asm volatile("s_waitcnt vmcnt(0)" ::: "memory");
 }
 
@@ -77,8 +79,10 @@
     constexpr int NOPS = NOPS_ & 3;
     constexpr bool SUMS = (NOPS_ & 4) != 0;
     constexpr bool OSUMS = NOPS_ == 8;
-    static_assert((MI == 8 || (MI == 4 && !(NOPS_ & 12))) && NOPS_ >= 0 && (NOPS_ <= 7 || NOPS_ == 8) && NOPS_ != 4,
+    constexpr bool HINT = (NOPS_ & 32) != 0;
+    static_assert((MI == 8 || (MI == 4 && !(NOPS_ & 44))) && NOPS_ >= 0 && (NOPS_ <= 7 || NOPS_ == 8 || NOPS_ == 32 || NOPS_ == 33) && NOPS_ != 4,
                   "128-row wave sub-tiles (64 rows at a time: conv_row_duo_kernel, no sums); eval-BN sums need the mask operand, output sums no operand");
+    static_assert(!HINT || OUTS == 0, "the hint block: ping-pong kernels only");
     const kd_conv_epilogue &e = p.ep;
     asm volatile("" : "+v"(lane));
     const int frow = lane & 15, fq = lane >> 4;
@@ -98,12 +102,12 @@
     const uint32_t vo_raw = (uint32_t)(lrow * e.ld_raw + c0) * 2u, vo_act = (uint32_t)(lrow * e.ld_act + c0) * 2u;
     const short relu_w = e.act_relu ? (short)0 : (short)-32768;
     const i16x2_v relu_i16 = {relu_w, relu_w};
-    const T *s0 = (const T *)(has_p ? e.res_pre : has_m ? e.mask : e.res_post);
-    const int ld0 = has_p ? e.ld_res_pre : has_m ? e.ld_mask : e.ld_res_post;
-    const T *s1 = (const T *)(has_p && has_m ? e.mask : e.res_post);
-    const int ld1 = has_p && has_m ? e.ld_mask : e.ld_res_post;
-    constexpr int nops = NOPS;
-    const bool m_in1 = has_p && has_m, q_in1 = has_q && nops == 2;
+    const T *s0 = (const T *)(HINT && NOPS == 0 ? e.hint_t : has_p ? e.res_pre : has_m ? e.mask : e.res_post);
+    const int ld0 = HINT && NOPS == 0 ? e.ld_hint_t : has_p ? e.ld_res_pre : has_m ? e.ld_mask : e.ld_res_post;
+    const T *s1 = (const T *)(HINT ? e.hint_t : has_p && has_m ? e.mask : e.res_post);
+    const int ld1 = HINT ? e.ld_hint_t : has_p && has_m ? e.ld_mask : e.ld_res_post;
+    constexpr int nops = NOPS + (HINT ? 1 : 0);
+    const bool m_in1 = has_p && has_m, q_in1 = has_q && NOPS == 2;
     uint4 ra[8], rb[8], rc[NOPS == 3 ? 8 : 1];
     auto rowof = [&](int pass) { return (size_t)(mw + pass * 8 + lrow); };
     auto load64 = [&](const T *src, int ld, int hb, uint4 (&r)[8]) __attribute__((always_inline)) {
@@ -169,8 +173,8 @@
                 float v[8], t[8];
                 ld8((const bf16_t *)&rawv, v);
                 const uint4 o0 = (hb == 1 && nops == 1) ? rb[ps] : ra[ps], o1 = rb[ps];
-                if (NOPS >= 1) asm volatile("" ::"v"(o0.x), "v"(o0.y), "v"(o0.z), "v"(o0.w));
-                if (NOPS >= 2) asm volatile("" ::"v"(o1.x), "v"(o1.y), "v"(o1.z), "v"(o1.w));
+                if (nops >= 1) asm volatile("" ::"v"(o0.x), "v"(o0.y), "v"(o0.z), "v"(o0.w));
+                if (nops >= 2) asm volatile("" ::"v"(o1.x), "v"(o1.y), "v"(o1.z), "v"(o1.w));
                 if constexpr (NOPS == 3) asm volatile("" ::"v"(rc[ps].x), "v"(rc[ps].y), "v"(rc[ps].z), "v"(rc[ps].w));
                 if (has_p) {
                     ld8((const T *)&o0, t);
@@ -215,7 +219,18 @@
                     }
                     continue;
                 }
-                if (OUTS ? (OUTS & 1) != 0 : e.out_raw != nullptr) {
+                if constexpr (HINT) {
+                    uint4 hv = rawv;
+                    if (NOPS != 0) hv = make_uint4(pack_bf16x2(v[0], v[1]), pack_bf16x2(v[2], v[3]), pack_bf16x2(v[4], v[5]), pack_bf16x2(v[6], v[7]));
+                    *(uint4 *)((T *)e.out_raw + m * e.ld_raw + c0) = hv;
+                    const uint4 oh = NOPS == 0 ? o0 : o1;
+                    float hs[8], d[8];
+                    ld8((const T *)&hv, hs);
+                    ld8((const T *)&oh, t);
+#pragma unroll
+                    for (int q = 0; q < 8; ++q) { d[q] = hs[q] - t[q]; bs1[q] = fmaf(d[q], d[q], bs1[q]); d[q] *= e.hint_gscale; }
+                    st8((T *)e.hint_grad + m * e.ld_hint_grad + c0, d);
+                } else if (OUTS ? (OUTS & 1) != 0 : e.out_raw != nullptr) {
                     if (nops == 0) *(uint4 *)((T *)e.out_raw + m * e.ld_raw + c0) = rawv;
                     else if (OUTS) st8_v((T *)e.out_raw + m * e.ld_raw + c0, v);
                     else st8((T *)e.out_raw + m * e.ld_raw + c0, v);
@@ -239,7 +254,7 @@
             __builtin_amdgcn_fence(__ATOMIC_ACQUIRE, "wavefront");
         }
     }
-    if constexpr (SUMS || OSUMS) {
+    if constexpr (SUMS || OSUMS || HINT) {
 #pragma unroll
         for (int q = 0; q < 8; ++q) {
 #pragma unroll
@@ -249,7 +264,7 @@
             }
         }
         if (lane < 8) {
-            float *dst = e.bn_sums + (size_t)(mw >> 7) * 2 * p.Cout + c0;
+            float *dst = (HINT ? e.hint_sums : e.bn_sums) + (size_t)(mw >> 7) * 2 * p.Cout + c0;
             *(float4 *)dst = make_float4(bs1[0], bs1[1], bs1[2], bs1[3]);
             *(float4 *)(dst + 4) = make_float4(bs1[4], bs1[5], bs1[6], bs1[7]);
             *(float4 *)(dst + p.Cout) = make_float4(bs2[0], bs2[1], bs2[2], bs2[3]);
diff --git a/knowledge-distillation-by-replacing-cheap-conv_amd/csrc/conv_igemm.hip b/knowledge-distillation-by-replacing-cheap-conv_amd/csrc/conv_igemm.hip
--- a/knowledge-distillation-by-replacing-cheap-conv_amd/csrc/conv_igemm.hip
+++ b/knowledge-distillation-by-replacing-cheap-conv_amd/csrc/conv_igemm.hip
@@ -954,7 +954,7 @@
         __builtin_amdgcn_sched_barrier(0);
     };
 
-    const int nst_epi = 2 * MI * ((p.ep.out_raw ? 1 : 0) + (p.ep.out_act ? 1 : 0)) + ((NOPS & 12) ? 4 : 0);
+    const int nst_epi = 2 * MI * ((p.ep.out_raw ? 1 : 0) + (p.ep.out_act ? 1 : 0)) + ((NOPS & 12) ? 4 : 0) + ((NOPS & 32) ? 2 * MI + 4 : 0);
     if constexpr (PP) {
         auto offsets = [&](int tile, int &tm0, int &tn0, int &ao, int &bo) {
             int tn, tm;
@@ -1329,7 +1329,11 @@
     }();
     return ncu;
 }
-static ConvSel conv_select_here(const kd_conv_desc *d, const kd_conv_epilogue *ep, int cin1) { return conv_select(d, ep, cin1, conv_ncu(), conv_switches()); }
+static bool hint_asked(const kd_conv_epilogue *ep) { return ep->hint_t || ep->hint_grad || ep->hint_sums; }
+static ConvSel conv_select_here(const kd_conv_desc *d, const kd_conv_epilogue *ep, int cin1)
+{
+    return conv_select(d, ep, cin1, conv_ncu(), conv_switches(), hint_asked(ep));
+}
 
 extern "C" int32_t kd_conv2d_bn_sums_rows(const kd_conv_desc *d, const kd_conv_epilogue *ep)
 {
@@ -1343,6 +1347,13 @@
     if (d->Cout != 256 || ep->ncls < 1 || ep->ncls > 32 || ep->ld_cls < ep->ncls || !kd_aligned16(ep->cls_w)) return 0;
     if (ep->out_raw || ep->out_act || ep->bn_sums || ep->raw_f32) return 0;
     return conv_select_here(d, ep, 0).cls_ok;
+}
+
+extern "C" int32_t kd_conv2d_hint_supported(const kd_conv_desc *d, const kd_conv_epilogue *ep)
+{
+    if (!d || !ep || !ep->hint_t || !ep->hint_grad || !ep->hint_sums || d->dtype != KD_BF16 || d->N <= 0 || d->Ho <= 0 || d->Wo <= 0) return 0;
+    if (ep->ld_hint_t < d->Cout || ep->ld_hint_grad < d->Cout || ep->cls_w || ep->cls_out) return 0;
+    return conv_select_here(d, ep, 0).hint_ok;
 }
 
 static std::atomic<int> g_persist_cus{-1};
@@ -1398,6 +1409,8 @@
     p.tiles_m = sel.tiles_m; p.tiles_n = sel.tiles_n; p.ntiles = sel.ntiles; p.tn_group = sel.tn_group;
     KD_REQUIRE(!ep->bn_sums || kd_conv2d_bn_sums_rows(d, ep) > 0, KD_ERR_UNSUPPORTED,
                "kd_conv2d_fwd: bn_sums is not produced by the kernel this problem selects (ask kd_conv2d_bn_sums_rows first)");
+    KD_REQUIRE(!hint_asked(ep) || (sel.hint_ok && !cls && ep->ld_hint_t >= d->Cout && ep->ld_hint_grad >= d->Cout), KD_ERR_UNSUPPORTED,
+               "kd_conv2d_fwd: the hint block needs conv_igemm_persist_kernel<pp> with out_raw, 16-B friendly hint views and at most one epilogue operand (ask kd_conv2d_hint_supported first)");
     if (ep->bn_sums) KD_NOTE_KERNEL(ep->mask ? "bn_sums_epilogue" : "out_sums_epilogue");
     if (cls) KD_NOTE_KERNEL("cls_epilogue");
     if (x2)
@@ -1435,6 +1448,7 @@
         if (sel.kernel == CONV_IGEMM_PERSIST_PP_DUAL) KD_NOTE_KERNEL("conv_igemm_persist_kernel<pp,dual>");
         else KD_NOTE_KERNEL("conv_igemm_persist_kernel<pp>");
         switch (sel.epi) {
+        KD_CASE(32, conv_igemm_persist_kernel<CfgWide, 32, true>) KD_CASE(33, conv_igemm_persist_kernel<CfgWide, 33, true>)
         KD_CASE(8, conv_igemm_persist_kernel<CfgWide, 8, true>) KD_CASE(0, conv_igemm_persist_kernel<CfgWide, 0, true>) KD_CASE(5, conv_igemm_persist_kernel<CfgWide, 5, true>)
         KD_CASE(6, conv_igemm_persist_kernel<CfgWide, 6, true>) KD_CASE(1, conv_igemm_persist_kernel<CfgWide, 1, true>) KD_CASE(2, conv_igemm_persist_kernel<CfgWide, 2, true>)
         default: KD_LAUNCH(512, conv_igemm_persist_kernel<CfgWide, 3, true>);
diff --git a/knowledge-distillation-by-replacing-cheap-conv_amd/csrc/conv_select.h b/knowledge-distillation-by-replacing-cheap-conv_amd/csrc/conv_select.h
--- a/knowledge-distillation-by-replacing-cheap-conv_amd/csrc/conv_select.h
+++ b/knowledge-distillation-by-replacing-cheap-conv_amd/csrc/conv_select.h
@@ -40,6 +40,7 @@
     int wg_per_cu;
     int sums_rows;
     bool cls_ok, dual_ok;
+    bool hint_ok;
 };
 
 static inline int conv_persist_cus(int n, int ncu)
@@ -55,7 +56,7 @@
     return (unsigned)((nwg + 7) / 8 * 8);
 }
 
-static inline ConvSel conv_select(const kd_conv_desc *d, const kd_conv_epilogue *ep, int cin1, int ncu, const ConvSwitches &sw)
+static inline ConvSel conv_select(const kd_conv_desc *d, const kd_conv_epilogue *ep, int cin1, int ncu, const ConvSwitches &sw, bool hint = false)
 {
     ConvSel c{};
     const bool bf16 = d->dtype == KD_BF16, lw_row = sw.lw != 0, pp_row = sw.pp != 0, dbg = (sw.tune & 512) != 0, sums = ep->bn_sums != nullptr;
@@ -87,6 +88,9 @@
                          (ep->mask ? (use_row_persist || use_igemm_persist || use_pp128) && !(use_row_persist && d->dil > 32) && nops <= 2
                                    : use_igemm_persist && nops == 0 && ep->out_raw && !ep->out_act && !ep->raw_f32 && !sw.lw_pw);
     c.sums_rows = sums_ok ? (int)((long long)d->N * d->Ho * d->Wo / 128) : 0;
+    c.hint_ok = hint && use_igemm_persist && pp_row && !dbg && !sw.lw_pw && nops <= 1 && !sums && ep->out_raw && !ep->raw_f32 &&
+                ep->hint_t && ep->hint_grad && ep->hint_sums && ok(ep->hint_t, ep->ld_hint_t, es) && ok(ep->hint_grad, ep->ld_hint_grad, es) &&
+                ((uintptr_t)ep->hint_sums & 15u) == 0;
     const int pp_epi = (sums && nops >= 1 && nops <= 2) ? (nops | 4) : nops, two_epi = nops < 2 ? nops : 2, lw_epi = nops | (sums ? 4 : 0);
     int bm = 256;
     ConvTile t = CONV_TILE_256;
@@ -100,7 +104,7 @@
     } else if (use_igemm_persist) {
         const bool lw = sw.lw_pw && lw_row && pp_row && d->Cin % 128 == 0 && !dbg && !cin1;
         c.kernel = lw ? CONV_PW_LW : !pp_row ? CONV_IGEMM_PERSIST_LOCKSTEP : cin1 ? CONV_IGEMM_PERSIST_PP_DUAL : CONV_IGEMM_PERSIST_PP;
-        c.epi = lw ? lw_epi : !pp_row ? two_epi : (sums && nops == 0) ? 8 : pp_epi;
+        c.epi = lw ? lw_epi : !pp_row ? two_epi : c.hint_ok ? (nops | 32) : (sums && nops == 0) ? 8 : pp_epi;
         c.wg_per_cu = 1;
     } else if (row_wide && half && bf16) {
         c.kernel = CONV_ROW_HALF; t = CONV_TILE_128_K64;
diff --git a/knowledge-distillation-by-replacing-cheap-conv_amd/csrc/losses.hip b/knowledge-distillation-by-replacing-cheap-conv_amd/csrc/losses.hip
--- a/knowledge-distillation-by-replacing-cheap-conv_amd/csrc/losses.hip
+++ b/knowledge-distillation-by-replacing-cheap-conv_amd/csrc/losses.hip
@@ -1474,6 +1474,39 @@
     hipLaunchKernelGGL(finish_kernel, dim3(1), dim3(256), 0, st, (const double *)partial, sel.blocks, (double)num_classes / (double)numel,
                        (const double *)nullptr, loss);
     KD_CHECK_LAUNCH("kd_hint_mse(finish)");
+    return KD_OK;
+}
+
+namespace {
+constexpr int HINT_FINISH_BLOCKS = 1024;
+__global__ __launch_bounds__(256) void hint_sums_stage_kernel(const float *__restrict__ part, int rows, int C, int rpb, double *partial)
+{
+    const int r0 = blockIdx.x * rpb, r1 = min(rows, r0 + rpb), c4 = C / 4;
+    double acc = 0.0;
+    for (int i = threadIdx.x; i < (r1 - r0) * c4; i += 256) {
+        const int r = r0 + i / c4, c = (i - (i / c4) * c4) * 4;
+        const float4 v = *(const float4 *)(part + (size_t)r * 2 * C + c);
+        acc += ((double)v.x + (double)v.y) + ((double)v.z + (double)v.w);
+    }
+    block_partials<1>({acc}, {partial});
+}
+int hint_finish_rpb(int rows) { return (rows + HINT_FINISH_BLOCKS - 1) / HINT_FINISH_BLOCKS; }
+}
+
+extern "C" int kd_hint_sums_finish(const float *part, int32_t rows, int32_t C, double factor, float *loss, void *workspace,
+                                   size_t workspace_bytes, kd_stream_t stream)
+{
+    KD_REQUIRE(part && loss && workspace, KD_ERR_INVALID, "kd_hint_sums_finish: null argument");
+    KD_REQUIRE(rows > 0 && C > 0 && C % 4 == 0 && kd_aligned16(part), KD_ERR_INVALID, "kd_hint_sums_finish: rows > 0, C a multiple of 4, 16-B aligned rows");
+    static_assert(HINT_FINISH_BLOCKS * sizeof(double) == KD_HINT_SUMS_FINISH_WORKSPACE, "one double per first-stage block");
+    KD_REQUIRE(workspace_bytes >= KD_HINT_SUMS_FINISH_WORKSPACE, KD_ERR_WORKSPACE, "kd_hint_sums_finish: workspace too small");
+    KD_REQUIRE(((uintptr_t)workspace & 7) == 0, KD_ERR_INVALID, "kd_hint_sums_finish: workspace must be 8-B aligned");
+    const int rpb = hint_finish_rpb(rows), blocks = (rows + rpb - 1) / rpb;
+    hipStream_t st = (hipStream_t)stream;
+    hipLaunchKernelGGL(hint_sums_stage_kernel, dim3(blocks), dim3(256), 0, st, part, (int)rows, (int)C, rpb, (double *)workspace);
+    KD_CHECK_LAUNCH("kd_hint_sums_finish(stage)");
+    hipLaunchKernelGGL(finish_kernel, dim3(1), dim3(256), 0, st, (const double *)workspace, blocks, factor, (const double *)nullptr, loss);
+    KD_CHECK_LAUNCH("kd_hint_sums_finish");
     return KD_OK;
 }
 
diff --git a/knowledge-distillation-by-replacing-cheap-conv_amd/engine.py b/knowledge-distillation-by-replacing-cheap-conv_amd/engine.py
--- a/knowledge-distillation-by-replacing-cheap-conv_amd/engine.py
+++ b/knowledge-distillation-by-replacing-cheap-conv_amd/engine.py
@@ -113,6 +113,10 @@
         self.edge_prior = None
         self.exported = None
         self._next_prefix = None
+        self.hint_targets = None
+        self.hint_mse_scale = None
+        self.last_hint_fuses = []
+        self._fuse_state = None
         self.logits_need_grad = False
         self.lazy_logits = os.environ.get("KDCC_LAZY_LOGITS", "1") != "0"
         self._lazy_call = False
@@ -361,9 +365,14 @@
         hints = []
         tape = {"blocks": [], "aspp": None, "hint_slots": [], "pools": {}}
 
-        def note_hint(name, tensor, slot):
+        fuses = []
+        targets = self.hint_targets if (self.hint_mse_scale is not None and self.dtype == torch.bfloat16 and ops.hint_fuse_enabled()) else None
+        self._fuse_state = (hints, targets)
+
+        def note_hint(name, tensor, slot, fuse=None):
             seen.append(name)
             hints.append(tensor)
+            fuses.append(fuse if (fuse is not None and fuse.grad is not None) else None)
             tape["hint_slots"].append(slot)
 
         xin = x.detach()
@@ -432,8 +441,24 @@
         if missing:
             raise EngineError(f"hint layers not found in the student graph: {sorted(missing)}")
         self._tape = tape
+        self._fuse_state = None
         self.last_hint_names = list(seen)
+        self.last_hint_fuses = fuses
         return logits, hints
+
+    def _hint_fuse(self, shape):
+        if self._fuse_state is None or self._fuse_state[1] is None:
+            return None
+        hints, targets = self._fuse_state
+        if len(hints) >= len(targets):
+            return None
+        t = targets[len(hints)]
+        if not torch.is_tensor(t) or t.dim() != 4 or not t.is_cuda or t.dtype != self.dtype:
+            return None
+        tn = t.permute(0, 2, 3, 1)
+        if tuple(tn.shape) != tuple(shape) or not tn.is_contiguous():
+            return None
+        return ops.HintFuse(tn, ops.hint_mse_gscale(tn.numel(), self.hint_mse_scale))
 
     def _aspp_fwd(self, aspp, x7, rg7, want, note_hint, tape):
         N, h8, w8, _ = x7.shape
@@ -463,6 +488,7 @@
             act_gate = _gate_split(br[2])[1] if len(br) > 2 else None
             sc, sh = self._act_fold(br[1], act_gate)
             hinted = site.name in want
+            hf = None
             probed = site.name in self._probes or site.gate is not None
             raw = self._new(N, h8, w8, red) if (hinted or probed) else None
             out = cat[..., red * (i + lead):red * (i + lead + 1)]
@@ -471,15 +497,16 @@
                 mid = mids.get(i)
                 if mid is None:
                     mid = ops.dwconv(x7, self._w_dw(site.mod.separable_conv, False), site.k, site.pad, site.dil)
+                hf = self._hint_fuse(raw.shape) if hinted else None
                 ops.conv2d(mid, self._w_fwd(site.mod.pointwise_conv), out_raw=raw, out_act=out, act_scale=sc, act_shift=sh,
-                           act_relu=True)
+                           act_relu=True, hint=hf)
             elif site.masked:
                 mid = self._masked_fwd(site, x7, out_raw=raw, out_act=out, act_scale=sc, act_shift=sh, act_relu=True)
             else:
                 ops.conv2d(x7, self._w_fwd(site.mod, gate=site.gate), 1, site.pad, site.dil, out_raw=raw, out_act=out, act_scale=sc,
                            act_shift=sh, act_relu=True)
             if hinted:
-                note_hint(site.name, raw, ("aspp", i))
+                note_hint(site.name, raw, ("aspp", i), hf)
             arec["branches"].append({"site": site, "mid": mid, "bn": br[1], "probe_raw": raw if probed else None, "act_gate": act_gate})
             rg_cat = rg_cat or site.trainable or _is_trainable(br[1]) or probed or act_gate is not None
         if "aspp" in want:
@@ -844,9 +871,12 @@
                 act = self._new(N, ho, wo, site.cout)
                 raw = self._new(N, ho, wo, site.cout) if (hinted or probed) else None
                 kw.update(out_raw=raw, out_act=act, act_scale=sc, act_shift=sh, act_relu=True)
+            hf = None
             if site.cheap:
                 mid = ops.dwconv(a, self._w_dw(site.mod.separable_conv, False), site.k, site.pad, site.dil)
-                ops.conv2d(mid, self._w_fwd(site.mod.pointwise_conv), **kw)
+                if hinted and kw.get("out_sums") is None and (not last or sum(nm in want for nm in (site.name, f"{name}.convs", name)) == 1):
+                    hf = self._hint_fuse(raw.shape)
+                ops.conv2d(mid, self._w_fwd(site.mod.pointwise_conv), hint=hf, **kw)
             elif site.masked:
                 mid = self._masked_fwd(site, a, **kw)
             elif last and dual:
@@ -871,10 +901,10 @@
                 if last:
                     for nm in (site.name, f"{name}.convs", name):
                         if nm in want:
-                            note_hint(nm, raw, ("block", bi, "out"))
+                            note_hint(nm, raw, ("block", bi, "out"), hf)
                 else:
                     rec["hint_raw"][i] = raw
-                    note_hint(site.name, raw, ("block", bi, i))
+                    note_hint(site.name, raw, ("block", bi, i), hf)
             if not last:
                 a = act
                 rg = rg or _is_trainable(bns[f"bn{i + 2}"])
@@ -1460,11 +1490,27 @@
 def run_student(engine, x, prefix=None):
     engine._next_prefix = prefix
     engine._lazy_call = True
+    engine.last_hint_fuses = []
     try:
-        return _run_student(engine, x, prefix)
+        logits, hints = _run_student(engine, x, prefix)
     finally:
         engine._next_prefix = None
         engine._lazy_call = False
+    targets, fuses = engine.hint_targets, engine.last_hint_fuses
+    for i, h in enumerate(hints):
+        fuse = fuses[i] if i < len(fuses) else None
+        h._kdcc_hint = HintSlot(engine, fuse, targets[i] if (fuse is not None and targets is not None) else None)
+    engine.last_hint_fuses = []
+    return logits, hints
+
+
+class HintSlot:
+
+    def __init__(self, engine, fuse, target):
+        self.engine, self.fuse, self.target = engine, fuse, target
+
+    def drop(self):
+        self.fuse = self.target = None
 
 
 def _run_student(engine, x, prefix):
diff --git a/knowledge-distillation-by-replacing-cheap-conv_amd/losses/__init__.py b/knowledge-distillation-by-replacing-cheap-conv_amd/losses/__init__.py
--- a/knowledge-distillation-by-replacing-cheap-conv_amd/losses/__init__.py
+++ b/knowledge-distillation-by-replacing-cheap-conv_amd/losses/__init__.py
@@ -16,6 +16,10 @@
             loss, grad = ops.kldiv(s, t, arg, want_grad=want)
         elif kind == "mse":
             loss, grad = ops.hint_mse(s, t, arg, want_grad=want)
+        elif kind == "mse_fused":
+            scale, fuse = arg
+            loss = ops.hint_sums_finish(fuse.part, ops.hint_mse_factor(s.numel(), scale))
+            grad = fuse.grad.permute(0, 3, 1, 2) if want else None
         elif kind == "jsd":
             loss, grad = ops.jsdiv(s, t, arg, want_grad=want)
         elif kind == "ekl":
@@ -38,6 +42,13 @@
         return None, grad * g.to(grad.dtype), None, None, None
 
 
+def _not_plain_mse(inputs):
+    slot = getattr(inputs, "_kdcc_hint", None)
+    if slot is not None:
+        slot.drop()
+        slot.engine.hint_mse_scale = None
+
+
 def _same_device_dtype(inputs, targets):
     if targets.dtype != inputs.dtype and not (targets.dtype in (torch.float32, torch.bfloat16)):
         targets = targets.to(inputs.dtype)
@@ -72,6 +83,13 @@
 
     def forward(self, inputs, targets):
         scale = float(self.num_classes) * (inputs.numel() if self.reduction == 'sum' else 1)
+        slot = getattr(inputs, "_kdcc_hint", None)
+        if slot is not None:
+            fuse, hit = slot.fuse, slot.fuse is not None and slot.target is targets and slot.engine.hint_mse_scale == scale
+            slot.drop()
+            slot.engine.hint_mse_scale = scale
+            if hit:
+                return _FusedLoss.apply("mse_fused", inputs, targets, (scale, fuse), None)
         return _FusedLoss.apply("mse", inputs, _same_device_dtype(inputs, targets), scale, None)
 
 
@@ -83,6 +101,7 @@
         self.num_classes = num_classes
 
     def forward(self, inputs, targets, filter_weight):
+        _not_plain_mse(inputs)
         return _FusedLoss.apply("whmse", inputs, _same_device_dtype(inputs, targets), None, filter_weight)
 
 
@@ -164,6 +183,7 @@
         if targets.dim() != 4 or inputs.shape != targets.shape:
             raise ValueError(f"TopkHintMSELoss: (N,C,H,W) inputs and targets of one shape only, got {tuple(inputs.shape)} and "
                              f"{tuple(targets.shape)}")
+        _not_plain_mse(inputs)
         num_channels = targets.shape[1]
         k = int(self.topk * num_channels)
         if k <= 0:
diff --git a/knowledge-distillation-by-replacing-cheap-conv_amd/models/students/depthwise_student.py b/knowledge-distillation-by-replacing-cheap-conv_amd/models/students/depthwise_student.py
--- a/knowledge-distillation-by-replacing-cheap-conv_amd/models/students/depthwise_student.py
+++ b/knowledge-distillation-by-replacing-cheap-conv_amd/models/students/depthwise_student.py
@@ -295,7 +295,11 @@
             self.teacher_hidden_outputs = thints
             self.prefetch_hits = getattr(self, "prefetch_hits", 0) + 1
             self._prefix = None
-            student_pred, hints = run_student(engine, x)
+            engine.hint_targets = list(thints) if self.save_hidden else None
+            try:
+                student_pred, hints = run_student(engine, x)
+            finally:
+                engine.hint_targets = None
         elif self.overlap_teacher and (not hip_teacher or self.hip_teacher_side_stream):
             if self._side_stream is None or self._side_stream.device != x.device:
                 self._side_stream = torch.cuda.Stream(device=x.device)
@@ -313,7 +317,11 @@
         else:
             self._prefix = None
             teacher_pred = self._teacher_forward(x)
-            student_pred, hints = run_student(engine, x, prefix=self._prefix)
+            engine.hint_targets = list(self.teacher_hidden_outputs) if self.save_hidden else None
+            try:
+                student_pred, hints = run_student(engine, x, prefix=self._prefix)
+            finally:
+                engine.hint_targets = None
             self._prefix = None
         if self.save_hidden:
             self.student_hidden_outputs = hints
diff --git a/knowledge-distillation-by-replacing-cheap-conv_amd/ops.py b/knowledge-distillation-by-replacing-cheap-conv_amd/ops.py
--- a/knowledge-distillation-by-replacing-cheap-conv_amd/ops.py
+++ b/knowledge-distillation-by-replacing-cheap-conv_amd/ops.py
@@ -110,9 +110,37 @@
     """conv2d(..., cls_w=, cls_out=) on a problem whose kernel does not carry the classifier epilogue: store the activation and run the 1x1."""
 
 
+class HintFuse:
+
+    def __init__(self, t, gscale):
+        self.t, self.gscale, self.grad, self.part = t, float(gscale), None, None
+
+
+def hint_mse_gscale(numel, num_classes, grad_scale=1.0):
+    f = lambda v: C.c_float(v).value
+    return f(f(f(f(grad_scale) * 2.0) * f(num_classes)) / f(numel))
+
+
+def hint_mse_factor(numel, num_classes):
+    return C.c_float(num_classes).value / numel
+
+
+def hint_fuse_enabled():
+    return os.environ.get("KDCC_FUSE_HINT", "1") != "0"
+
+
+def hint_sums_finish(part, factor):
+    rows, _, Cc = part.shape
+    loss = torch.empty((), dtype=torch.float32, device=part.device)
+    need = _lib.KD_HINT_SUMS_FINISH_WORKSPACE
+    ws = _ws(need, part.device)
+    check(_lib.lib().kd_hint_sums_finish(_ptr(part), rows, Cc, float(factor), _ptr(loss), _ptr(ws), need, stream_ptr()), "kd_hint_sums_finish")
+    return loss
+
+
 def conv2d(x, w_packed, stride=1, pad=0, dil=1, *, res_pre=None, mask=None, mask_scale=None, res_post=None,
            out_raw=None, out_act=None, act_scale=None, act_shift=None, act_relu=False, algo_cin=None, algo_cout=None, bn_sums=None,
-           x2=None, out_sums=None, cls_w=None, cls_out=None):
+           x2=None, out_sums=None, cls_w=None, cls_out=None, hint=None):
     _need_cuda(x, w_packed)
     N, H, W, Cin = x.shape
     Cout, kh, kw, Cin_w = w_packed.shape
@@ -178,6 +206,17 @@
         if out_rows > 0:
             opart = _scratch((out_rows, 2, Cout), torch.float32, x.device)
             ep.bn_sums = _ptr(opart)
+    hint_bufs = None
+    if hint is not None and out_raw is not None and x.dtype == torch.bfloat16 and out_raw.dtype == x.dtype and cls_w is None and \
+            ep.bn_sums is None and (N * Ho * Wo) % 128 == 0 and hint_fuse_enabled():
+        ep.hint_t, ep.ld_hint_t = _ptr(hint.t), chk(hint.t, "hint.t")
+        hint_bufs = (_scratch((N, Ho, Wo, Cout), x.dtype, x.device), _scratch((N * Ho * Wo // 128, 2, Cout), torch.float32, x.device))
+        ep.hint_grad, ep.ld_hint_grad, ep.hint_gscale, ep.hint_sums = _ptr(hint_bufs[0]), Cout, hint.gscale, _ptr(hint_bufs[1])
+        dq = ConvDesc(dt_of(x), N, H, W, Cin + Cin2, Ho, Wo, Cout, kh, kw, stride, pad, dil, nhwc_ld(x))
+        if not _lib.lib().kd_conv2d_hint_supported(C.byref(dq), C.byref(ep)):
+            ep.hint_t = ep.hint_grad = ep.hint_sums = None
+            ep.ld_hint_t = ep.ld_hint_grad = 0
+            hint_bufs = None
     prof = PROFILER
     if prof is not None:
         e0 = torch.cuda.Event(enable_timing=True)
@@ -191,6 +230,8 @@
         check(_lib.lib().kd_conv2d_fwd(C.byref(d), _ptr(x), _ptr(w_packed), C.byref(ep), stream_ptr()), "kd_conv2d_fwd")
     if out_rows > 0:
         out_sums.append(opart)
+    if hint_bufs is not None:
+        hint.grad, hint.part = hint_bufs
     if prof is not None:
         e1 = torch.cuda.Event(enable_timing=True)
         e1.record()
```

New measurement: 46.09 images/sec, median of 6. No clear change (+0.3%).
